# ajzhai/PEANUT

Measured on AMD Instinct MI355X. Metric: maps/sec for 480x480x(4+N_cat) prediction fwd, batch 32, higher is better.
Workload: dtype f32; 1 GPU; 480x480, 14-channel (4+10) partial maps -> 6-class prediction forward (PSPNet R50-V1c-D8), batch 32 per GPU, seeded random-init weights; survey_config=2, global_batch=32, parallelism=dp1 (map shards, no data-path collective)

## Files before the change

include/peanut_hip.h:

```cpp
#ifndef PEANUT_HIP_H_
#define PEANUT_HIP_H_

#include <stddef.h>
#include <stdint.h>

#ifdef __cplusplus
extern "C" {
#endif

#define PEANUT_OK 0
#define PEANUT_EINVAL (-2)
#define PEANUT_EHIP (-3)
#define PEANUT_EWEIGHTS (-4)
#define PEANUT_ERANGE (-5)

const char* peanut_last_error(void);
const char* peanut_last_conv_kernel(void);
int peanut_abi_version(void);
const char* peanut_build_arch(void);
const char* peanut_source_hash(void);
int peanut_debug_weight_pieces(const float* values, int n, int precision, unsigned short* pieces, float* pack_scale);
int peanut_debug_wino_weights(const float* w_oihw, int cout, int cin, int tile, float* out);
long long peanut_debug_deferred_splitk_count(void);
int peanut_debug_lds_canary(int workgroups, int lds_bytes, int rounds, int* mismatches, void* stream);
// ... 28 lines not shown
#define PEANUT_PREC_FP16X3 2
#define PEANUT_PREC_BF16X6 3

typedef struct peanut_tensor {
  const char* name;
  const float* data;
  int ndim;
  int64_t shape[4];
} peanut_tensor;

typedef struct peanut_pred peanut_pred_t;

int peanut_pred_create(peanut_pred_t** out, const peanut_pred_cfg* cfg, const peanut_tensor* tensors,
                       int n_tensors);
void peanut_pred_destroy(peanut_pred_t* h);

int peanut_pred_forward(peanut_pred_t* h, const float* in_dev, float* out_dev, int B, int H, int W,
                        int apply_sigmoid, void* stream);

size_t peanut_pred_workspace_bytes(peanut_pred_t* h, int B, int H, int W);

double peanut_pred_flops_per_map(peanut_pred_t* h, int H, int W);

int peanut_pred_debug_keep(peanut_pred_t* h, int keep);
int peanut_pred_debug_tensor(peanut_pred_t* h, const char* name, const float** dev_out, int dims[4]);
int peanut_pred_debug_read(peanut_pred_t* h, const char* name, float* dst_dev, size_t max_floats, int dims[4],
                           void* stream);

int peanut_pred_probe_enable(peanut_pred_t* h, int enable);
int peanut_pred_probe_collect(peanut_pred_t* h, int max_ops, const char** names, const char** kernels,
                              double* ms_sum, double* flops, double* bytes, int* n_forwards);
int peanut_pred_use_graph(peanut_pred_t* h, int enable);
int peanut_pred_set_option(peanut_pred_t* h, const char* key, long long value);
int peanut_pred_get_option(peanut_pred_t* h, const char* key, long long* value);


typedef struct peanut_map_cfg {
  int frame_height, frame_width;
  int map_resolution;
  int map_size_cm;
  int global_downscaling;
  int vision_range;
  double hfov;
  int du_scale;
  double cat_pred_threshold, exp_pred_threshold, map_pred_threshold;
  int num_sem_categories;
  double camera_height;
} peanut_map_cfg;

typedef struct peanut_map peanut_map_t;

int peanut_map_create(peanut_map_t** out, const peanut_map_cfg* cfg);
void peanut_map_destroy(peanut_map_t* h);
int peanut_map_dims(peanut_map_t* h, int dims[4]);

int peanut_map_forward(peanut_map_t* h, const float* obs, const float* pose_obs, const float* maps_last,
                       float* poses_inout, float* fp_map_pred, float* map_pred, void* stream);
int peanut_map_mark_agent(float* local_map, int channels, int m, int r0, int r1, int c0, int c1, const uint8_t* selem,
                          int selem_radius, int n_centres, const int* centres_rc, void* stream);
int peanut_map_use_graph(peanut_map_t* h, int enable);

#define PEANUT_MAP_MAX_BATCH 16
int peanut_map_reserve(peanut_map_t* h, int max_batch);
int peanut_map_forward_batch(peanut_map_t* h, int E, const float* obs, const float* pose_obs, const float* const* maps_last,
                             float* poses_inout, float* fp_map_pred, float* const* map_pred, void* stream);
int peanut_map_mark_agent_batch(int E, float* const* local_maps, int channels, int m, const int* squares, const uint8_t* selem,
                                int selem_radius, const int* n_centres, const int* centres_rc, void* stream);
int peanut_map_debug_launches(peanut_map_t* h);

typedef struct peanut_rcnn_cfg {
  int depth;
  int stem_out;
  int res2_out;
  int stride_in_1x1;
  int fpn_out;
  int num_anchors;
  int min_size, max_size;
  int size_divisibility;
  float pixel_mean[3], pixel_std[3];
  float bn_eps;
  int precision;
  int conv_algo;
  float anchor_sizes[5];
  float aspect_ratios[8];
  int rpn_pre_nms_topk;
  int rpn_post_nms_topk;
  float rpn_nms_thresh;
  float rpn_bbox_weights[4];
  int num_classes;
  int box_pooler_resolution, mask_pooler_resolution;
  int fc_dim;
  int mask_conv_dim, num_mask_convs;
  float roi_bbox_weights[4];
  float score_thresh_test;
  float nms_thresh_test;
  int detections_per_image;
  float mask_threshold;
} peanut_rcnn_cfg;

typedef struct peanut_rcnn peanut_rcnn_t;

int peanut_rcnn_create(peanut_rcnn_t** out, const peanut_rcnn_cfg* cfg, const peanut_tensor* tensors, int n_tensors);
void peanut_rcnn_destroy(peanut_rcnn_t* h);
int peanut_rcnn_set_option(peanut_rcnn_t* h, const char* key, long long value);
int peanut_rcnn_plan(peanut_rcnn_t* h, int B, int H, int W, int resized_hw[2], int padded_hw[2], int level_hw[10],
                     size_t* workspace_bytes, double* flops_per_image);
int peanut_rcnn_forward_front(peanut_rcnn_t* h, const uint8_t* img_bgr, int B, int H, int W, float* const* pyramid,
                              float* const* objectness, float* const* deltas, void* stream);

int peanut_rcnn_probe_front(peanut_rcnn_t* h, const uint8_t* img_bgr, int B, int H, int W, int reps, int max_ops,
                            const char** names, const char** kernels, double* ms, double* flops, void* stream);

int peanut_rcnn_set_stage_timing(peanut_rcnn_t* h, int on);
int peanut_rcnn_stage_times(peanut_rcnn_t* h, int max_stages, const char** names, const char** bounds, double* ms, double* work);

int peanut_rcnn_preprocess(peanut_rcnn_t* h, const uint8_t* img_bgr, int B, int H, int W, float* out_nchw, void* stream);

int peanut_rcnn_inference(peanut_rcnn_t* h, const uint8_t* img_bgr, int B, int H, int W, int* n_det_host, float* boxes,
                          float* scores, int32_t* classes, uint8_t* masks, void* stream);
int peanut_rcnn_semantic(peanut_rcnn_t* h, const uint8_t* img_bgr, int B, int H, int W, int n_cats, float sem_pred_prob_thr,
                         float goal_thr, const int32_t* goal_cat_host, float* semantic, int* n_det_host, float* boxes,
                         float* scores, int32_t* classes, uint8_t* masks, void* stream);
int peanut_rcnn_debug_stage(peanut_rcnn_t* h, const char* name, const void** dev, size_t* bytes);

int peanut_roi_align(const float* const* feats, const int* feat_hw, const float* scales, int n_levels, int C,
                     const float* rois, const int* levels, int n_rois, int pooled, int sampling_ratio, int aligned,
                     float* out, void* stream);
size_t peanut_nms_workspace_bytes(int n);
int peanut_nms(const float* boxes_sorted, const int* categories, int n, float iou_threshold, void* workspace,
               unsigned char* keep, void* stream);
int peanut_nms_segments(const float* boxes_sorted, const int* categories, const int* seg_offsets_host, int n_segments,
                        float iou_threshold, void* workspace, unsigned char* keep, void* stream);
int peanut_paste_masks(const float* masks, const float* boxes, int n, int M, int H, int W, float threshold,
                       unsigned char* out, void* stream);

int peanut_preprocess_obs(const uint8_t* rgb, const float* depth, const float* sem, int H, int W, int ncat, int ds,
                          double min_d, double max_d, float* obs, void* stream);
int peanut_preprocess_obs_batch(const uint8_t* rgb, const float* depth, const float* sem, int E, int H, int W, int ncat, int ds,
                                double min_d, double max_d, float* obs, void* stream);

int peanut_seg_accumulate(const uint8_t* masks, const int32_t* classes, const float* scores, int n, int H, int W,
                          int n_cats, float sem_pred_prob_thr, float goal_thr, int goal_cat, float* out,
                          void* stream);

typedef struct peanut_conv peanut_conv_t;
int peanut_conv_create(peanut_conv_t** out, const float* w_oihw_host, const float* scale_host,
                       const float* shift_host, int cout, int cin, int cin_pad, int kh, int kw, int stride,
                       int pad, int dil, int relu, int precision, int conv_algo);
void peanut_conv_destroy(peanut_conv_t* c);
int peanut_conv_precision(peanut_conv_t* c);
int peanut_conv_set_option(peanut_conv_t* c, const char* key, long long value);
int peanut_conv_forward(peanut_conv_t* c, const float* x_dev, const float* x2_dev, int c1, const float* res_dev,
                        float* y_dev, int B, int H, int W, void* stream);

typedef struct peanut_goal peanut_goal_t;
int peanut_goal_create(peanut_goal_t** out, int full_h, int full_w, int col_rad);
void peanut_goal_destroy(peanut_goal_t* g);
int peanut_goal_reset(peanut_goal_t* g);
int peanut_goal_rounds(peanut_goal_t* g);
int peanut_goal_passes(peanut_goal_t* g);
int peanut_goal_converged(peanut_goal_t* g);
int peanut_goal_traversible(peanut_goal_t* g, const float* full_obstacle, const uint8_t* collision_map,
                            const uint8_t* visited_vis, uint8_t* trav_out, void* stream);
int peanut_fmm_distance(peanut_goal_t* g, const uint8_t* traversible, const uint8_t* goal_mask, int goal_r, int goal_c,
                        int fill_mode, double* dist_out, void* stream);
int peanut_goal_select_begin(peanut_goal_t* g, const float* full_obstacle, const uint8_t* collision_map,
                             const uint8_t* visited_vis, const int lmb[4], int loc_r, int loc_c, void* stream);
int peanut_goal_select(peanut_goal_t* g, const float* full_obstacle, const uint8_t* collision_map,
                       const uint8_t* visited_vis, const int lmb[4], int loc_r, int loc_c, const float* target_pred,
                       double dist_weight_temperature, int map_resolution, int goal_rc_out[2], double stats_out[4],
                       double* dist_out, double* value_out, void* stream);
#define PEANUT_GOAL_MAX_BATCH 16
int peanut_goal_select_begin_batch(int E, peanut_goal_t* const* g, const float* const* full_obstacle,
                                   const uint8_t* const* collision_map, const uint8_t* const* visited_vis,
                                   const int* lmb, const int* loc_rc, void* stream);
int peanut_goal_select_batch(int E, peanut_goal_t* const* g, const float* const* full_obstacle,
                             const uint8_t* const* collision_map, const uint8_t* const* visited_vis,
                             const int* lmb, const int* loc_rc, const float* const* target_pred,
                             double dist_weight_temperature, int map_resolution, int* goal_rc_out, double* stats_out,
                             double* const* dist_out, double* const* value_out, void* stream);

#define PEANUT_COMM_ID_BYTES 128
typedef struct peanut_comm peanut_comm_t;
int peanut_comm_unique_id(unsigned char id[PEANUT_COMM_ID_BYTES]);
int peanut_comm_create(peanut_comm_t** out, int n_ranks, int rank, const unsigned char id[PEANUT_COMM_ID_BYTES]);
void peanut_comm_destroy(peanut_comm_t* c);
int peanut_comm_info(peanut_comm_t* c, int* n_ranks, int* rank);
const char* peanut_comm_backend(void);
int peanut_allgather_maps(peanut_comm_t* c, const float* local, float* all, size_t count, void* stream);

#ifdef __cplusplus
}
#endif
#endif
```

peanut_amd/_lib.py:

```python
from __future__ import annotations

import ctypes as C
import os
import threading

import torch

from . import build as _build

_LOCK = threading.Lock()
_LIB = None
ABI_VERSION = 17


class PeanutHipError(RuntimeError):
    pass


class PeanutRangeError(PeanutHipError, FloatingPointError):
    """PEANUT_ERANGE: precision fp16x3 and a value left fp16's exponent range (include/peanut_hip.h)."""


class PredCfgC(C.Structure):
    _fields_ = [
        ("in_channels", C.c_int), ("num_classes", C.c_int),
        ("strides", C.c_int * 4), ("dilations", C.c_int * 4), ("contract_dilation", C.c_int),
        ("pool_scales", C.c_int * 8), ("n_pool_scales", C.c_int),
        ("head_channels", C.c_int), ("align_corners", C.c_int), ("bn_eps", C.c_float),
        ("precision", C.c_int), ("fold_ppm", C.c_int), ("conv_algo", C.c_int),
    ]


class MapCfgC(C.Structure):
    _fields_ = [
        ("frame_height", C.c_int), ("frame_width", C.c_int), ("map_resolution", C.c_int),
        ("map_size_cm", C.c_int), ("global_downscaling", C.c_int), ("vision_range", C.c_int),
        ("hfov", C.c_double), ("du_scale", C.c_int),
        ("cat_pred_threshold", C.c_double), ("exp_pred_threshold", C.c_double),
        ("map_pred_threshold", C.c_double), ("num_sem_categories", C.c_int), ("camera_height", C.c_double),
    ]


class RcnnCfgC(C.Structure):
    _fields_ = [
        ("depth", C.c_int), ("stem_out", C.c_int), ("res2_out", C.c_int), ("stride_in_1x1", C.c_int),
        ("fpn_out", C.c_int), ("num_anchors", C.c_int), ("min_size", C.c_int), ("max_size", C.c_int),
        ("size_divisibility", C.c_int), ("pixel_mean", C.c_float * 3), ("pixel_std", C.c_float * 3),
        ("bn_eps", C.c_float), ("precision", C.c_int), ("conv_algo", C.c_int),
        ("anchor_sizes", C.c_float * 5), ("aspect_ratios", C.c_float * 8),
        ("rpn_pre_nms_topk", C.c_int), ("rpn_post_nms_topk", C.c_int), ("rpn_nms_thresh", C.c_float),
        ("rpn_bbox_weights", C.c_float * 4), ("num_classes", C.c_int), ("box_pooler_resolution", C.c_int),
        ("mask_pooler_resolution", C.c_int), ("fc_dim", C.c_int), ("mask_conv_dim", C.c_int), ("num_mask_convs", C.c_int),
        ("roi_bbox_weights", C.c_float * 4), ("score_thresh_test", C.c_float), ("nms_thresh_test", C.c_float),
        ("detections_per_image", C.c_int), ("mask_threshold", C.c_float),
    ]


class TensorC(C.Structure):
    _fields_ = [("name", C.c_char_p), ("data", C.c_void_p), ("ndim", C.c_int), ("shape", C.c_int64 * 4)]


_P = C.c_void_p
SIGNATURES = {
    "peanut_last_error": (C.c_char_p, []),
    "peanut_last_conv_kernel": (C.c_char_p, []),
    "peanut_abi_version": (C.c_int, []),
    "peanut_build_arch": (C.c_char_p, []),
    "peanut_source_hash": (C.c_char_p, []),
    "peanut_debug_weight_pieces": (C.c_int, [C.c_void_p, C.c_int, C.c_int, C.c_void_p, C.POINTER(C.c_float)]),
    "peanut_debug_wino_weights": (C.c_int, [C.c_void_p, C.c_int, C.c_int, C.c_int, C.c_void_p]),
    "peanut_debug_deferred_splitk_count": (C.c_longlong, []),
    "peanut_debug_lds_canary": (C.c_int, [C.c_int, C.c_int, C.c_int, C.c_void_p, C.c_void_p]),
    "peanut_debug_pkfma_canary": (C.c_int, [C.c_int, C.c_int, C.c_void_p, C.c_void_p]),
    "peanut_pred_create": (C.c_int, [C.POINTER(_P), C.POINTER(PredCfgC), C.POINTER(TensorC), C.c_int]),
    "peanut_pred_destroy": (None, [_P]),
    "peanut_pred_forward": (C.c_int, [_P, _P, _P, C.c_int, C.c_int, C.c_int, C.c_int, _P]),
    "peanut_pred_workspace_bytes": (C.c_size_t, [_P, C.c_int, C.c_int, C.c_int]),
    "peanut_pred_flops_per_map": (C.c_double, [_P, C.c_int, C.c_int]),
    "peanut_pred_debug_keep": (C.c_int, [_P, C.c_int]),
    "peanut_pred_debug_tensor": (C.c_int, [_P, C.c_char_p, C.POINTER(_P), C.POINTER(C.c_int * 4)]),
    "peanut_pred_debug_read": (C.c_int, [_P, C.c_char_p, _P, C.c_size_t, C.POINTER(C.c_int * 4), _P]),
    "peanut_pred_probe_enable": (C.c_int, [_P, C.c_int]),
    "peanut_pred_use_graph": (C.c_int, [_P, C.c_int]),
    "peanut_map_use_graph": (C.c_int, [_P, C.c_int]),
    "peanut_map_mark_agent": (C.c_int, [_P, C.c_int, C.c_int, C.c_int, C.c_int, C.c_int, C.c_int, _P, C.c_int, C.c_int, _P, _P]),
    "peanut_pred_probe_collect": (C.c_int, [_P, C.c_int, C.POINTER(C.c_char_p), C.POINTER(C.c_char_p),
                                            C.POINTER(C.c_double), C.POINTER(C.c_double), C.POINTER(C.c_double),
                                            C.POINTER(C.c_int)]),
    "peanut_map_create": (C.c_int, [C.POINTER(_P), C.POINTER(MapCfgC)]),
    "peanut_map_destroy": (None, [_P]),
    "peanut_map_dims": (C.c_int, [_P, C.POINTER(C.c_int * 4)]),
    "peanut_map_forward": (C.c_int, [_P, _P, _P, _P, _P, _P, _P, _P]),
    "peanut_map_reserve": (C.c_int, [_P, C.c_int]),
    "peanut_map_forward_batch": (C.c_int, [_P, C.c_int, _P, _P, C.POINTER(_P), _P, _P, C.POINTER(_P), _P]),
    "peanut_map_mark_agent_batch": (C.c_int, [C.c_int, C.POINTER(_P), C.c_int, C.c_int, C.POINTER(C.c_int), _P, C.c_int,
                                              C.POINTER(C.c_int), C.POINTER(C.c_int), _P]),
    "peanut_map_debug_launches": (C.c_int, [_P]),
    "peanut_preprocess_obs_batch": (C.c_int, [_P, _P, _P, C.c_int, C.c_int, C.c_int, C.c_int, C.c_int, C.c_double, C.c_double, _P, _P]),
    "peanut_rcnn_create": (C.c_int, [C.POINTER(_P), C.POINTER(RcnnCfgC), C.POINTER(TensorC), C.c_int]),
    "peanut_rcnn_destroy": (None, [_P]),
    "peanut_rcnn_plan": (C.c_int, [_P, C.c_int, C.c_int, C.c_int, C.POINTER(C.c_int * 2), C.POINTER(C.c_int * 2),
                                   C.POINTER(C.c_int * 10), C.POINTER(C.c_size_t), C.POINTER(C.c_double)]),
    "peanut_rcnn_forward_front": (C.c_int, [_P, _P, C.c_int, C.c_int, C.c_int, C.POINTER(_P), C.POINTER(_P),
                                            C.POINTER(_P), _P]),
    "peanut_rcnn_probe_front": (C.c_int, [_P, _P, C.c_int, C.c_int, C.c_int, C.c_int, C.c_int, C.POINTER(C.c_char_p), C.POINTER(C.c_char_p),
                                          C.POINTER(C.c_double), C.POINTER(C.c_double), _P]),
    "peanut_rcnn_set_stage_timing": (C.c_int, [_P, C.c_int]),
    "peanut_rcnn_stage_times": (C.c_int, [_P, C.c_int, C.POINTER(C.c_char_p), C.POINTER(C.c_char_p), C.POINTER(C.c_double), C.POINTER(C.c_double)]),
    "peanut_rcnn_preprocess": (C.c_int, [_P, _P, C.c_int, C.c_int, C.c_int, _P, _P]),
    "peanut_rcnn_inference": (C.c_int, [_P, _P, C.c_int, C.c_int, C.c_int, C.POINTER(C.c_int), _P, _P, _P, _P, _P]),
    "peanut_rcnn_semantic": (C.c_int, [_P, _P, C.c_int, C.c_int, C.c_int, C.c_int, C.c_float, C.c_float, C.POINTER(C.c_int32), _P,
                                       C.POINTER(C.c_int), _P, _P, _P, _P, _P]),
    "peanut_rcnn_debug_stage": (C.c_int, [_P, C.c_char_p, C.POINTER(_P), C.POINTER(C.c_size_t)]),
    "peanut_roi_align": (C.c_int, [C.POINTER(_P), C.POINTER(C.c_int), C.POINTER(C.c_float), C.c_int, C.c_int, _P, _P,
                                   C.c_int, C.c_int, C.c_int, C.c_int, _P, _P]),
    "peanut_nms_workspace_bytes": (C.c_size_t, [C.c_int]),
    "peanut_nms": (C.c_int, [_P, _P, C.c_int, C.c_float, _P, _P, _P]),
    "peanut_nms_segments": (C.c_int, [_P, _P, C.POINTER(C.c_int), C.c_int, C.c_float, _P, _P, _P]),
    "peanut_paste_masks": (C.c_int, [_P, _P, C.c_int, C.c_int, C.c_int, C.c_int, C.c_float, _P, _P]),
    "peanut_preprocess_obs": (C.c_int, [_P, _P, _P, C.c_int, C.c_int, C.c_int, C.c_int, C.c_double, C.c_double, _P, _P]),
    "peanut_seg_accumulate": (C.c_int, [_P, _P, _P, C.c_int, C.c_int, C.c_int, C.c_int, C.c_float, C.c_float,
                                        C.c_int, _P, _P]),
    "peanut_goal_create": (C.c_int, [C.POINTER(_P), C.c_int, C.c_int, C.c_int]),
    "peanut_goal_destroy": (None, [_P]),
    "peanut_goal_reset": (C.c_int, [_P]),
    "peanut_goal_rounds": (C.c_int, [_P]),
    "peanut_goal_passes": (C.c_int, [_P]),
    "peanut_goal_select_begin": (C.c_int, [_P, _P, _P, _P, _P, C.c_int, C.c_int, _P]),
    "peanut_goal_converged": (C.c_int, [_P]),
    "peanut_goal_traversible": (C.c_int, [_P, _P, _P, _P, _P, _P]),
    "peanut_fmm_distance": (C.c_int, [_P, _P, _P, C.c_int, C.c_int, C.c_int, _P, _P]),
    "peanut_goal_select": (C.c_int, [_P, _P, _P, _P, C.POINTER(C.c_int * 4), C.c_int, C.c_int, _P, C.c_double, C.c_int,
                                     C.POINTER(C.c_int * 2), C.POINTER(C.c_double * 4), _P, _P, _P]),
    "peanut_goal_select_begin_batch": (C.c_int, [C.c_int, C.POINTER(_P), C.POINTER(_P), C.POINTER(_P), C.POINTER(_P),
                                                 C.POINTER(C.c_int), C.POINTER(C.c_int), _P]),
    "peanut_goal_select_batch": (C.c_int, [C.c_int, C.POINTER(_P), C.POINTER(_P), C.POINTER(_P), C.POINTER(_P), C.POINTER(C.c_int),
                                           C.POINTER(C.c_int), C.POINTER(_P), C.c_double, C.c_int, C.POINTER(C.c_int),
                                           C.POINTER(C.c_double), C.POINTER(_P), C.POINTER(_P), _P]),
    "peanut_comm_unique_id": (C.c_int, [C.POINTER(C.c_ubyte * 128)]),
    "peanut_comm_create": (C.c_int, [C.POINTER(_P), C.c_int, C.c_int, C.POINTER(C.c_ubyte * 128)]),
    "peanut_comm_destroy": (None, [_P]),
    "peanut_comm_info": (C.c_int, [_P, C.POINTER(C.c_int), C.POINTER(C.c_int)]),
    "peanut_comm_backend": (C.c_char_p, []),
    "peanut_allgather_maps": (C.c_int, [_P, _P, _P, C.c_size_t, _P]),
    "peanut_conv_create": (C.c_int, [C.POINTER(_P), _P, _P, _P] + [C.c_int] * 11),
    "peanut_conv_destroy": (None, [_P]),
    "peanut_conv_precision": (C.c_int, [_P]),
    "peanut_conv_forward": (C.c_int, [_P, _P, _P, C.c_int, _P, _P, C.c_int, C.c_int, C.c_int, _P]),
    "peanut_set_default_option": (C.c_int, [C.c_char_p, C.c_longlong]),
    "peanut_get_default_option": (C.c_int, [C.c_char_p, C.POINTER(C.c_longlong)]),
    "peanut_option_list": (C.c_char_p, []),
    "peanut_pred_set_option": (C.c_int, [_P, C.c_char_p, C.c_longlong]),
    "peanut_pred_get_option": (C.c_int, [_P, C.c_char_p, C.POINTER(C.c_longlong)]),
    "peanut_conv_set_option": (C.c_int, [_P, C.c_char_p, C.c_longlong]),
    "peanut_rcnn_set_option": (C.c_int, [_P, C.c_char_p, C.c_longlong]),
}


CONV_ALGOS = {"auto": 0, "direct": 1}
PRECISIONS = {"fp32": 0, "bf16x3": 1, "fp16x3": 2, "bf16x6": 3}


def lib_path() -> str:
    return os.environ.get("PEANUT_HIP_LIB", _build.LIB_PATH)


def _stale_reason(lib, path) -> str:
    if path != _build.LIB_PATH or not os.path.isdir(_build.CSRC):
        return ""
    have = (lib.peanut_source_hash() or b"").decode()
    want = _build.source_hash()
    return "" if have == want else f"built from sources {have or '<unknown>'}, the tree holds {want}"


def load() -> C.CDLL:
    global _LIB
    with _LOCK:
        if _LIB is not None:
            return _LIB
        path = lib_path()
        if path == _build.LIB_PATH and os.path.exists(path) and os.path.isdir(_build.CSRC) and _build._built_hash() and \
                _build._built_hash() != _build.source_hash():
            try:
                _build.build()
            except Exception as e:
                raise PeanutHipError(f"{path} is stale (csrc/ changed since it was built) and rebuilding failed: {e}") from e
        if not os.path.exists(path):
            raise PeanutHipError(
                f"HIP extension not built: {path} is missing. Build it with "
                "`python -c 'import __graft_entry__ as g; g.build()'` (or `python -m peanut_amd.build`). "
                "peanut_amd has no CPU fallback.")
        try:
            lib = C.CDLL(path, mode=C.RTLD_LOCAL)
        except OSError as e:
            raise PeanutHipError(f"failed to load {path}: {e}") from e
        for name, (res, args) in SIGNATURES.items():
            try:
                fn = getattr(lib, name)
            except AttributeError as e:
                raise PeanutHipError(f"{path} does not export {name}; rebuild the extension") from e
            fn.restype = res
            fn.argtypes = args
        got = lib.peanut_abi_version()
        if got != ABI_VERSION:
            raise PeanutHipError(f"{path} implements ABI version {got}, this package binds version {ABI_VERSION}: "
                                 "rebuild the extension (python -m peanut_amd.build --force)")
        why = _stale_reason(lib, path)
        if why:
            raise PeanutHipError(f"{path} is stale: {why}.  Rebuild it (python -m peanut_amd.build --force); a stale kernel "
                                 "library must not answer for the sources next to it")
        _LIB = lib
        return lib


_OPTION_LOCK = threading.RLock()


class default_options:

    def __init__(self, **options):
        self.options = {k: int(v) for k, v in options.items()}
        self.saved = {}

    def __enter__(self):
        lib = load()
        _OPTION_LOCK.acquire()
        try:
            for k, v in self.options.items():
                old = C.c_longlong()
                check(lib.peanut_get_default_option(k.encode(), C.byref(old)), "peanut_get_default_option")
                self.saved[k] = old.value
                check(lib.peanut_set_default_option(k.encode(), v), "peanut_set_default_option")
        except Exception:
            self.__exit__(None, None, None)
            raise
        return self

    def __exit__(self, *exc):
        lib = load()
        try:
            for k, v in self.saved.items():
                lib.peanut_set_default_option(k.encode(), v)
            self.saved = {}
        finally:
            _OPTION_LOCK.release()
        return False


def check(rc: int, what: str = "") -> None:
    if rc != 0:
        msg = load().peanut_last_error()
        if rc == -5:
            raise PeanutRangeError(f"{what} failed (code {rc}): {msg.decode() if msg else ''}")
        raise PeanutHipError(f"{what} failed (code {rc}): {msg.decode() if msg else ''}")


def current_stream_ptr(device=None) -> int:
    return int(torch.cuda.current_stream(device).cuda_stream)
```

peanut_amd/csrc/common.h:

```cpp
#pragma once
#include <hip/hip_runtime.h>
#include <stdint.h>
#include <string>

namespace peanut {

void set_error(const std::string& msg);
int fail(int code, const std::string& msg);
void note_kernel(const char* family);
const char* noted_kernel();

#define PEANUT_HIP_CHECK(expr)                                                            \
  do {                                                                                    \
    hipError_t _e = (expr);                                                               \
    if (_e != hipSuccess)                                                                 \
      return ::peanut::fail(-3, std::string(#expr) + ": " + hipGetErrorString(_e));       \
  } while (0)

struct ConvDesc {
  int cin;
  int cout;
  int kh, kw, stride, pad, dil;
  int relu;
  int bn_tile;
  int bk;
  int cout_pad;
  const float* w_packed;
  const float* scale;
  const float* shift;
  int rs;
  const void* w_s;
  int s_planes;
  float s_alpha;
  int flush_ch;
};

struct DeferredSplit {
  bool valid;
  const float* partial;
  int split_p, ntiles, M, cout, relu;
  const float* scale;
  const float* shift;
  float alpha;
};

struct ConvArgs {
  const float* x;
  const float* x2;
  const float* res;
  float* y;
  int B, H, W;
  int c1, c2;
  int Ho, Wo;
  float* ws;
  size_t ws_floats;
  int mt_per_group;
  size_t w_group_stride;
  int ss_group_stride;
  int group_valid_rows;
  DeferredSplit* defer;
  const int* group_rows;
};

constexpr size_t kSplitKScratchFloats = (size_t)48 << 20;
constexpr size_t kSplitKSideFloats = (size_t)8 << 20;

#if defined(__HIP_DEVICE_COMPILE__)
#define PEANUT_NO_PK_F32 __attribute__((target("no-packed-fp32-ops")))
#else
#define PEANUT_NO_PK_F32
#endif

__device__ __forceinline__ float paste_value(const float* __restrict__ m, int M, const float* __restrict__ bx, int x, int y) {
#pragma clang fp contract(off)
  const float gx = ((float)x + 0.5f - bx[0]) / (bx[2] - bx[0]) * 2.f - 1.f;
  const float gy = ((float)y + 0.5f - bx[1]) / (bx[3] - bx[1]) * 2.f - 1.f;
  const float ix = ((gx + 1.f) * (float)M - 1.f) / 2.f, iy = ((gy + 1.f) * (float)M - 1.f) / 2.f;
  const float fx = floorf(ix), fy = floorf(iy);
  const int x0 = (int)fminf(fmaxf(fx, -2.f), (float)M + 1.f), y0 = (int)fminf(fmaxf(fy, -2.f), (float)M + 1.f);
  if (x0 < -1 || x0 >= M || y0 < -1 || y0 >= M) return 0.f;
  const float lx = ix - fx, ly = iy - fy;
  const float wx = 1.f - lx, wy = 1.f - ly;
  auto at = [&](int yy, int xx) -> float {
    return ((unsigned)yy < (unsigned)M && (unsigned)xx < (unsigned)M) ? m[yy * M + xx] : 0.f;
  };
  return at(y0, x0) * wy * wx + at(y0, x0 + 1) * wy * lx + at(y0 + 1, x0) * ly * wx + at(y0 + 1, x0 + 1) * ly * lx;
}

inline int conv_out_dim(int n, int k, int s, int p, int d) { return (n + 2 * p - d * (k - 1) - 1) / s + 1; }

void conv_pick_tiles(int cin_pad, int cout, int* bn_tile, int* bk, bool pointwise = false);
size_t conv_packed_floats(int cin_pad, int cout, int kh, int kw, int bn_tile);
void pack_conv_weights(const float* w_oihw, int cout, int cin_real, int cin_pad, int kh, int kw,
                       int bn_tile, int bk, float* out);
int launch_conv(const ConvDesc& d, const ConvArgs& a, hipStream_t stream);
bool conv_pw_enabled();
bool conv_pw_uses_256(int cout, long long M, int mt_per_group, int bn_tile, int cin);
int conv_pw_256_min_k();
bool conv_pw_uses_256w(int cout, long long M, int mt_per_group, int bn_tile, int cin, int flush_ktiles);
bool conv_pw_narrow_tiles(int cin, int cout, long long M, int bn_tile, int mt_per_group);
bool conv_pw_uses_256p(int cout, long long M, int mt_per_group, int bn_tile, int cin, int flush_ktiles, long long in_pixels = 0);
struct ConvKParams;
bool gemm_skinny_takes(const ConvKParams& p, int bn_tile, size_t ws_floats);
int launch_gemm_skinny(const ConvKParams& p, float* ws, size_t ws_floats, hipStream_t stream);
bool conv_pw_uses_256wp(int cout, long long M, int stride, int mt_per_group, int bn_tile, int c1, int c2, int flush_ktiles);
bool conv_pw_uses_ares(int cin, int cout, long long M, int stride, bool two_source, int flush_ktiles, int bn_tile);

bool conv_patch_eligible(const ConvDesc& d, const ConvArgs& a);
const char* conv_patch_kernel_name(const ConvDesc& d, bool nchw);
bool conv_patch_nchw_eligible(const ConvDesc& d, int B, int Ho, int Wo, int creal);
int launch_conv_patch_nchw(const ConvDesc& d, const float* x_nchw, int creal, float* y, int B, int H, int W, int Ho, int Wo, hipStream_t stream);

void wino_geometry(int B, int H, int W, int dil, int* th, int* tw, long long* n_tiles, long long* m_pad, int gran = 128, int m = 4);
void wino_transform_weights(const float* w_oihw, int cout, int cin, float* out, int m = 4);
int launch_wino_input(const float* x, float* V, int B, int H, int W, int C, int dil, hipStream_t s, int gran = 128, int m = 4, long long m_pad_total = 0,
                      const DeferredSplit* df = nullptr);
bool wino_input_accepts_deferred(int B, int H, int W, int C, int dil, int gran, int m);
long long wino_deferred_count();
int launch_wino_output(const float* Mb, const float* scale, const float* shift, const float* res, float* y,
                       int B, int H, int W, int C, int dil, int relu, hipStream_t s, int gran = 128, int m = 4, long long m_pad_total = 0);

bool gemm_rs_uses_256(int cout, long long M, int mt_per_group, int bn_tile, int cin);
const char* gemm_rs_kernel_name(int cout, long long M, int mt_per_group, int bn_tile, int cin, int planes);
size_t sx_packed_bytes(int cin_pad, int cout, int bn_tile, int planes);
void pack_weights_sx(const float* w, int cout, int cin_real, int cin_pad, int bn_tile, int planes, float wscale, void* out);
float sx_pack_scale(const float* w, size_t n, int planes);
size_t sx_conv_packed_bytes(int cin_pad, int cout, int kh, int kw, int bn_tile, int planes);
void pack_weights_sx_conv(const float* w_oihw, int cout, int cin_real, int cin_pad, int kh, int kw, int bn_tile, int planes,
                          float wscale, void* out);

int launch_nchw_to_nhwc_pad(const float* x, float* y, int B, int C, int H, int W, int Cpad, hipStream_t s);
int launch_maxpool3x3s2(const float* x, float* y, int B, int H, int W, int C, int Ho, int Wo, hipStream_t s);
int launch_ppm_pool(const float* x, float* out, int B, int H, int W, int C, const int* scales, int nscales,
                    hipStream_t s, int scale_rows = 0);
size_t ppm_pool_scratch_floats(int B, int H, int C, const int* scales, int nscales);
int launch_ppm_pool2(const float* x, float* scratch, float* out, int B, int H, int W, int C, const int* scales,
                     int nscales, hipStream_t s, int scale_rows = 0);
int launch_ppm_upsample_concat(const float* table, float* out, int B, int H, int W, int Cp, const int* scales,
                               int nscales, int align_corners, hipStream_t s);
int launch_ppm_conv_term(const float* Q, float* R, int B, int H, int W, int C, const int* scales, int nscales,
                         int align_corners, hipStream_t s, int scale_rows = 0);
int launch_upsample_logits(const float* lo, float* out, int B, int h, int w, int K, int H, int W,
                           int align_corners, int sigmoid, hipStream_t s);

}
```

peanut_amd/csrc/conv_common.h:

```cpp
#pragma once
#include <stdlib.h>

#include <atomic>

#include "common.h"
#include "options.h"

namespace peanut {

typedef float f32x16 __attribute__((ext_vector_type(16)));
typedef float f32x4 __attribute__((ext_vector_type(4)));

__device__ __forceinline__ float relu_keep_nan(float v) { return v < 0.f ? 0.f : v; }
__device__ __forceinline__ f32x4 relu_keep_nan(f32x4 v) {
  return f32x4{relu_keep_nan(v.x), relu_keep_nan(v.y), relu_keep_nan(v.z), relu_keep_nan(v.w)};
}

struct ConvKParams {
  const float* x;
  const float* x2;
  const float* w;
  const float* scale;
  const float* shift;
  const float* res;
  const float* zeros;
  float* y;
  int H, W, c1, c2, Ho, Wo, cout;
  int kw, ntaps, stride, pad, dil, relu;
  int M, nkt, ntiles, HoWo;
  int n_full, n_sp, split_p;
  float* partial;
  int mt_per_group;
  long long w_group_stride;
  int ss_group_stride;
  int mtiles;
  int nchunk;
  int res_prefetch;
  float alpha;
  int ares_pbn;
  int phase_shift;
  int sk_units, sk_maxp, sk_g, sk_q;
  int pack_bn;
  int group_valid;
  int p_order;
  float* dump;
  int stagger;
  int flush;
  DeferredSplit* defer;
  const int* group_rows;
};

template <int I>
struct IC { static constexpr int value = I; };
template <int N, int I = 0, class F>
__device__ __forceinline__ void static_for(F&& f) {
  if constexpr (I < N) {
    f(IC<I>{});
    static_for<N, I + 1>(f);
  }
}

struct KIter {
  int tap, ky, kx, cbase;
  const float* wtile;
};


const float* zero_page();
bool conv_pw_enabled();
int launch_conv_pw(const ConvKParams& p, int bn_tile, float* ws, size_t ws_floats, hipStream_t stream);
int launch_conv_pw_ares(const ConvKParams& p, int bn_tile, hipStream_t stream);
int launch_conv_pw256p(const ConvKParams& p, float* ws, size_t ws_floats, hipStream_t stream);
int launch_conv_pw256wp(const ConvKParams& p, float* ws, size_t ws_floats, hipStream_t stream);
int launch_conv_patch(const ConvKParams& p, const ConvDesc& d, int B, hipStream_t stream);
int launch_gemm_rs(const ConvKParams& p, int bn_tile, int planes, float* ws, size_t ws_floats, hipStream_t stream);
int launch_conv_rs(const ConvKParams& p, int bn_tile, int planes, float* ws, size_t ws_floats, hipStream_t stream);


struct Work { int mt, nt, kt0, kt1, item; };

__host__ __device__ __forceinline__ int sk_owner(long long U, int G, long long u) {
  int w = (int)(u * G / U);
  while (w + 1 < G && U * (w + 1) / G <= u) ++w;
  while (w > 0 && U * w / G > u) --w;
  return w;
}

__device__ __forceinline__ void tile_to_mn(const ConvKParams& p, int tile, int* mt_out, int* nt_out) {
  int mt, nt;
  if (p.nchunk > 0 && p.ntiles > p.nchunk) {
    const int full = p.ntiles / p.nchunk, rem = p.ntiles - full * p.nchunk;
    const int per_chunk = p.mtiles * p.nchunk;
    if (tile < full * per_chunk) {
      const int c = tile / per_chunk, r = tile - c * per_chunk;
      mt = r / p.nchunk;
      nt = c * p.nchunk + (r - mt * p.nchunk);
    } else {
      const int r = tile - full * per_chunk;
      mt = r / rem;
      nt = full * p.nchunk + (r - mt * rem);
    }
  } else {
    mt = tile / p.ntiles;
    nt = tile - mt * p.ntiles;
  }
  *mt_out = mt;
  *nt_out = nt;
}

__device__ __forceinline__ Work decode_work(const ConvKParams& p) {
  const int G = gridDim.x, bid = blockIdx.x;
  const int q = G >> 3, r = G & 7, xcd = bid & 7, local = bid >> 3;
  const int sq = p.n_sp >> 3, sr = p.n_sp & 7;
  const int sp_x = sq + (xcd < sr), sp_before = xcd * sq + (xcd < sr ? xcd : sr);
  const int chunk_before = xcd * q + (xcd < r ? xcd : r);
  Work w;
  int tile;
  if (local < sp_x) {
    const int s = sp_before + local;
    const int j = s / p.split_p, part = s - j * p.split_p;
    tile = p.n_full + j;
    w.item = s;
    w.kt0 = (int)((long long)part * p.nkt / p.split_p);
    w.kt1 = (int)((long long)(part + 1) * p.nkt / p.split_p);
  } else {
    tile = (chunk_before - sp_before) + (local - sp_x);
    w.item = -1;
    w.kt0 = 0;
    w.kt1 = p.nkt;
  }
  tile_to_mn(p, tile, &w.mt, &w.nt);
  return w;
}

constexpr int kResPrefetchRows = 8;
struct ResPrefetch { f32x4 v[kResPrefetchRows]; bool on; };

template <int BM, int BN, int EP, int NT>
__device__ __forceinline__ ResPrefetch conv_res_prefetch(const ConvKParams& p, const Work& wk, int m0, int n0) {
  constexpr int NV = BN / 4, ROWS_PER_PASS = NT / NV, ER = BM / EP;
  const int tid = threadIdx.x;
  const int c4 = (tid % NV) * 4, r0 = tid / NV, n = n0 + c4;
  ResPrefetch r;
  r.on = p.res_prefetch && p.res && wk.item < 0 && (p.cout & 3) == 0 && n < p.cout;
  if (r.on) {
#pragma unroll
    for (int i = 0; i < kResPrefetchRows; ++i) {
      const int row = r0 + i * ROWS_PER_PASS, m = m0 + row;
      r.v[i] = (row < ER && m < p.M) ? *reinterpret_cast<const f32x4*>(p.res + (size_t)m * p.cout + n) : f32x4{0.f, 0.f, 0.f, 0.f};
    }
  }
  return r;
}

template <int BM, int BN, int WM, int WN, int EP, int NT = 256, int MI = 0, int NI = 0>
__device__ __forceinline__ void conv_epilogue(const ConvKParams& p, const Work& wk, f32x16 (&acc)[MI][NI], float* smem,
                                              int m0, int n0, const ResPrefetch* early = nullptr) {
  constexpr int TM = BM / WM, TN = BN / WN;
  constexpr int CS = BN + 4, ER = BM / EP;
  static_assert(MI == TM / 32 && NI == TN / 32, "accumulator shape");
  const int tid = threadIdx.x;
  const int lane = tid & 63, wave = tid >> 6;
  const int wm = wave / WN, wn = wave % WN;
  const int li = lane & 31, hi = lane >> 5;
  constexpr int NV = BN / 4;
  constexpr int ROWS_PER_PASS = NT / NV;
  const int c4 = (tid % NV) * 4, r0 = tid / NV;
  const int n = n0 + c4;
  const int ss_off = (p.mt_per_group && p.ss_group_stride) ? (wk.mt / p.mt_per_group) * p.ss_group_stride : 0;
  const f32x4 sc = *reinterpret_cast<const f32x4*>(p.scale + ss_off + n) * p.alpha;
  const f32x4 sh = *reinterpret_cast<const f32x4*>(p.shift + ss_off + n);
  const bool vec_ok = (p.cout & 3) == 0;
  constexpr int PRE = kResPrefetchRows;
  const ResPrefetch rp = early ? *early : conv_res_prefetch<BM, BN, EP, NT>(p, wk, m0, n0);
  const f32x4 (&rpre)[PRE] = rp.v;
  const bool pre = rp.on;
#pragma unroll
  for (int ep = 0; ep < EP; ++ep) {
    if (EP == 1 || wm == ep) {
#pragma unroll
      for (int t = 0; t < MI; ++t)
#pragma unroll
        for (int u = 0; u < NI; ++u)
#pragma unroll
          for (int r = 0; r < 16; ++r) {
            const int row = wm * TM + t * 32 + (r & 3) + 8 * (r >> 2) + 4 * hi - ep * ER;
            smem[row * CS + wn * TN + u * 32 + li] = acc[t][u][r];
          }
    }
    __syncthreads();
    if (wk.item >= 0) {
      float* dst = p.partial + (size_t)wk.item * (BM * BN) + (size_t)ep * ER * BN;
      for (int row = r0; row < ER; row += ROWS_PER_PASS)
        *reinterpret_cast<f32x4*>(dst + row * BN + c4) = *reinterpret_cast<const f32x4*>(smem + row * CS + c4);
    } else {
      int row_first = r0;
      if (pre && ep == 0) {
#pragma unroll
        for (int i = 0; i < PRE; ++i) {
          const int row = r0 + i * ROWS_PER_PASS, m = m0 + row;
          if (row < ER && m < p.M) {
            f32x4 v = *reinterpret_cast<const f32x4*>(smem + row * CS + c4);
            v = v * sc + sh;
// ... 193 lines not shown
```

peanut_amd/csrc/conv_igemm.hip:

```cpp
#include <stdlib.h>

#include "conv_common.h"

namespace peanut {

template <int BN, int BK, int A_PER>
__device__ __forceinline__ void prep_addr(const ConvKParams& p, KIter& it, const int (&a_iy0)[A_PER],
                                          const int (&a_ix0)[A_PER], const int (&a_pix)[A_PER], int a_c4,
                                          unsigned long long (&a_addr)[A_PER], const float*& b_tile) {
  const bool second = it.cbase >= p.c1;
  const float* src = second ? p.x2 : p.x;
  const int C = second ? p.c2 : p.c1, cb = second ? it.cbase - p.c1 : it.cbase;
  const int dy = it.ky * p.dil, dx = it.kx * p.dil;
  static_for<A_PER>([&](auto J) __attribute__((always_inline)) {
    constexpr int j = decltype(J)::value;
    const int iy = a_iy0[j] + dy, ix = a_ix0[j] + dx;
    const bool ok = (unsigned)iy < (unsigned)p.H && (unsigned)ix < (unsigned)p.W;
    const float* ptr = src + (size_t)(a_pix[j] + iy * p.W + ix) * C + cb + a_c4;
    const unsigned long long m = ok ? ~0ull : 0ull;
    a_addr[j] = ((unsigned long long)ptr & m) | ((unsigned long long)p.zeros & ~m);
  });
  b_tile = it.wtile;
  it.wtile += BN * BK;
  const int tap1 = it.tap + 1, kx1 = it.kx + 1;
// ... 100 lines not shown
#define PEANUT_STORE_TILES(stage) store_tiles<BM, BN, BK, A_PER, B_PER>(stage, tid, ra, rb)

  const int lane = tid & 63, wave = tid >> 6;
  const int wm = wave / WN, wn = wave % WN;
  const int li = lane & 31, hi = lane >> 5;
  const int a_off = (wm * TM + li) * LS + hi * 4;
  const int b_off = BM * LS + (wn * TN + li) * LS + hi * 4;

  f32x16 acc[MI][NI];
#pragma unroll
  for (int t = 0; t < MI; ++t)
#pragma unroll
    for (int u = 0; u < NI; ++u)
#pragma unroll
      for (int r = 0; r < 16; ++r) acc[t][u][r] = 0.f;

  PEANUT_PREP_ADDR();
  PEANUT_ISSUE_LOADS();
  PEANUT_STORE_TILES(smem);
  PEANUT_PREP_ADDR();
  if (nk > 1) PEANUT_ISSUE_LOADS();
  PEANUT_PREP_ADDR();
  __syncthreads();

  constexpr int KH = BK / 16;
  f32x4 afA[KH][MI], bfA[KH][NI], afB[KH][MI], bfB[KH][NI];
#define PEANUT_LOAD_FRAGS(af, bf, stage, half)                                                           \
  _Pragma("unroll") for (int j = 0; j < KH; ++j) {                                                       \
    _Pragma("unroll") for (int t = 0; t < MI; ++t)                                                       \
      af[j][t] = *reinterpret_cast<const f32x4*>((stage) + a_off + t * 32 * LS + ((half) * KH + j) * 8); \
    _Pragma("unroll") for (int u = 0; u < NI; ++u)                                                       \
      bf[j][u] = *reinterpret_cast<const f32x4*>((stage) + b_off + u * 32 * LS + ((half) * KH + j) * 8); \
  }
#define PEANUT_MFMA_HALF(af, bf)                                                                         \
  _Pragma("unroll") for (int j = 0; j < KH; ++j)                                                         \
    _Pragma("unroll") for (int kk = 0; kk < 4; ++kk)                                                     \
      _Pragma("unroll") for (int t = 0; t < MI; ++t)                                                     \
        _Pragma("unroll") for (int u = 0; u < NI; ++u)                                                   \
          acc[t][u] = __builtin_amdgcn_mfma_f32_32x32x2f32(af[j][t][kk], bf[j][u][kk], acc[t][u], 0, 0, 0);

  PEANUT_LOAD_FRAGS(afA, bfA, smem, 0);
  int kt = 0;
  for (; kt + 2 < nk; ++kt) {
    float* const nxt = smem + ((kt + 1) & 1) * STAGE;
    const float* const cur = smem + (kt & 1) * STAGE;
    PEANUT_STORE_TILES(nxt);
    PEANUT_ISSUE_LOADS();
    PEANUT_LOAD_FRAGS(afB, bfB, cur, 1);
    __builtin_amdgcn_sched_barrier(0);
    PEANUT_PREP_ADDR();
    PEANUT_MFMA_HALF(afA, bfA);
    __builtin_amdgcn_sched_barrier(0);
    __syncthreads();
    PEANUT_LOAD_FRAGS(afA, bfA, nxt, 0);
    __builtin_amdgcn_sched_barrier(0);
    PEANUT_MFMA_HALF(afB, bfB);
    __builtin_amdgcn_sched_barrier(0);
  }
  if (kt + 1 < nk) {
    float* const nxt = smem + ((kt + 1) & 1) * STAGE;
    const float* const cur = smem + (kt & 1) * STAGE;
    PEANUT_STORE_TILES(nxt);
    PEANUT_LOAD_FRAGS(afB, bfB, cur, 1);
    __builtin_amdgcn_sched_barrier(0);
    PEANUT_MFMA_HALF(afA, bfA);
    __builtin_amdgcn_sched_barrier(0);
    __syncthreads();
    PEANUT_LOAD_FRAGS(afA, bfA, nxt, 0);
    __builtin_amdgcn_sched_barrier(0);
    PEANUT_MFMA_HALF(afB, bfB);
    __builtin_amdgcn_sched_barrier(0);
    ++kt;
  }
  {
    const float* const cur = smem + (kt & 1) * STAGE;
    PEANUT_LOAD_FRAGS(afB, bfB, cur, 1);
    __builtin_amdgcn_sched_barrier(0);
    PEANUT_MFMA_HALF(afA, bfA);
    PEANUT_MFMA_HALF(afB, bfB);
  }
  __syncthreads();
#undef PEANUT_LOAD_FRAGS
#undef PEANUT_MFMA_HALF

  conv_epilogue<BM, BN, WM, WN, EP>(p, wk, acc, smem, m0, n0);
}

const float* zero_page() {
  static float* pages[64] = {nullptr};
  int dev = 0;
  if (hipGetDevice(&dev) != hipSuccess || dev < 0 || dev >= 64) return nullptr;
  if (!pages[dev]) {
    float* ptr = nullptr;
    if (hipMalloc(&ptr, 4096) != hipSuccess) return nullptr;
    if (hipMemset(ptr, 0, 4096) != hipSuccess) return nullptr;
    pages[dev] = ptr;
  }
  return pages[dev];
}

void conv_pick_tiles(int cin_pad, int cout, int* bn_tile, int* bk, bool pointwise) {
  const int forced_bk = (int)opt(OPT_FP32_BK);
  *bk = (cin_pad % 32 == 0) ? 32 : 16;
  if (forced_bk == 16) *bk = 16;
  *bn_tile = cout >= 128 ? 128 : (cout > 32 ? 64 : 32);
  const int bn64_maxk = (int)opt(pointwise ? OPT_PW_BN64_MAXK : OPT_BN64_MAXK);
  if (*bn_tile == 128 && cin_pad <= bn64_maxk) *bn_tile = 64;
}

size_t conv_packed_floats(int cin_pad, int cout, int kh, int kw, int bn_tile) {
  const int cout_pad = (cout + bn_tile - 1) / bn_tile * bn_tile;
  return (size_t)cout_pad * kh * kw * cin_pad;
}

void pack_conv_weights(const float* w, int cout, int cin_real, int cin_pad, int kh, int kw, int bn_tile,
                       int bk, float* out) {
  const int ntaps = kh * kw;
  const int cout_pad = (cout + bn_tile - 1) / bn_tile * bn_tile;
  const int nchunks = cin_pad / bk;
  const int nkt = nchunks * ntaps;
  for (int n = 0; n < cout_pad; ++n) {
    const int nt = n / bn_tile, nn = n % bn_tile;
    for (int ch = 0; ch < nchunks; ++ch)
      for (int tap = 0; tap < ntaps; ++tap) {
        float* dst = out + (((size_t)nt * nkt + (size_t)ch * ntaps + tap) * bn_tile + nn) * bk;
        for (int c = 0; c < bk; ++c) {
          const int ci = ch * bk + c;
          dst[c] = (n < cout && ci < cin_real) ? w[((size_t)n * cin_real + ci) * ntaps + tap] : 0.f;
        }
      }
  }
}

template <int BM, int BN, int BK, int WM, int WN>
static int launch_t(const ConvKParams& p, float* ws, size_t ws_floats, hipStream_t stream) {
  static SlotCache slots;
  return launch_with_tail_split<decltype(&conv_igemm_kernel<BM, BN, BK, WM, WN>), BM, BN>(
      &conv_igemm_kernel<BM, BN, BK, WM, WN>, p, ws, ws_floats, stream, &slots);
}

int launch_conv(const ConvDesc& d, const ConvArgs& a, hipStream_t stream) {
  if (a.c1 + a.c2 != d.cin) return fail(-2, "launch_conv: c1 + c2 != cin");
  const bool rs_fallback = d.rs == 1 && a.c2 != 0 && d.stride != 1;
  const int kgran = (d.rs && !rs_fallback) ? 16 : d.bk;
  if (a.c1 % kgran != 0 || (a.c2 % kgran) != 0) return fail(-2, "launch_conv: channel split not a multiple of the k-tile");
  ConvKParams p{};
  p.x = a.x; p.x2 = a.x2 ? a.x2 : a.x; p.w = d.w_packed; p.scale = d.scale; p.shift = d.shift;
  p.res = a.res; p.y = a.y;
  p.zeros = zero_page();
  if (!p.zeros) return fail(-3, "launch_conv: zero page allocation failed");
  p.H = a.H; p.W = a.W; p.c1 = a.c1; p.c2 = a.c2; p.Ho = a.Ho; p.Wo = a.Wo; p.cout = d.cout;
  p.kw = d.kw; p.ntaps = d.kh * d.kw; p.stride = d.stride; p.pad = d.pad; p.dil = d.dil; p.relu = d.relu;
  p.HoWo = a.Ho * a.Wo;
  const long long M = (long long)a.B * p.HoWo;
  if (M <= 0 || M > 0x7fffffffLL || (long long)a.B * a.H * a.W > 0x7fffffffLL)
    return fail(-2, "launch_conv: problem size out of range");
  p.M = (int)M;
  p.nkt = (d.cin / d.bk) * p.ntaps;
  p.ntiles = d.cout_pad / d.bn_tile;
  p.n_full = 0; p.n_sp = 0; p.split_p = 1; p.partial = nullptr;
  p.alpha = 1.f;
  p.flush = (d.rs && !rs_fallback) ? 0 : d.flush_ch / d.bk;
  p.mt_per_group = a.mt_per_group; p.w_group_stride = (long long)a.w_group_stride; p.ss_group_stride = a.ss_group_stride;
  p.group_valid = a.mt_per_group ? a.group_valid_rows : 0;
  if (a.defer) a.defer->valid = false;
  p.defer = a.defer;
  p.group_rows = a.mt_per_group ? a.group_rows : nullptr;
  if (d.rs && !rs_fallback) {
    if (!d.w_s) return fail(-2, "launch_conv: register-split layer without pre-split weights");
    p.w = static_cast<const float*>(d.w_s);
    p.nkt = (d.cin / 16) * p.ntaps;
    p.alpha = d.s_alpha;
    if (d.rs == 2) return launch_conv_rs(p, d.bn_tile, d.s_planes, a.ws, a.ws_floats, stream);
    return launch_gemm_rs(p, d.bn_tile, d.s_planes, a.ws, a.ws_floats, stream);
  }
  if (d.bk == 32 && p.ntaps == 1 && p.pad == 0 && p.c1 % 32 == 0 && p.c2 % 32 == 0 && (p.c2 == 0 || p.stride == 1) && conv_pw_enabled())
    return launch_conv_pw(p, d.bn_tile, a.ws, a.ws_floats, stream);
  if (conv_patch_eligible(d, a)) return launch_conv_patch(p, d, a.B, stream);
  {
    static const char* const names[2][3] = {{"conv_igemm_128x128x32", "conv_igemm_128x64x32", "conv_igemm_128x32x32"},
                                            {"conv_igemm_128x128x16", "conv_igemm_128x64x16", "conv_igemm_128x32x16"}};
    note_kernel(names[d.bk == 32 ? 0 : 1][d.bn_tile == 128 ? 0 : (d.bn_tile == 64 ? 1 : 2)]);
  }
  if (d.bk == 32) {
    if (d.bn_tile == 128) return launch_t<128, 128, 32, 2, 2>(p, a.ws, a.ws_floats, stream);
    if (d.bn_tile == 64) return launch_t<128, 64, 32, 2, 2>(p, a.ws, a.ws_floats, stream);
    if (d.bn_tile == 32) return launch_t<128, 32, 32, 4, 1>(p, a.ws, a.ws_floats, stream);
  } else if (d.bk == 16) {
    if (d.bn_tile == 128) return launch_t<128, 128, 16, 2, 2>(p, a.ws, a.ws_floats, stream);
    if (d.bn_tile == 64) return launch_t<128, 64, 16, 2, 2>(p, a.ws, a.ws_floats, stream);
    if (d.bn_tile == 32) return launch_t<128, 32, 16, 4, 1>(p, a.ws, a.ws_floats, stream);
  }
  return fail(-2, "launch_conv: unsupported tile configuration");
}

}
```

peanut_amd/csrc/conv_pw.hip:

```cpp
#include <stdlib.h>

#include "common.h"
#include "conv_common.h"

namespace peanut {

namespace {

typedef const __attribute__((address_space(1))) void* gptr_t;
typedef __attribute__((address_space(3))) void* lptr_t;

template <int BN, int WM, int WN>
__global__ __launch_bounds__(256) __attribute__((amdgpu_waves_per_eu(BN == 128 ? 2 : (BN == 64 ? 3 : 4))))
void conv_pw_glds_kernel(const ConvKParams p) {
  constexpr int BM = 128, BK = 32;
  constexpr int TM = BM / WM, TN = BN / WN;
  constexpr int MI = TM / 32, NI = TN / 32;
  constexpr int A_FLOATS = BM * BK, B_FLOATS = BN * BK, STAGE = A_FLOATS + B_FLOATS;
  constexpr int A_INSTR = BM / 32, B_INSTR = BN / 32;
  constexpr int CS = BN + 4;
  constexpr int EP = (BM * CS > 2 * STAGE) ? WM : 1;
  constexpr int ER = BM / EP;
  constexpr int SMEM_FLOATS = (2 * STAGE > ER * CS) ? 2 * STAGE : ER * CS;
  static_assert(WM * WN == 4 && TM % 32 == 0 && TN % 32 == 0, "4 waves, wave tile a multiple of 32x32");
  __shared__ __attribute__((aligned(1024))) float smem[SMEM_FLOATS];

  const int tid = threadIdx.x;
  const Work wk = decode_work(p);
  const int mt = wk.mt, nt = wk.nt, nk = wk.kt1 - wk.kt0;
  const int m0 = mt * BM, n0 = nt * BN;
  const int lane = tid & 63;
  const int wave = __builtin_amdgcn_readfirstlane(tid >> 6);
  const int lr = lane >> 3, lp = lane & 7;

  const float* a_src[A_INSTR];
  const float* a_src2[A_INSTR];
#pragma unroll
  for (int j = 0; j < A_INSTR; ++j) {
    const int r = (wave * A_INSTR + j) * 8 + lr;
    const int m = m0 + r;
    const int mc = m < p.M ? m : p.M - 1;
    const int b = mc / p.HoWo;
    const int rem = mc - b * p.HoWo;
    const int oy = rem / p.Wo, ox = rem - oy * p.Wo;
    const size_t pix = (size_t)b * p.H * p.W + (size_t)oy * p.stride * p.W + (size_t)ox * p.stride;
    const int c = lp ^ ((r >> 1) & 7);
    const int k1 = p.c1 / BK;
    a_src[j] = wk.kt0 < k1 ? p.x + pix * p.c1 + (size_t)wk.kt0 * BK + c * 4 : p.x2 + pix * p.c2 + (size_t)(wk.kt0 - k1) * BK + c * 4;
    a_src2[j] = p.x2 + pix * p.c2 + c * 4;
  }
  int to_switch = p.c2 ? p.c1 / BK - wk.kt0 : 0x7fffffff;
  const float* b_src[B_INSTR];
  {
    const int pack = p.pack_bn > BN ? p.pack_bn : BN;
    const int n_row = nt * BN;
    const float* wtile = p.w + (p.mt_per_group ? (size_t)(mt / p.mt_per_group) * p.w_group_stride : 0) +
                         ((size_t)(n_row / pack) * p.nkt + wk.kt0) * ((size_t)pack * BK) + (size_t)(n_row % pack) * BK;
#pragma unroll
    for (int j = 0; j < B_INSTR; ++j) {
      const int r = (wave * B_INSTR + j) * 8 + lr;
      const int c = lp ^ ((r >> 1) & 7);
      b_src[j] = wtile + r * BK + c * 4;
    }
  }
  const int b_step = (p.pack_bn > BN ? p.pack_bn : BN) * BK;
#define PEANUT_DMA_TILE(stage)                                                                                   \
  {                                                                                                              \
    if (to_switch-- == 0) {                                                                                      \
      _Pragma("unroll") for (int j = 0; j < A_INSTR; ++j) a_src[j] = a_src2[j];                                  \
    }                                                                                                            \
    _Pragma("unroll") for (int j = 0; j < A_INSTR; ++j) {                                                        \
      __builtin_amdgcn_global_load_lds((gptr_t)a_src[j], (lptr_t)((stage) + (wave * A_INSTR + j) * 256), 16, 0, 0); \
      a_src[j] += BK;                                                                                            \
    }                                                                                                            \
    _Pragma("unroll") for (int j = 0; j < B_INSTR; ++j) {                                                        \
      __builtin_amdgcn_global_load_lds((gptr_t)b_src[j], (lptr_t)((stage) + A_FLOATS + (wave * B_INSTR + j) * 256), 16, 0, 0); \
      b_src[j] += b_step;                                                                                        \
    }                                                                                                            \
  }
#define PEANUT_DMA_LANDED_BARRIER()          \
  asm volatile("s_waitcnt vmcnt(0)" ::: "memory"); \
  __syncthreads();

  const int wm = wave / WN, wn = wave % WN;
  const int li = lane & 31, hi = lane >> 5;
  const int swz = (li >> 1) & 7;
  int sw[BK / 8];
#pragma unroll
  for (int ks = 0; ks < BK / 8; ++ks) sw[ks] = ((ks * 2 + hi) ^ swz) * 4;
  const int a_row = (wm * TM + li) * BK;
  const int b_row = A_FLOATS + (wn * TN + li) * BK;

  f32x16 acc[MI][NI];
#pragma unroll
  for (int t = 0; t < MI; ++t)
#pragma unroll
    for (int u = 0; u < NI; ++u)
#pragma unroll
      for (int r = 0; r < 16; ++r) acc[t][u][r] = 0.f;
  PEANUT_FLUSH_DECL();

  constexpr int KH = BK / 16;
  f32x4 afA[KH][MI], bfA[KH][NI], afB[KH][MI], bfB[KH][NI];
#define PEANUT_LOAD_FRAGS(af, bf, stage, half)                                                          \
  _Pragma("unroll") for (int j = 0; j < KH; ++j) {                                                      \
    _Pragma("unroll") for (int t = 0; t < MI; ++t)                                                      \
      af[j][t] = *reinterpret_cast<const f32x4*>((stage) + a_row + t * 32 * BK + sw[(half) * KH + j]);  \
    _Pragma("unroll") for (int u = 0; u < NI; ++u)                                                      \
      bf[j][u] = *reinterpret_cast<const f32x4*>((stage) + b_row + u * 32 * BK + sw[(half) * KH + j]);  \
  }
#define PEANUT_MFMA_HALF(af, bf)                                                                        \
  _Pragma("unroll") for (int j = 0; j < KH; ++j)                                                        \
    _Pragma("unroll") for (int kk = 0; kk < 4; ++kk)                                                    \
      _Pragma("unroll") for (int t = 0; t < MI; ++t)                                                    \
        _Pragma("unroll") for (int u = 0; u < NI; ++u)                                                  \
          acc[t][u] = __builtin_amdgcn_mfma_f32_32x32x2f32(af[j][t][kk], bf[j][u][kk], acc[t][u], 0, 0, 0);

  PEANUT_DMA_TILE(smem);
  PEANUT_DMA_LANDED_BARRIER();
  PEANUT_LOAD_FRAGS(afA, bfA, smem, 0);

  int kt = 0;
  for (; kt + 1 < nk; ++kt) {
    float* const nxt = smem + ((kt + 1) & 1) * STAGE;
    const float* const cur = smem + (kt & 1) * STAGE;
    PEANUT_DMA_TILE(nxt);
    PEANUT_LOAD_FRAGS(afB, bfB, cur, 1);
    __builtin_amdgcn_sched_barrier(0);
    PEANUT_MFMA_HALF(afA, bfA);
    __builtin_amdgcn_sched_barrier(0);
    PEANUT_DMA_LANDED_BARRIER();
    PEANUT_LOAD_FRAGS(afA, bfA, nxt, 0);
    __builtin_amdgcn_sched_barrier(0);
    PEANUT_MFMA_HALF(afB, bfB);
    __builtin_amdgcn_sched_barrier(0);
    PEANUT_FLUSH_STEP();
  }
  const ResPrefetch rp = conv_res_prefetch<BM, BN, EP, 256>(p, wk, m0, n0);
  {
    const float* const cur = smem + (kt & 1) * STAGE;
    PEANUT_LOAD_FRAGS(afB, bfB, cur, 1);
    __builtin_amdgcn_sched_barrier(0);
    PEANUT_MFMA_HALF(afA, bfA);
    PEANUT_MFMA_HALF(afB, bfB);
  }
  PEANUT_FLUSH_FINISH();
  __syncthreads();
#undef PEANUT_LOAD_FRAGS
#undef PEANUT_MFMA_HALF
#undef PEANUT_DMA_TILE
#undef PEANUT_DMA_LANDED_BARRIER

  conv_epilogue<BM, BN, WM, WN, EP>(p, wk, acc, smem, m0, n0, &rp);
}

__global__ __launch_bounds__(512) void conv_pw_glds256_kernel(const ConvKParams p) {
  constexpr int BM = 256, BN = 128, BK = 32, WM = 4, WN = 2, NT = 512, STAGES = 3;
  constexpr int TM = BM / WM, TN = BN / WN;
  constexpr int MI = TM / 32, NI = TN / 32;
  constexpr int A_FLOATS = BM * BK, B_FLOATS = BN * BK, STAGE = A_FLOATS + B_FLOATS;
  constexpr int A_INSTR = BM / 64, B_INSTR = BN / 64;
  constexpr int CS = BN + 4;
  constexpr int SMEM_FLOATS = (STAGES * STAGE > BM * CS) ? STAGES * STAGE : BM * CS;
  __shared__ __attribute__((aligned(1024))) float smem[SMEM_FLOATS];

  const int tid = threadIdx.x;
  const Work wk = decode_work(p);
  const int mt = wk.mt, nt = wk.nt, nk = wk.kt1 - wk.kt0;
  const int m0 = mt * BM, n0 = nt * BN;
  const int lane = tid & 63;
  const int wave = __builtin_amdgcn_readfirstlane(tid >> 6);
  const int lr = lane >> 3, lp = lane & 7;

  const float* a_src[A_INSTR];
  const float* a_src2[A_INSTR];
#pragma unroll
  for (int j = 0; j < A_INSTR; ++j) {
    const int r = (wave * A_INSTR + j) * 8 + lr;
    const int m = m0 + r;
    const int mc = m < p.M ? m : p.M - 1;
    const int b = mc / p.HoWo;
    const int rem = mc - b * p.HoWo;
    const int oy = rem / p.Wo, ox = rem - oy * p.Wo;
    const size_t pix = (size_t)b * p.H * p.W + (size_t)oy * p.stride * p.W + (size_t)ox * p.stride;
    const int c = lp ^ ((r >> 1) & 7);
    const int k1 = p.c1 / BK;
    a_src[j] = wk.kt0 < k1 ? p.x + pix * p.c1 + (size_t)wk.kt0 * BK + c * 4 : p.x2 + pix * p.c2 + (size_t)(wk.kt0 - k1) * BK + c * 4;
    a_src2[j] = p.x2 + pix * p.c2 + c * 4;
  }
  int to_switch = p.c2 ? p.c1 / BK - wk.kt0 : 0x7fffffff;
  const float* b_src[B_INSTR];
  {
    const float* wtile = p.w + (p.mt_per_group ? (size_t)(mt / p.mt_per_group) * p.w_group_stride : 0) +
                         ((size_t)nt * p.nkt + wk.kt0) * (BN * BK);
#pragma unroll
    for (int j = 0; j < B_INSTR; ++j) {
      const int r = (wave * B_INSTR + j) * 8 + lr;
      const int c = lp ^ ((r >> 1) & 7);
      b_src[j] = wtile + r * BK + c * 4;
    }
  }
#define PW256_DMA_TILE(stage)                                                                                    \
// ... 90 lines not shown
#undef PW256_MFMA_GROUP
  PEANUT_FLUSH_FINISH();
  conv_epilogue<BM, BN, WM, WN, 1, NT>(p, wk, acc, smem, m0, n0);
}

__global__ __launch_bounds__(512) void conv_pw_glds256w_kernel(const ConvKParams p) {
  constexpr int BM = 256, BN = 256, BK = 32, WM = 4, WN = 2, NT = 512, STAGES = 2;
  constexpr int TM = BM / WM, TN = BN / WN;
  constexpr int MI = TM / 32, NI = TN / 32;
  constexpr int A_FLOATS = BM * BK, B_FLOATS = BN * BK, STAGE = A_FLOATS + B_FLOATS;
  constexpr int A_INSTR = BM / 64, B_INSTR = BN / 64;
  constexpr int CS = BN + 4, ER = BM / WM;
  constexpr int SMEM_FLOATS = (STAGES * STAGE > ER * CS) ? STAGES * STAGE : ER * CS;
  __shared__ __attribute__((aligned(1024))) float smem[SMEM_FLOATS];

  const int tid = threadIdx.x;
  const Work wk = decode_work(p);
  const int mt = wk.mt, nt = wk.nt, nk = wk.kt1 - wk.kt0;
  const int m0 = mt * BM, n0 = nt * BN;
  const int lane = tid & 63;
  const int wave = __builtin_amdgcn_readfirstlane(tid >> 6);
  const int lr = lane >> 3, lp = lane & 7;

  const float* a_src[A_INSTR];
  const float* a_src2[A_INSTR];
#pragma unroll
  for (int j = 0; j < A_INSTR; ++j) {
    const int r = (wave * A_INSTR + j) * 8 + lr;
    const int m = m0 + r;
    const int mc = m < p.M ? m : p.M - 1;
    const int b = mc / p.HoWo;
    const int rem = mc - b * p.HoWo;
    const int oy = rem / p.Wo, ox = rem - oy * p.Wo;
    const size_t pix = (size_t)b * p.H * p.W + (size_t)oy * p.stride * p.W + (size_t)ox * p.stride;
    const int c = lp ^ ((r >> 1) & 7);
    const int k1 = p.c1 / BK;
    a_src[j] = wk.kt0 < k1 ? p.x + pix * p.c1 + (size_t)wk.kt0 * BK + c * 4 : p.x2 + pix * p.c2 + (size_t)(wk.kt0 - k1) * BK + c * 4;
    a_src2[j] = p.x2 + pix * p.c2 + c * 4;
  }
  int to_switch = p.c2 ? p.c1 / BK - wk.kt0 : 0x7fffffff;
  const float* b_src[B_INSTR];
#pragma unroll
  for (int j = 0; j < B_INSTR; ++j) {
    const int r = (wave * B_INSTR + j) * 8 + lr;
    const int c = lp ^ ((r >> 1) & 7);
    b_src[j] = p.w + ((size_t)(2 * nt + (r >> 7)) * p.nkt + wk.kt0) * (128 * BK) + (r & 127) * BK + c * 4;
  }
#define PW256W_DMA_TILE(stage)                                                                                   \
  {                                                                                                              \
    if (to_switch-- == 0) {                                                                                      \
      _Pragma("unroll") for (int j = 0; j < A_INSTR; ++j) a_src[j] = a_src2[j];                                  \
    }                                                                                                            \
    _Pragma("unroll") for (int j = 0; j < A_INSTR; ++j) {                                                        \
      __builtin_amdgcn_global_load_lds((gptr_t)a_src[j], (lptr_t)((stage) + (wave * A_INSTR + j) * 256), 16, 0, 0); \
      a_src[j] += BK;                                                                                            \
    }                                                                                                            \
    _Pragma("unroll") for (int j = 0; j < B_INSTR; ++j) {                                                        \
      __builtin_amdgcn_global_load_lds((gptr_t)b_src[j], (lptr_t)((stage) + A_FLOATS + (wave * B_INSTR + j) * 256), 16, 0, 0); \
      b_src[j] += 128 * BK;                                                                                      \
    }                                                                                                            \
  }
#define PW256W_BARRIER()                                  \
  asm volatile("s_waitcnt lgkmcnt(0)" ::: "memory");      \
  __builtin_amdgcn_s_barrier();                           \
  asm volatile("" ::: "memory");

  const int wm = wave / WN, wn = wave % WN;
  const int li = lane & 31, hi = lane >> 5;
  const int swz = (li >> 1) & 7;
  int sw[BK / 8];
#pragma unroll
  for (int ks = 0; ks < BK / 8; ++ks) sw[ks] = ((ks * 2 + hi) ^ swz) * 4;
  const int a_row = (wm * TM + li) * BK;
  const int b_row = A_FLOATS + (wn * TN + li) * BK;

  f32x16 acc[MI][NI];
#pragma unroll
  for (int t = 0; t < MI; ++t)
#pragma unroll
    for (int u = 0; u < NI; ++u)
#pragma unroll
      for (int r = 0; r < 16; ++r) acc[t][u][r] = 0.f;

  PW256W_DMA_TILE(smem);
  asm volatile("s_waitcnt vmcnt(0)" ::: "memory");
  PW256W_BARRIER();
  const bool late = p.phase_shift && wave >= 4;
#define PW256W_READ_PAIR(g)                                                                                          \
  _Pragma("unroll") for (int j = 0; j < 2; ++j) {                                                                    \
    _Pragma("unroll") for (int t = 0; t < MI; ++t) af[j][t] = *reinterpret_cast<const f32x4*>(cur + a_row + t * 32 * BK + sw[(g) + j]); \
    _Pragma("unroll") for (int u = 0; u < NI; ++u) bf[j][u] = *reinterpret_cast<const f32x4*>(cur + b_row + u * 32 * BK + sw[(g) + j]); \
  }
#define PW256W_MFMA_PAIR()                                                                                \
  _Pragma("unroll") for (int j = 0; j < 2; ++j)                                                           \
    _Pragma("unroll") for (int kk = 0; kk < 4; ++kk)                                                      \
      _Pragma("unroll") for (int t = 0; t < MI; ++t)                                                      \
        _Pragma("unroll") for (int u = 0; u < NI; ++u)                                                    \
          acc[t][u] = __builtin_amdgcn_mfma_f32_32x32x2f32(af[j][t][kk], bf[j][u][kk], acc[t][u], 0, 0, 0);
  for (int kt = 0; kt < nk; ++kt) {
    const float* const cur = smem + (kt & 1) * STAGE;
    float* const fill = smem + ((kt + 1) & 1) * STAGE;
    const bool more = kt + 1 < nk;
    if (more && !late) PW256W_DMA_TILE(fill);
    f32x4 af[2][MI], bf[2][NI];
    PW256W_READ_PAIR(0);
    PW256W_MFMA_PAIR();
    __builtin_amdgcn_sched_barrier(0);
    if (more && late) PW256W_DMA_TILE(fill);
    __builtin_amdgcn_sched_barrier(0);
    PW256W_READ_PAIR(2);
    PW256W_MFMA_PAIR();
    asm volatile("s_waitcnt vmcnt(0)" ::: "memory");
    PW256W_BARRIER();
  }
#undef PW256W_DMA_TILE
#undef PW256W_BARRIER
#undef PW256W_READ_PAIR
#undef PW256W_MFMA_PAIR
  conv_epilogue<BM, BN, WM, WN, WM, NT>(p, wk, acc, smem, m0, n0);
}

template <int BN, int WM, int WN>
int launch_pw_t(const ConvKParams& p, float* ws, size_t ws_floats, hipStream_t stream) {
  static SlotCache slots;
  return launch_with_tail_split<decltype(&conv_pw_glds_kernel<BN, WM, WN>), 128, BN>(&conv_pw_glds_kernel<BN, WM, WN>, p, ws,
                                                                                      ws_floats, stream, &slots);
}

}

bool conv_pw_enabled() { return opt(OPT_PW_GLDS) != 0; }

int conv_pw_256_min_k() { return (int)opt(OPT_PW256_MINK); }
bool conv_pw_uses_256(int cout, long long M, int mt_per_group, int bn_tile, int cin) {
  const long long min_tiles = opt(OPT_PW256_MINTILES);
  return bn_tile == 128 && cin >= conv_pw_256_min_k() && mt_per_group % 2 == 0 && M * cout >= min_tiles * 256 * 128;
}

bool conv_pw_uses_256w(int cout, long long M, int mt_per_group, int bn_tile, int cin, int flush) {
  const int min_k = (int)opt(OPT_PW256W_MINK);
  const long long min_tiles = opt(OPT_PW256W_MINTILES);
  return min_k > 0 && bn_tile == 128 && cout % 256 == 0 && mt_per_group == 0 && flush == 0 && cin >= min_k &&
         ((M + 255) / 256) * (cout / 256) >= min_tiles;
}

bool conv_pw_narrow_tiles(int cin, int cout, long long M, int bn_tile, int mt_per_group) {
  (void)mt_per_group;
  if (bn_tile != 128 || cin > opt(OPT_BN64_MAXK) || cout % 128 != 0) return false;
  return ((M + 127) / 128) * (cout / 128) < opt(OPT_PW64_MAXTILES);
}

int launch_conv_pw(const ConvKParams& p, int bn_tile, float* ws, size_t ws_floats, hipStream_t stream) {
  const int phase_shift_w = opt(OPT_PW256_PHASE) != 0;
  if (gemm_skinny_takes(p, bn_tile, ws ? ws_floats : 0)) return launch_gemm_skinny(p, ws, ws_floats, stream);
  if (conv_pw_uses_256wp(p.cout, p.M, p.stride, p.mt_per_group, bn_tile, p.c1, p.c2, p.flush)) {
    const int rc = launch_conv_pw256wp(p, ws, ws_floats, stream);
    if (rc != 1) return rc;
  }
  if (conv_pw_uses_ares(p.c1, p.cout, p.M, p.stride, p.c2 != 0, p.flush, bn_tile)) return launch_conv_pw_ares(p, bn_tile, stream);
  if (conv_pw_uses_256w(p.cout, p.M, p.mt_per_group, bn_tile, p.c1 + p.c2, p.flush)) {
    static SlotCache slots256w;
    ConvKParams q = p;
    q.ntiles = p.cout / 256;
    q.phase_shift = phase_shift_w;
    note_kernel("conv_pw_glds_256x256");
    return launch_with_tail_split<decltype(&conv_pw_glds256w_kernel), 256, 256, 512>(&conv_pw_glds256w_kernel, q, ws, ws_floats, stream,
                                                                                      &slots256w);
  }
  if (conv_pw_uses_256p(p.cout, p.M, p.mt_per_group, bn_tile, p.c1 + p.c2, p.flush, (long long)(p.M / p.HoWo) * p.H * p.W) && !(p.flush && p.res)) {
    const int rc = launch_conv_pw256p(p, ws, ws_floats, stream);
    if (rc != 1) return rc;
  }
  if (conv_pw_uses_256(p.cout, p.M, p.mt_per_group, bn_tile, p.c1 + p.c2)) {
    static SlotCache slots256;
    ConvKParams q = p;
    if (q.mt_per_group) q.mt_per_group /= 2;
    q.phase_shift = phase_shift_w;
    if (opt(OPT_PW256_SKIP_PAD) == 0) q.group_valid = 0;
    note_kernel("conv_pw_glds_256x128");
    return launch_with_tail_split<decltype(&conv_pw_glds256_kernel), 256, 128, 512>(&conv_pw_glds256_kernel, q, ws, ws_floats, stream,
                                                                                     &slots256);
  }
  if (conv_pw_narrow_tiles(p.c1 + p.c2, p.cout, p.M, bn_tile, p.mt_per_group)) {
    ConvKParams q = p;
    q.pack_bn = 128;
    q.ntiles = p.ntiles * 2;
    note_kernel("conv_pw_glds_128x64");
    return launch_pw_t<64, 2, 2>(q, ws, ws_floats, stream);
  }
  note_kernel(bn_tile == 128 ? "conv_pw_glds_128x128" : (bn_tile == 64 ? "conv_pw_glds_128x64" : "conv_pw_glds_128x32"));
  if (bn_tile == 128) return launch_pw_t<128, 2, 2>(p, ws, ws_floats, stream);
  if (bn_tile == 64) return launch_pw_t<64, 2, 2>(p, ws, ws_floats, stream);
  if (bn_tile == 32) return launch_pw_t<32, 4, 1>(p, ws, ws_floats, stream);
  return fail(-2, "launch_conv_pw: unsupported tile configuration");
}

}
```

peanut_amd/csrc/conv_pw256p.hip:

```cpp
#include <stdlib.h>

#include "common.h"
#include "conv_common.h"

namespace peanut {

namespace {

typedef const __attribute__((address_space(1))) void* gptr_t;
typedef __attribute__((address_space(3))) void* lptr_t;

__device__ __forceinline__ float p_load_uncounted(const float* base, unsigned byte_off) {
  float v;
  asm volatile("s_nop 4\n\tglobal_load_dword %0, %1, %2" : "=v"(v) : "v"(byte_off), "s"(base) : "memory");
  return v;
}
template <int N>
__device__ __forceinline__ void p_wait(const float (&r)[8], float a, float b, float c, float d) {
  __builtin_amdgcn_sched_barrier(0);
  if constexpr (N == 6)
    asm volatile("s_waitcnt vmcnt(6)" ::"v"(r[0]), "v"(r[1]), "v"(r[2]), "v"(r[3]), "v"(r[4]), "v"(r[5]), "v"(r[6]), "v"(r[7]), "v"(a), "v"(b),
                 "v"(c), "v"(d)
                 : "memory");
  else
    asm volatile("s_waitcnt vmcnt(0)" ::"v"(r[0]), "v"(r[1]), "v"(r[2]), "v"(r[3]), "v"(r[4]), "v"(r[5]), "v"(r[6]), "v"(r[7]), "v"(a), "v"(b),
                 "v"(c), "v"(d)
                 : "memory");
  __builtin_amdgcn_sched_barrier(0);
}

struct PItem { int mt, nt, kt0, kt1, part; };

template <bool RAGGED, bool FLUSH>
__global__ __launch_bounds__(512) void conv_pw_glds256p_kernel(const ConvKParams p) {
  constexpr int BM = 256, BN = 128, BK = 32, WN = 2;
  constexpr int A_FLOATS = BM * BK, B_FLOATS = BN * BK, STAGE = A_FLOATS + B_FLOATS;
  constexpr int A_INSTR = 4, B_INSTR = 2;
  constexpr int kMaxItems = 120;
  __shared__ __attribute__((aligned(1024))) float smem[3 * STAGE + kMaxItems * 8];
  int* const plan = reinterpret_cast<int*>(smem + 3 * STAGE);

  const int tid = threadIdx.x, lane = tid & 63;
  const int wave = __builtin_amdgcn_readfirstlane(tid >> 6);
  const int lr = lane >> 3, lp = lane & 7;
  const int wm = wave / WN, wn = wave % WN;
  const int li = lane & 31, hi = lane >> 5;
  const bool late = p.phase_shift && wave >= 4;

  const int G = gridDim.x, bid = blockIdx.x;
  const int lw = (bid & 7) * (G >> 3) + (bid >> 3);
  const int nf = p.n_full / G;
  const int sp0 = (int)((long long)p.n_sp * lw / G), sp1 = (int)((long long)p.n_sp * (lw + 1) / G);
  const long long skU = p.sk_units;
  const int u0 = (skU > 0 && lw < p.sk_g) ? (int)(skU * lw / p.sk_g) : 0, u1 = (skU > 0 && lw < p.sk_g) ? (int)(skU * (lw + 1) / p.sk_g) : 0;
  const int upt = skU > 0 ? p.nkt / p.sk_q : 1;
  const int n_frag = u1 > u0 ? (u1 - 1) / upt - u0 / upt + 1 : 0;
  const int n_items = nf + (skU > 0 ? n_frag : sp1 - sp0);
  if (n_items == 0) return;
  if (n_items > kMaxItems) __builtin_trap();
  if (tid < n_items) {
    const int i = tid;
    PItem it;
    int tile;
    if (i >= nf && skU > 0) {
      const int j = u0 / upt + (i - nf);
      const int t0 = j * upt;
      it.kt0 = ((u0 > t0 ? u0 : t0) - t0) * p.sk_q;
      it.kt1 = ((u1 < t0 + upt ? u1 : t0 + upt) - t0) * p.sk_q;
      it.part = j * p.sk_maxp + (lw - sk_owner(skU, p.sk_g, (long long)t0));
      tile = p.n_full + j;
    } else if (i < nf) {
      tile = p.p_order ? (lw / (G >> 3)) * (nf * (G >> 3)) + i * (G >> 3) + lw % (G >> 3) : lw * nf + i;
      it.kt0 = 0; it.kt1 = p.nkt; it.part = -1;
    } else {
      const int s = sp0 + (i - nf);
      const int j = s / p.split_p, part = s - j * p.split_p;
      tile = p.n_full + j;
      it.part = s;
      it.kt0 = (int)((long long)part * p.nkt / p.split_p);
      it.kt1 = (int)((long long)(part + 1) * p.nkt / p.split_p);
    }
    tile_to_mn(p, tile, &it.mt, &it.nt);
    int* e = plan + i * 8;
    e[0] = it.mt; e[1] = it.nt; e[2] = it.kt0; e[3] = it.kt1; e[4] = it.part;
  }
  __syncthreads();
  auto item_at = [&](int i) {
    const int* e = plan + i * 8;
    PItem it;
    it.mt = __builtin_amdgcn_readfirstlane(e[0]);
    it.nt = __builtin_amdgcn_readfirstlane(e[1]);
    it.kt0 = __builtin_amdgcn_readfirstlane(e[2]);
    it.kt1 = __builtin_amdgcn_readfirstlane(e[3]);
    it.part = __builtin_amdgcn_readfirstlane(e[4]);
    return it;
  };

  unsigned a_pix[A_INSTR], a_chunk[A_INSTR], b_off[B_INSTR];
#pragma unroll
  for (int j = 0; j < A_INSTR; ++j) {
    const int r = (wave * A_INSTR + j) * 8 + lr;
    a_chunk[j] = (unsigned)((lp ^ ((r >> 1) & 7)) * 16);
    a_pix[j] = 0;
  }
#pragma unroll
  for (int j = 0; j < B_INSTR; ++j) {
    const int r = (wave * B_INSTR + j) * 8 + lr;
    b_off[j] = (unsigned)(r * BK * 4 + (lp ^ ((r >> 1) & 7)) * 16);
  }
  int d_item = 0, d_left = 0, d_kt = 0;
  const float* d_wtile = p.w;
  auto cursor_open = [&](int i) {
    const PItem it = item_at(i);
    const int m0 = it.mt * BM;
#pragma unroll
    for (int j = 0; j < A_INSTR; ++j) {
      int m = m0 + (wave * A_INSTR + j) * 8 + lr;
      if (RAGGED) m = m < p.M ? m : p.M - 1;
      const int b = m / p.HoWo;
      const int rem = m - b * p.HoWo;
      const int oy = rem / p.Wo, ox = rem - oy * p.Wo;
      a_pix[j] = (unsigned)(b * p.H * p.W + oy * p.stride * p.W + ox * p.stride);
    }
    d_wtile = p.w + (p.mt_per_group ? (size_t)(it.mt / p.mt_per_group) * p.w_group_stride : 0) + (size_t)it.nt * p.nkt * (BN * BK);
    d_kt = it.kt0;
    d_left = it.kt1 - it.kt0;
  };
  const int k1 = p.c1 / BK;
  auto request = [&](float* stage) {
    const bool live = d_left > 0;
    if (!live) --d_kt;
    const bool second = d_kt >= k1;
    const char* abase = reinterpret_cast<const char*>(second ? p.x2 : p.x) + (size_t)(second ? d_kt - k1 : d_kt) * (BK * 4);
    const unsigned cbytes = (unsigned)(second ? p.c2 : p.c1) * 4u;
#pragma unroll
    for (int j = 0; j < A_INSTR; ++j)
      __builtin_amdgcn_global_load_lds((gptr_t)(abase + (a_pix[j] * cbytes + a_chunk[j])), (lptr_t)(stage + (wave * A_INSTR + j) * 256), 16, 0, 0);
    const char* bbase = reinterpret_cast<const char*>(d_wtile + (size_t)d_kt * (BN * BK));
#pragma unroll
    for (int j = 0; j < B_INSTR; ++j)
      __builtin_amdgcn_global_load_lds((gptr_t)(bbase + b_off[j]), (lptr_t)(stage + A_FLOATS + (wave * B_INSTR + j) * 256), 16, 0, 0);
    ++d_kt;
    if (live) --d_left;
  };
  auto cursor_advance = [&]() {
    if (d_left == 0 && d_item + 1 < n_items) {
      ++d_item;
      cursor_open(d_item);
    }
  };

  const int swz = (li >> 1) & 7;
  int sw[4];
#pragma unroll
  for (int ks = 0; ks < 4; ++ks) sw[ks] = ((ks * 2 + hi) ^ swz) * 4;
  const int a_row = (wm * 64 + li) * BK;
  const int b_row = A_FLOATS + (wn * 64 + li) * BK;

  f32x16 acc[2][2], prev[2][2], acc2[2][2];
#pragma unroll
  for (int t = 0; t < 2; ++t)
#pragma unroll
    for (int u = 0; u < 2; ++u)
#pragma unroll
      for (int r = 0; r < 16; ++r) { acc[t][u][r] = 0.f; prev[t][u][r] = 0.f; acc2[t][u][r] = 0.f; }
#define P256_PREV(t, u, r) (FLUSH ? acc2[t][u][r] : prev[t][u][r])
#define P256_FLUSH_STEP()                                                                                 \
  if (FLUSH) {                                                                                            \
    _Pragma("unroll") for (int t = 0; t < 2; ++t)                                                         \
      _Pragma("unroll") for (int u = 0; u < 2; ++u) {                                                     \
        acc2[t][u] += acc[t][u];                                                                          \
        _Pragma("unroll") for (int r = 0; r < 16; ++r) acc[t][u][r] = 0.f;                                \
      }                                                                                                   \
  }

  const int cout = p.cout;
  bool prev_valid = false, prev_raw = false;
  const float* prev_res = p.zeros;
  float* prev_out = p.y;
  const float* prev_ss = p.scale;
  unsigned prev_rs = 0;
  unsigned prev_os = (unsigned)cout * 4;
  int prev_rows = BM;
  const unsigned lane_row = (unsigned)(wm * 64 + 4 * hi), lane_col = (unsigned)(wn * 64 + li);
  const unsigned ss_lane = lane_col * 4;
  const unsigned shift_delta = (unsigned)((p.shift - p.scale) * 4);
  float sc0 = 1.f, sc1 = 1.f, sh0 = 0.f, sh1 = 0.f;
  const bool has_res = p.res != nullptr;
  const float alpha = p.alpha;
  const bool relu = p.relu != 0;

#define P256_EPI_SS_LOADS()                                                                                       \
  {                                                                                                               \
    sc0 = p_load_uncounted(prev_ss, ss_lane);                                                                     \
    sc1 = p_load_uncounted(prev_ss, ss_lane + 128);                                                               \
    sh0 = p_load_uncounted(prev_ss, ss_lane + shift_delta);                                                       \
    sh1 = p_load_uncounted(prev_ss, ss_lane + shift_delta + 128);                                                 \
  }
#define P256_EPI_LOADS(c)                                                                                         \
  float resv[8];                                                                                                  \
  {                                                                                                               \
    if ((c) == 0) {                                                                                               \
      sc0 = p_load_uncounted(prev_ss, ss_lane);                                                                   \
      sc1 = p_load_uncounted(prev_ss, ss_lane + 128);                                                             \
      sh0 = p_load_uncounted(prev_ss, ss_lane + shift_delta);                                                     \
      sh1 = p_load_uncounted(prev_ss, ss_lane + shift_delta + 128);                                               \
    }                                                                                                             \
    const unsigned lane_off = (lane_row * prev_rs) + (prev_rs ? lane_col * 4 : 0);                                \
                                                      \
    int row_limit = prev_rows - 1;                                                                                \
    if (RAGGED) asm volatile("" : "+s"(row_limit));                                                               \
    _Pragma("unroll") for (int i = 0; i < 8; ++i) {                                                               \
      const int r = ((c) & 1) * 8 + i, row = ((c) >> 2) * 32 + (r & 3) + 8 * (r >> 2);                            \
      unsigned roff = lane_off + (unsigned)row * prev_rs;                                                         \
      if (RAGGED) {                                                                                               \
        const int rr = (int)lane_row + row;                                                                       \
                                           \
        roff = __umul24((unsigned)(rr < row_limit ? rr : row_limit), prev_rs) + (prev_rs ? lane_col * 4 : 0);     \
      }                                                                                                           \
      resv[i] = p_load_uncounted(prev_res, roff + (prev_rs ? (((c) >> 1) & 1) * 128u : 0u));                      \
    }                                                                                                             \
  }
#define P256_EPI_FINISH(c) P256_EPI_FINISH_RV(c, resv)
#define P256_EPI_FINISH_RV(c, RV)                                                                                 \
  if (prev_valid) {                                                                                               \
    const float scv = (((c) >> 1) & 1) ? sc1 : sc0, shv = (((c) >> 1) & 1) ? sh1 : sh0;                           \
    char* const obase = reinterpret_cast<char*>(prev_out) + (lane_row * prev_os + lane_col * 4 + (((c) >> 1) & 1) * 128u); \
    _Pragma("unroll") for (int i = 0; i < 8; ++i) {                                                               \
      const int r = ((c) & 1) * 8 + i, row = ((c) >> 2) * 32 + (r & 3) + 8 * (r >> 2);                            \
      float v = P256_PREV((c) >> 2, ((c) >> 1) & 1, r);                                                           \
      if (!prev_raw) {                                                                                            \
        v = v * (scv * alpha) + shv;                                                                              \
        v += RV[i];                                                                                               \
        if (relu) v = relu_keep_nan(v);                                                                           \
      }                                                                                                           \
      if (!RAGGED || (int)lane_row + row < prev_rows) *reinterpret_cast<float*>(obase + (unsigned)row * prev_os) = v; \
    }                                                                                                             \
  }

  cursor_open(0);
  request(smem);
  cursor_advance();
  request(smem + STAGE);
  cursor_advance();
  asm volatile("s_waitcnt vmcnt(6)" ::: "memory");
  asm volatile("s_waitcnt lgkmcnt(0)" ::: "memory");
  __builtin_amdgcn_s_barrier();
  asm volatile("" ::: "memory");
  int o_cur = 0, o_mid = STAGE, o_fill = 2 * STAGE;

#define P256_MFMA_PAIR()                                                                                  \
  _Pragma("unroll") for (int j = 0; j < 2; ++j)                                                           \
    _Pragma("unroll") for (int kk = 0; kk < 4; ++kk)                                                      \
      _Pragma("unroll") for (int t = 0; t < 2; ++t)                                                       \
        _Pragma("unroll") for (int u = 0; u < 2; ++u)                                                     \
          acc[t][u] = __builtin_amdgcn_mfma_f32_32x32x2f32(af[j][t][kk], bf[j][u][kk], acc[t][u], 0, 0, 0);
#define P256_READ_PAIR(g)                                                                                            \
  _Pragma("unroll") for (int j = 0; j < 2; ++j) {                                                                    \
    _Pragma("unroll") for (int t = 0; t < 2; ++t) af[j][t] = *reinterpret_cast<const f32x4*>(cur + a_row + t * 32 * BK + sw[(g) + j]); \
    _Pragma("unroll") for (int u = 0; u < 2; ++u) bf[j][u] = *reinterpret_cast<const f32x4*>(cur + b_row + u * 32 * BK + sw[(g) + j]); \
  }
#define P256_ITERATION()                                                                                  \
  {                                                                                                       \
    const float* const cur = smem + o_cur;                                                                \
    float* const fill = smem + o_fill;                                                                    \
    float resv_none[8] = {0.f, 0.f, 0.f, 0.f, 0.f, 0.f, 0.f, 0.f};                                        \
    (void)resv_none;                                                                                      \
    P256_EPI_LOADS_IF                                                                                     \
    if (!late) request(fill);                                                                             \
    __builtin_amdgcn_sched_barrier(0);                                                                    \
    f32x4 af[2][2], bf[2][2];                                                                             \
    P256_READ_PAIR(0);                                                                                    \
    P256_MFMA_PAIR();                                                                                     \
    __builtin_amdgcn_sched_barrier(0);                                                                    \
    if (late) request(fill);                                                                              \
    __builtin_amdgcn_sched_barrier(0);                                                                    \
    P256_READ_PAIR(2);                                                                                    \
    P256_MFMA_PAIR();                                                                                     \
    p_wait<6>(P256_RESV, sc0, sc1, sh0, sh1);                                                             \
    P256_EPI_FINISH_IF                                                                                    \
    P256_FLUSH_IF                                                                                         \
    cursor_advance();                                                                                     \
    asm volatile("s_waitcnt lgkmcnt(0)" ::: "memory");                                                    \
    __builtin_amdgcn_s_barrier();                                                                         \
    asm volatile("" ::: "memory");                                                                        \
    { const int tmp = o_cur; o_cur = o_mid; o_mid = o_fill; o_fill = tmp; }                               \
  }

  for (int ci = 0; ci < n_items; ++ci) {
    const PItem it = item_at(ci);
    const int nk = it.kt1 - it.kt0;
    static_for<8>([&](auto kc) {
      constexpr int c = decltype(kc)::value;
      if (c < nk) {
        if constexpr (!FLUSH) {
#define P256_EPI_LOADS_IF P256_EPI_LOADS(c)
#define P256_EPI_FINISH_IF P256_EPI_FINISH(c)
#define P256_FLUSH_IF
#define P256_RESV resv
          P256_ITERATION()
#undef P256_EPI_LOADS_IF
#undef P256_EPI_FINISH_IF
#undef P256_FLUSH_IF
#undef P256_RESV
        } else {
#define P256_EPI_LOADS_IF if (c == 0) P256_EPI_SS_LOADS()
#define P256_EPI_FINISH_IF                                                                   \
  if (c == 0) { P256_EPI_FINISH_RV(0, resv_none) P256_EPI_FINISH_RV(1, resv_none) P256_EPI_FINISH_RV(2, resv_none) P256_EPI_FINISH_RV(3, resv_none) } \
  if (c == 1) {                                                                              \
    P256_EPI_FINISH_RV(4, resv_none) P256_EPI_FINISH_RV(5, resv_none) P256_EPI_FINISH_RV(6, resv_none) P256_EPI_FINISH_RV(7, resv_none) \
    _Pragma("unroll") for (int t = 0; t < 2; ++t)                                            \
      _Pragma("unroll") for (int u = 0; u < 2; ++u)                                          \
        _Pragma("unroll") for (int r = 0; r < 16; ++r) acc2[t][u][r] = 0.f;                  \
  }
#define P256_FLUSH_IF if (c & 1) { P256_FLUSH_STEP() }
#define P256_RESV resv_none
          P256_ITERATION()
#undef P256_EPI_LOADS_IF
#undef P256_EPI_FINISH_IF
#undef P256_FLUSH_IF
#undef P256_RESV
        }
      }
    });
    for (int kt = 8; kt < nk; ++kt) {
#define P256_EPI_LOADS_IF
#define P256_EPI_FINISH_IF
#define P256_FLUSH_IF if (kt & 1) { P256_FLUSH_STEP() }
#define P256_RESV resv_none
      P256_ITERATION()
#undef P256_EPI_LOADS_IF
#undef P256_EPI_FINISH_IF
#undef P256_FLUSH_IF
#undef P256_RESV
    }
    if (FLUSH && (nk & 1)) { P256_FLUSH_STEP() }
    if (!FLUSH && nk < 8 && prev_valid) {
      static_for<8>([&](auto kc) {
        constexpr int c = decltype(kc)::value;
        if (c >= nk) {
          P256_EPI_LOADS(c)
          p_wait<0>(resv, sc0, sc1, sh0, sh1);
          P256_EPI_FINISH(c)
        }
      });
    }
    if (!FLUSH) {
#pragma unroll
      for (int t = 0; t < 2; ++t)
#pragma unroll
        for (int u = 0; u < 2; ++u) {
          prev[t][u] = acc[t][u];
#pragma unroll
          for (int r = 0; r < 16; ++r) acc[t][u][r] = 0.f;
        }
    }
    {
      const size_t tile_el = (size_t)it.mt * BM * cout + (size_t)it.nt * BN;
      prev_valid = true;
      prev_raw = it.part >= 0;
      prev_rows = BM;
      if (prev_raw) {
        prev_out = p.partial + (size_t)it.part * (BM * BN);
        prev_os = BN * 4;
        prev_res = p.zeros;
        prev_rs = 0;
      } else {
        if (RAGGED && p.M - it.mt * BM < BM) prev_rows = p.M - it.mt * BM;
        prev_out = p.y + tile_el;
        prev_os = (unsigned)cout * 4;
        prev_res = has_res ? p.res + tile_el : p.zeros;
        prev_rs = has_res ? (unsigned)cout * 4 : 0;
      }
      prev_ss = p.scale + ((p.mt_per_group && p.ss_group_stride) ? (it.mt / p.mt_per_group) * p.ss_group_stride : 0) + it.nt * BN;
    }
  }
  static_for<8>([&](auto kc) {
    constexpr int c = decltype(kc)::value;
    P256_EPI_LOADS(c)
    p_wait<0>(resv, sc0, sc1, sh0, sh1);
    P256_EPI_FINISH(c)
  });
  asm volatile("s_waitcnt vmcnt(0)" ::: "memory");
#undef P256_PREV
#undef P256_FLUSH_STEP
#undef P256_EPI_SS_LOADS
#undef P256_EPI_FINISH_RV
#undef P256_ITERATION
#undef P256_READ_PAIR
#undef P256_MFMA_PAIR
#undef P256_EPI_LOADS
#undef P256_EPI_FINISH
}

}

bool conv_pw_uses_256p(int cout, long long M, int mt_per_group, int bn_tile, int cin, int flush_ktiles, long long in_pixels) {
  const int min_k = (int)opt(OPT_PW256P_MINK);
  if (min_k <= 0 || bn_tile != 128 || cin < min_k || cin < 256) return false;
  if (flush_ktiles != 0 && (flush_ktiles != 2 || cin > opt(OPT_PW256P_FLUSH))) return false;
  if (mt_per_group % 2 != 0) return false;
  if (cout % 128 != 0) return false;
  const long long in_rows = in_pixels > M ? in_pixels : M;
  if (in_rows * (long long)cin * 4 >= (1LL << 32) || M * (long long)cout * 4 >= (1LL << 32)) return false;
  return ((M + 255) / 256) * (cout / 128) >= opt(OPT_PW256P_MINTILES);
}

int launch_conv_pw256p(const ConvKParams& p0, float* ws, size_t ws_floats, hipStream_t stream) {
  ConvKParams p = p0;
  int dev = 0, cus = 0;
  if (hipGetDevice(&dev) != hipSuccess || hipDeviceGetAttribute(&cus, hipDeviceAttributeMultiprocessorCount, dev) != hipSuccess || cus < 8)
    return fail(-3, "conv_pw256p: no current device");
  const int mtiles = (p.M + 255) / 256;
  const int T = mtiles * p.ntiles;
  const int G = cus - cus % 8;
  const int t = T % G;
  int sp = 1;
  if (t > 0) {
    double best = 1e30;
    for (int cand = 1; cand <= 16 && p.nkt / cand >= 4; ++cand) {
      if (ws == nullptr || (size_t)t * cand * 256 * 128 > ws_floats) break;
      const double parts = (double)(((long long)t * cand + G - 1) / G);
      const double cost = parts * ((double)p.nkt / cand + 1.5 + (p.nkt / cand < 8 ? 2.0 : 0.0));
      if (cost < best - 1e-9) { best = cost; sp = cand; }
    }
  }
  p.split_p = sp;
  p.n_sp = t * sp;
  p.n_full = T - t;
  p.sk_units = 0; p.sk_maxp = 0; p.sk_g = 0; p.sk_q = 1;
  const int q = p.flush ? 2 : 1;
  if (t * 4 >= G && opt(OPT_PW256P_STREAMK) != 0 && ws != nullptr && p.nkt % q == 0) {
    const int upt = p.nkt / q;
    const long long U = (long long)t * upt;
    const int Gs = (int)std::min<long long>(G, std::max<long long>(1, U * q / 4));
    const int run = (int)(U / Gs);
    const int maxp = run > 0 ? (upt + run - 1) / run + 1 : 0;
    const double parts_now = (double)(((long long)t * sp + G - 1) / G);
    const double cost_now = parts_now * ((double)p.nkt / sp + 1.5 + (p.nkt / sp < 8 ? 2.0 : 0.0));
    const double cost_stream = (double)((U + Gs - 1) / Gs) * q + 3.0;
    if (run * q >= 4 && (size_t)t * maxp * 256 * 128 <= ws_floats && cost_stream < cost_now - 0.5) {
      p.sk_units = (int)U; p.sk_maxp = maxp; p.sk_g = Gs; p.sk_q = q;
      p.n_sp = 0; p.split_p = 1;
    }
  }
  if (p.n_sp > 0 && (!ws || (size_t)p.n_sp * 256 * 128 > ws_floats)) return fail(-2, "conv_pw256p: split-K scratch too small");
  if (p.n_full / G + (p.n_sp + G - 1) / G + 4 > 120) return 1;
  p.partial = ws;
  p.mtiles = mtiles;
  p.nchunk = (int)opt(OPT_NCHUNK);
  p.phase_shift = opt(OPT_PW256_PHASE) != 0;
  p.p_order = opt(OPT_PW256P_ORDER) != 0;
  note_kernel("conv_pw_glds_256x128p");
  if (p.mt_per_group) p.mt_per_group /= 2;
  const bool ragged = p.M % 256 != 0;
  if (p.flush) {
    if (p.res) return fail(-2, "conv_pw256p: the two-level accumulation variant takes no residual");
    if (ragged) hipLaunchKernelGGL((conv_pw_glds256p_kernel<true, true>), dim3((unsigned)G), dim3(512), 0, stream, p);
    else hipLaunchKernelGGL((conv_pw_glds256p_kernel<false, true>), dim3((unsigned)G), dim3(512), 0, stream, p);
  } else {
    if (ragged) hipLaunchKernelGGL((conv_pw_glds256p_kernel<true, false>), dim3((unsigned)G), dim3(512), 0, stream, p);
    else hipLaunchKernelGGL((conv_pw_glds256p_kernel<false, false>), dim3((unsigned)G), dim3(512), 0, stream, p);
  }
  if (p.n_sp > 0 || p.sk_units > 0)
    hipLaunchKernelGGL((conv_splitk_reduce_kernel<256, 128>), dim3((unsigned)t, 256 / 16), dim3(256), 0, stream, p);
  hipError_t e = hipGetLastError();
  if (e != hipSuccess) return fail(-3, std::string("conv_pw256p launch: ") + hipGetErrorString(e));
  return 0;
}

}
```

peanut_amd/csrc/options.h:

```cpp
#pragma once
#include <stdlib.h>
#include <string.h>

#include <string>

namespace peanut {

enum OptionId {
  OPT_PW_GLDS, OPT_PW256_MINK, OPT_PW256_MINTILES, OPT_PW256_PHASE, OPT_PW256_SKIP_PAD, OPT_PW256W_MINK, OPT_PW256W_MINTILES, OPT_PW256P_MINK, OPT_PW256P_MINTILES, OPT_PW256P_FLUSH, OPT_PW256P_ORDER, OPT_PW256P_STREAMK, OPT_PW256WP_MINK, OPT_PW256WP_MINTILES, OPT_PW256WP_NPRE, OPT_PW256WP_STAGGER, OPT_PW_ARES, OPT_PW_SKINNY,
  OPT_PW_ARES_MINUNITS, OPT_PATCH_MINTILES, OPT_STEM_NCHW, OPT_BN64_MAXK, OPT_PW_BN64_MAXK, OPT_PW64_MAXTILES, OPT_FP32_BK, OPT_NCHUNK, OPT_RES_PREFETCH, OPT_SPLIT_MODEL,
  OPT_RS_CONV, OPT_RS_BN64_MAXK, OPT_RS256_MINK, OPT_RS256_MINTILES, OPT_RS64_MAXK, OPT_RS64_MAXTILES,
  OPT_WINO_M, OPT_WINO_HEAD_M, OPT_WINO6_MAXDIL, OPT_WINO5_MINDIL, OPT_WINO_FLUSH_CH, OPT_WINO_MIN_CIN, OPT_WINO_NARROW_MINPIX, OPT_WINO_SMALL_MAXWG, OPT_DEFER_SPLITK,
  OPT_PPM_OVERLAP, OPT_PPM_GROUPED, OPT_PPM_TERM_ROWS, OPT_PPM_GROUP_ROWS, OPT_RCNN_WINO_M, OPT_RCNN_STEM_S2D, OPT_RCNN_RPN_FUSED, OPT_RCNN_FPN_OVERLAP, OPT_RCNN_RANK_SORT, OPT_RCNN_TOPK_SLICE, OPT_RCNN_NMS_LEVELS, OPT_FMM_LOCAL32, OPT_FMM_MAX_PASSES, OPT_FMM_BLOCKED, OPT_FMM_INNER,
  OPT_COUNT
};

struct OptionInfo {
  const char* key;
  long long def;
  bool upload_time;
  const char* help;
};

inline const OptionInfo* option_table() {
  static const OptionInfo t[OPT_COUNT] = {
      {"pw_glds", 1, false, "fp32 1x1 convs / grouped GEMMs on the LDS-DMA kernels of conv_pw.hip (0: conv_igemm)"},
      {"pw256_mink", 1024, false, "fewest input channels for the 256 x 128 three-stage kernel"},
      {"pw256_mintiles", 256, false, "fewest 256 x 128 tiles for that kernel"},
      {"pw256_phase", 1, false, "the two waves of a SIMD request their LDS-DMA pieces half an iteration apart"},
      {"pw256_skip_pad", 1, false, "256 x 128 kernel, grouped GEMMs: waves whose rows are all group padding issue no MFMAs (0: compute the zero rows)"},
      {"pw256w_mink", 768, false, "fewest input channels for the 256 x 256 two-stage kernel (0: off)"},
      {"pw256w_mintiles", 1536, false, "fewest 256 x 256 tiles for that kernel"},
      {"pw256p_mink", 512, false, "fewest input channels for the persistent 256 x 128 kernel (conv_pw256p.hip; 0: off)"},
      {"pw256p_mintiles", 512, false, "fewest 256 x 128 tiles for that kernel"},
      {"pw256p_flush", 512, false, "most input channels of a Winograd position GEMM (two-level accumulation) that runs on the persistent kernel (0: none)"},
      {"pw256p_order", 1, false, "persistent 256 x 128 kernel: 1 = the workgroups of an XCD walk its run of tiles side by side (neighbours share operand panels in L2), 0 = one contiguous run per workgroup"},
      {"pw256p_streamk", 1, false, "persistent 256 x 128 kernel: the tail tiles' k-tiles as one stream in equal runs per workgroup (0: every tail tile cut into the same number of parts)"},
      {"pw256wp_mink", 512, false, "fewest input channels for the persistent 256 x 256 kernel (conv_pw256wp.hip; 0: off)"},
      {"pw256wp_mintiles", 768, false, "fewest 256 x 256 tiles for that kernel"},
      {"pw256wp_npre", 0, false, "persistent 256 x 256 kernel: accumulator blocks per in-place epilogue group (2 or 4; 0 = two with a residual, four without)"},
      {"pw256wp_stagger", 0, false, "persistent 256 x 256 kernel: spread of the workgroups' start times in sleeps of ~3.4 us (their tile boundaries -- 512 KiB of epilogue traffic per CU -- then fall at different times)"},
      {"pw_ares", 1, false, "K = 128 / 256 pointwise layers on the persistent A-resident kernel (conv_pw_ares.hip)"},
      {"pw_skinny", 1, false, "grouped pointwise launches with at most 64 data rows per group (the PSP pyramid's per-scale convs and Q tables at batch 1) on the skinny weight-streaming kernel (gemm_skinny.hip: 6 KiB of LDS, fits next to any other kernel; 0: the MFMA kernels on 128-row padded tiles)"},
      {"pw_ares_minunits", 512, false, "fewest (m-tile, n-tile) units for that kernel"},
      {"patch_mintiles", 1024, false, "3x3 convs of 16 / 32 input channels on the persistent LDS-patch kernel (conv_patch.hip) from this many 8 x 16 output tiles (0: off)"},
      {"stem_nchw", 1, false, "prediction forward: the first stem conv reads the NCHW input itself (conv_patch.hip, NCHW variant) instead of a layout pass + NHWC conv (fp32 mode, when the patch kernel takes the layer)"},
      {"bn64_maxk", 256, true, "128 x 64 tiles for layers with at most this many input channels"},
      {"pw_bn64_maxk", 128, true, "pointwise layers / Winograd position GEMMs: weights PACKED 64 wide up to this many input channels (wider layers: 128-wide packing, 64-wide tiles chosen per shape)"},
      {"pw64_maxtiles", 512, false, "a 128-wide-packed pointwise layer with at most bn64_maxk input channels runs 128 x 64 tiles while its 128 x 128 tiling has fewer tiles than this (two per CU)"},
      {"fp32_bk", 0, true, "16: force 16-channel k-tiles in conv_igemm (experiment)"},
      {"nchunk", 8, false, "n-tiles per chunk of the tile order (0: n fastest over all n-tiles)"},
      {"res_prefetch", 1, false, "request the first residual rows before the last k-tile's MFMAs"},
      {"split_model", 1, false, "tail split-K plan counts CUs (1) or resident slots (0)"},
      {"rs_conv", 1, true, "emulated modes: non-pointwise convs on conv_rs.hip (0: fp32 MFMA kernel)"},
      {"rs_bn64_maxk", 128, true, "emulated modes: 128 x 64 tiles up to this many input channels"},
      {"rs256_mink", 512, false, "emulated modes: fewest input channels for the 256 x 256 kernel"},
      {"rs256_mintiles", 256, false, "emulated modes: fewest 256 x 256 tiles for it"},
      {"rs64_maxk", 512, false, "emulated modes: 64 x 64 tiles up to this many input channels"},
      {"rs64_maxtiles", 128, false, "emulated modes: ... and below this many 128-row tiles"},
      {"wino_m", 0, true, "4 / 5 / 6: force one Winograd form on every eligible layer (0: policy)"},
      {"wino_head_m", 0, true, "4 / 5 / 6: Winograd form of the PSP bottleneck (0: policy)"},
      {"wino6_maxdil", 4, true, "largest dilation that gets an F(6x6) form"},
      {"wino5_mindil", 4, true, "smallest dilation that also gets an F(5x5) form (0: none)"},
      {"wino_flush_ch", 64, true, "channels per partial sum of the position GEMMs' two-level accumulation (0: off)"},
      {"wino_min_cin", 0, true, "fewest input channels of a Winograd layer (0: the planner's policy)"},
      {"wino_narrow_minpix", 20000, false, "layers under 128 channels take their Winograd form from this many input pixels on (round 6: 100 000 -> 20 000 -- with the small-problem transforms one 720 x 720 map's layer1 conv2, 32 400 pixels, gains 5 us per layer as F(6x6); profiles/r9e)"},
      {"wino_small_maxwg", 1024, false, "Winograd transforms: launches with fewer workgroups than this of the one-thread-per-tile kernels take the small-problem variants (a workgroup per tile and 64-channel slice, a thread per line, through LDS; bit-identical; 0: never)"},
      {"defer_splitk", 1, false, "a Bottleneck conv1 whose every tile is split along k leaves its partial tiles unsummed and conv2's (small-problem) Winograd input transform sums them: one launch fewer per block at batch 1, bit-identical (0: every conv runs its own reduce); read when a (B, H, W) plan is built"},
      {"ppm_overlap", -1, false, "pyramid branch of the PSP head on a side stream: 0 / 1, -1 = by size"},
      {"ppm_grouped", -1, false, "per-scale PSP GEMMs as one grouped launch: 0 / 1, -1 = by size"},
      {"ppm_term_rows", 1, false, "folded pyramid term: one wave per output row, no barrier in the row loop (0: the workgroup-wide two-phase kernel)"},
      {"ppm_group_rows", 0, false, "pyramid pooling, row pass: rows added up per workgroup (1..5; 0 = by size: as many as still leave ~768 workgroups)"},
      {"rcnn_wino_m", 0, true, "detector front end: 4 / 5 / 6 pins one Winograd form (0: per shape)"},
      {"rcnn_stem_s2d", 1, true, "detector stem 7x7 stride 2 as a space-to-depth 4x4 conv"},
      {"rcnn_rpn_fused", 1, false, "detector: the RPN head on all five pyramid levels as one chain (five input transforms, ONE grouped Winograd GEMM, five output transforms, one objectness and one anchor-delta GEMM over all levels' rows: 12 launches instead of 25); read when a (B, H, W) plan is built"},
      {"rcnn_fpn_overlap", 0, false, "detector: the FPN output convs of p5, p4, p3 on a side stream next to the lateral / top-down chain that ends in p2's (round 5 experiment, bit-identical; measured SLOWER at batch 1, 5.70 against 5.61 ms per frame, profiles/r8: off); read when a (B, H, W) plan is built"},
      {"rcnn_rank_sort", 1, false, "detector: the RPN candidates of an image are ordered by counting the larger keys (n / 64 workgroups) instead of one workgroup's bitonic sort (round 5; same order: the keys are distinct)"},
      {"rcnn_topk_slice", 20480, false, "detector: objectness logits per workgroup of the per-level top-k (a level is cut into up to 8 ranges whose k largest are merged by counting; 0: one workgroup per level, round 4)"},
      {"rcnn_nms_levels", 1, false, "detector: the proposal NMS level by level (five 16 x 16-word suppression blocks and five scans per image side by side, post-NMS top-k by counting) instead of one score-sorted list per image (round 5; same proposals)"},
      {"fmm_local32", 1, false, "goal solver: single-precision local solve inside a tile"},
      {"fmm_max_passes", 24, false, "goal solver: hard ceiling of the second-order ordering passes; they stop as soon as a pass changes nothing (6-10 passes on the agent's 960 x 960 map; peanut_goal_converged reports whether they reached their fixed point)"},
      {"fmm_blocked", 1, false, "goal solver: a wave relaxes its 8 x 8 block of the tile to convergence between workgroup barriers (round 5; 0: one Jacobi sweep of the whole tile per barrier pair)"},
      {"fmm_inner", 48, false, "goal solver: iterations a wave spends on its block before it publishes it (blocked rounds)"},
  };
  return t;
}

struct Options {
  long long v[OPT_COUNT];
};

inline int option_index(const char* key) {
  if (!key) return -1;
  std::string k(key);
  for (auto& c : k) c = (char)((c >= 'A' && c <= 'Z') ? c - 'A' + 'a' : c);
  if (k.rfind("peanut_", 0) == 0) k = k.substr(7);
  const OptionInfo* t = option_table();
  for (int i = 0; i < OPT_COUNT; ++i)
    if (k == t[i].key) return i;
  return -1;
}

inline Options& default_options() {
  static Options d = [] {
    Options o;
    const OptionInfo* t = option_table();
    for (int i = 0; i < OPT_COUNT; ++i) {
      o.v[i] = t[i].def;
      std::string env = "PEANUT_";
      for (const char* c = t[i].key; *c; ++c) env += (char)((*c >= 'a' && *c <= 'z') ? *c - 'a' + 'A' : *c);
      const char* e = getenv(env.c_str());
      if (e && *e) o.v[i] = atoll(e);
    }
    return o;
  }();
  return d;
}

inline const Options*& active_options_ptr() {
  static thread_local const Options* p = nullptr;
  return p;
}

inline long long opt(OptionId id) {
  const Options* a = active_options_ptr();
  return (a ? a : &default_options())->v[id];
}

struct OptionScope {
  const Options* saved;
  explicit OptionScope(const Options* o) : saved(active_options_ptr()) { active_options_ptr() = o; }
  ~OptionScope() { active_options_ptr() = saved; }
  OptionScope(const OptionScope&) = delete;
  OptionScope& operator=(const OptionScope&) = delete;
};

}
```

peanut_amd/csrc/pred_api.hip:

```cpp
#include <math.h>
#include <string.h>

#include <map>
#include <memory>
#include <string>
#include <vector>

#include "net_common.h"

namespace peanut {

static thread_local std::string g_err;
void set_error(const std::string& msg) { g_err = msg; }
int fail(int code, const std::string& msg) {
  g_err = msg;
  return code;
}
static thread_local const char* g_kernel = "";
void note_kernel(const char* family) { g_kernel = family; }
const char* noted_kernel() { return g_kernel; }

namespace {

enum OpKind { OP_TO_NHWC, OP_CONV, OP_CONV_NCHW, OP_MAXPOOL, OP_PPM_POOL, OP_PPM_UP, OP_PPM_TERM, OP_UPSAMPLE, OP_WINO_IN, OP_WINO_GEMM, OP_WINO_OUT };

struct Op {
  OpKind kind;
  std::string name;
  std::string kernel;
  const ConvLayer* conv = nullptr;
  Act in, in2, res, out;
  bool has_in2 = false, has_res = false;
  double flops = 0;
  double bytes = 0;
  int wino_mt_per_group = 0;
  int wino_valid_rows = 0;
  int wino_gran = 128;
  int branch = 0;
  bool fork_before = false, join_before = false;
  int group_mt = 0;
  int ppm_scale_rows = 0;
  bool defer_ok = false;
};

struct Plan {
  int B = 0, H = 0, W = 0;
  Act splitk;
  Act splitk2;
  bool keep_all = false;
  size_t bytes = 0;
  std::vector<Op> ops;
  std::map<std::string, Act> named;
};

}
}

using namespace peanut;

struct peanut_conv {
  Options opts = default_options();
  ConvLayer L;
  DevBuf ws;
  DevBuf wino_v, wino_m;
};

struct peanut_pred {
  Options opts = default_options();
  DeferredSplit deferred{};
  peanut_pred_cfg cfg{};
  int cin_pad = 0;
  std::vector<std::unique_ptr<ConvLayer>> convs;
  ConvLayer* stem[3] = {nullptr, nullptr, nullptr};
  struct Block { ConvLayer *c1, *c2, *c3, *down, *c3d; };
  std::vector<std::vector<Block>> layers;
  std::vector<ConvLayer*> ppm;
  ConvLayer* bottleneck = nullptr;
  ConvLayer* bottleneck_x = nullptr;
  std::vector<ConvLayer*> ppm_q;
  std::unique_ptr<ConvLayer> ppm_grouped, ppmq_grouped;
  ConvLayer* conv_seg = nullptr;
  int feat_channels = 0;
  bool keep_all = false;
  std::map<std::string, std::unique_ptr<Plan>> plans;
  Plan* last_plan = nullptr;
  DevBuf ws;
  bool use_graph = false;
  GraphCache graphs;
  bool probe = false;
  Plan* probe_plan = nullptr;
  std::vector<std::vector<hipEvent_t>> probe_events;
  std::vector<hipEvent_t> event_pool;
  hipStream_t side = nullptr;
  hipEvent_t ev_fork = nullptr, ev_join = nullptr;
  ~peanut_pred() {
    for (auto& v : probe_events) for (auto e : v) (void)hipEventDestroy(e);
    for (auto e : event_pool) (void)hipEventDestroy(e);
    if (ev_fork) (void)hipEventDestroy(ev_fork);
    if (ev_join) (void)hipEventDestroy(ev_join);
    if (side) (void)hipStreamDestroy(side);
  }
};

namespace {

int bn_fold(peanut_pred* h, const TensorMap& tm, const std::string& bn, int cout, float* scale, float* shift) {
  return bn_fold_eps(tm, bn, cout, h->cfg.bn_eps, scale, shift);
}

int add_conv(peanut_pred* h, const TensorMap& tm, const std::string& conv, const std::string& bn, int cin,
             int cin_pad, int cout, int k, int stride, int pad, int dil, int relu, ConvLayer** out) {
  int rc = 0;
  const int64_t wshape[4] = {cout, cin, k, k};
  const peanut_tensor* w = tm.get(conv + ".weight", 4, wshape, &rc);
  if (!w) return rc;
  std::vector<float> scale(cout, 1.f), shift(cout, 0.f);
  const int64_t cshape[1] = {cout};
  if (!bn.empty()) {
    if ((rc = bn_fold(h, tm, bn, cout, scale.data(), shift.data()))) return rc;
  } else {
    const peanut_tensor* b = tm.get(conv + ".bias", 1, cshape, &rc); if (!b) return rc;
    for (int n = 0; n < cout; ++n) shift[n] = b->data[n];
  }
  auto L = std::make_unique<ConvLayer>();
  L->name = conv;
  rc = upload_conv(*L, w->data, scale.data(), shift.data(), cout, cin, cin_pad, k, k, stride, pad, dil, relu,
                   h->cfg.precision);
  if (rc) return rc;
  if (h->cfg.conv_algo == PEANUT_ALGO_AUTO && wino_eligible(cin_pad, cout, k, k, stride, pad, dil, h->cfg.precision, 64) &&
      (rc = upload_wino_forms(*L, w->data, scale.data(), shift.data(), cout, cin, cin_pad, pad, dil, relu, h->cfg.precision, 0)))
    return rc;
  *out = L.get();
  h->convs.push_back(std::move(L));
  return 0;
}

int add_fused_c3d(peanut_pred* h, const TensorMap& tm, const std::string& blk, int planes, int inplanes, int cout, ConvLayer** out) {
  int rc = 0;
  const int64_t w3s[4] = {cout, planes, 1, 1}, wds[4] = {cout, inplanes, 1, 1};
  const peanut_tensor* w3 = tm.get(blk + ".conv3.weight", 4, w3s, &rc);
  if (!w3) return rc;
  const peanut_tensor* wd = tm.get(blk + ".downsample.0.weight", 4, wds, &rc);
  if (!wd) return rc;
  std::vector<float> s3(cout), b3(cout), sd(cout), bd(cout);
  if ((rc = bn_fold(h, tm, blk + ".bn3", cout, s3.data(), b3.data()))) return rc;
  if ((rc = bn_fold(h, tm, blk + ".downsample.1", cout, sd.data(), bd.data()))) return rc;
  const int cin = planes + inplanes;
  std::vector<float> w((size_t)cout * cin), shift(cout);
  for (int n = 0; n < cout; ++n) {
    for (int c = 0; c < planes; ++c) w[(size_t)n * cin + c] = s3[n] * w3->data[(size_t)n * planes + c];
    for (int c = 0; c < inplanes; ++c) w[(size_t)n * cin + planes + c] = sd[n] * wd->data[(size_t)n * inplanes + c];
    shift[n] = b3[n] + bd[n];
  }
  auto L = std::make_unique<ConvLayer>();
  L->name = blk + ".conv3+downsample";
  if ((rc = upload_conv(*L, w.data(), nullptr, shift.data(), cout, cin, cin, 1, 1, 1, 0, 1, 1,
                        rs_planes_of(h->cfg.precision) ? h->cfg.precision : PEANUT_PREC_FP32))) return rc;
  *out = L.get();
  h->convs.push_back(std::move(L));
  return 0;
}

std::unique_ptr<ConvLayer> build_grouped(const std::vector<ConvLayer*>& parts, const std::string& name, int* rc) {
  *rc = 0;
  if (parts.size() < 2) return nullptr;
  const ConvDesc& d0 = parts[0]->d;
  for (const ConvLayer* L : parts)
    if (L->d.kh != 1 || L->d.kw != 1 || L->d.cin != d0.cin || L->d.cout != d0.cout || L->d.bn_tile != d0.bn_tile ||
        L->d.bk != d0.bk || L->d.relu != d0.relu || L->w.bytes != parts[0]->w.bytes || L->ss.bytes != parts[0]->ss.bytes)
      return nullptr;
  auto G = std::make_unique<ConvLayer>();
  G->name = name;
  G->d = d0;
  G->cin_real = parts[0]->cin_real;
  const size_t wb = parts[0]->w.bytes, sb = (size_t)d0.cout_pad * sizeof(float), n = parts.size();
  if ((*rc = G->w.ensure(wb * n)) || (*rc = G->ss.ensure(2 * sb * n))) return nullptr;
  for (size_t i = 0; i < n; ++i) {
    if (hipMemcpy((char*)G->w.p + i * wb, parts[i]->w.p, wb, hipMemcpyDeviceToDevice) != hipSuccess ||
        hipMemcpy((char*)G->ss.p + i * sb, parts[i]->d.scale, sb, hipMemcpyDeviceToDevice) != hipSuccess ||
        hipMemcpy((char*)G->ss.p + (n + i) * sb, parts[i]->d.shift, sb, hipMemcpyDeviceToDevice) != hipSuccess) {
      *rc = fail(PEANUT_EHIP, name + ": grouping the per-scale layers failed");
      return nullptr;
    }
  }
  G->d.w_packed = (const float*)G->w.p;
  G->d.scale = (const float*)G->ss.p;
  G->d.shift = (const float*)G->ss.p + n * d0.cout_pad;
  G->d.w_s = nullptr;
  G->d.rs = 0;
  return G;
}

std::string conv_kernel_name(const ConvDesc& d, bool two_source = false, long long M = 0, int mt_per_group = 0, const Act* out = nullptr,
                             bool has_res = false) {
  if (out && !two_source && !has_res) {
    ConvArgs a{};
    a.B = out->B; a.Ho = out->H; a.Wo = out->W;
    if (conv_patch_eligible(d, a)) return conv_patch_kernel_name(d, false);
  }
  if (d.rs == 2) return std::string(d.s_planes == 3 ? "conv_rs6_128x" : (d.s_planes == 4 ? "conv_rs3h_128x" : "conv_rs3_128x")) + std::to_string(d.bn_tile);
  if (d.rs) return gemm_rs_kernel_name(d.cout, M, mt_per_group, d.bn_tile, d.cin, d.s_planes);
  if (d.bk == 32 && d.kh == 1 && d.kw == 1 && d.pad == 0 && (!two_source || d.stride == 1) && d.cin % 32 == 0 && conv_pw_enabled())
  {
    const int flush = d.flush_ch / d.bk;
    if (conv_pw_uses_256wp(d.cout, M, d.stride, mt_per_group, d.bn_tile, d.cin, 0, flush))
      return "conv_pw_glds_256x256p";
    if (conv_pw_uses_ares(d.cin, d.cout, M, d.stride, two_source, flush, d.bn_tile)) return "conv_pw_ares_128x128";
    if (conv_pw_uses_256w(d.cout, M, mt_per_group, d.bn_tile, d.cin, flush)) return "conv_pw_glds_256x256";
    if (conv_pw_uses_256p(d.cout, M, mt_per_group, d.bn_tile, d.cin, flush, M * d.stride * d.stride)) return "conv_pw_glds_256x128p";
    if (conv_pw_uses_256(d.cout, M, mt_per_group, d.bn_tile, d.cin)) return "conv_pw_glds_256x128";
    if (conv_pw_narrow_tiles(d.cin, d.cout, M, d.bn_tile, mt_per_group)) return "conv_pw_glds_128x64";
    return "conv_pw_glds_128x" + std::to_string(d.bn_tile);
  }
  return "conv_igemm_128x" + std::to_string(d.bn_tile) + "x" + std::to_string(d.bk);
}

void push_conv(Plan& pl, const ConvLayer* L, const Act& in, const Act* in2, const Act* res, const Act& out, Arena* ar = nullptr) {
  const bool wino = L->has_wino && !in2 && ar && (long long)in.B * in.H * in.W >= wino_min_pixels(L->d.cin);
  if (wino) L = wino_pick_form(L, in.B, in.H, in.W);
  if (wino) {
    int th, tw;
    long long n_tiles, m_pad;
    const bool rs_gemm = L->wino.rs != 0;
    const int gran = wino_gran_for(*L, in.B, in.H, in.W);
    wino_geometry(in.B, in.H, in.W, L->d.dil, &th, &tw, &n_tiles, &m_pad, gran, L->wino_m);
    const double np = (double)L->wino_np();
    const long long npl = L->wino_np();
    Act v = make_act(*ar, 1, 1, (int)(npl * m_pad), in.C);
    Act m = make_act(*ar, 1, 1, (int)(npl * m_pad), L->d.cout);
    const std::string fam = L->wino_m == 6 ? "wino6_" : (L->wino_m == 5 ? "wino5_" : "wino_");
    const std::string tag = "[" + fam;
    Op a; a.kind = OP_WINO_IN; a.name = L->name + tag + "in]"; a.kernel = fam + "input"; a.conv = L; a.in = in; a.out = v;
    a.wino_gran = gran;
    a.bytes = (double)in.bytes + np * (double)n_tiles * in.C * 4.0;
    pl.ops.push_back(a);
    Op g; g.kind = OP_WINO_GEMM; g.name = L->name + tag + "gemm]"; g.kernel = conv_kernel_name(L->wino, false, npl * m_pad, (int)(m_pad / 128)); g.conv = L;
    g.in = v; g.in.W = (int)(npl * m_pad); g.in.C = in.C; g.out = m; g.wino_mt_per_group = (int)(m_pad / 128); g.wino_gran = gran; g.wino_valid_rows = (int)n_tiles;
    g.flops = 2.0 * np * (double)m_pad * L->d.cout * L->cin_real;
    g.bytes = np * (double)m_pad * (in.C * 4.0 + L->d.cout * 4.0) +
              np * (rs_gemm ? (double)L->wino_group_bytes : (double)L->wino_group_floats * 4);
    pl.ops.push_back(g);
    Op o; o.kind = OP_WINO_OUT; o.name = L->name + tag + "out]"; o.kernel = fam + "output"; o.conv = L; o.in = m; o.out = out;
    if (res) { o.res = *res; o.has_res = true; }
    o.wino_gran = gran;
    o.bytes = np * (double)n_tiles * L->d.cout * 4 + (double)out.bytes + (res ? (double)out.bytes : 0.0);
    pl.ops.push_back(o);
    ar->release(v.off, v.bytes);
    ar->release(m.off, m.bytes);
    return;
  }
  Op op;
  op.kind = OP_CONV; op.name = L->name; op.conv = L; op.in = in; op.out = out;
  op.kernel = conv_kernel_name(L->d, in2 != nullptr, (long long)out.B * out.H * out.W, 0, &out, res != nullptr);
  if (in2) { op.in2 = *in2; op.has_in2 = true; }
  if (res) { op.res = *res; op.has_res = true; }
  op.flops = conv_flops(L, out);
  op.bytes = (double)in.bytes + (in2 ? (double)in2->bytes : 0.0) + (double)out.bytes + (res ? (double)out.bytes : 0.0) +
             (L->d.rs == 2 ? (double)sx_conv_packed_bytes(L->d.cin, L->d.cout, L->d.kh, L->d.kw, L->d.bn_tile, L->d.s_planes)
              : L->d.rs ? (double)sx_packed_bytes(L->d.cin, L->d.cout, L->d.bn_tile, L->d.s_planes)
                      : (double)conv_packed_floats(L->d.cin, L->d.cout, L->d.kh, L->d.kw, L->d.bn_tile) * 4);
  pl.ops.push_back(op);
}

std::unique_ptr<Plan> build_plan(const peanut_pred* h, int B, int H, int W) {
  auto pl = std::make_unique<Plan>();
  pl->B = B; pl->H = H; pl->W = W; pl->keep_all = h->keep_all;
  Arena ar;
  ar.keep_all = h->keep_all;
  auto rel = [&](const Act& t) { ar.release(t.off, t.bytes); };

  pl->splitk.bytes = kSplitKScratchFloats * sizeof(float);
  pl->splitk.off = ar.alloc(pl->splitk.bytes);
  pl->splitk.B = pl->splitk.H = pl->splitk.W = 1; pl->splitk.C = 0;
  const ConvDesc& d0 = h->stem[0]->d;
  const int ho0 = conv_out_dim(H, d0.kh, d0.stride, d0.pad, d0.dil), wo0 = conv_out_dim(W, d0.kw, d0.stride, d0.pad, d0.dil);
  const bool nchw_stem = conv_patch_nchw_eligible(d0, B, ho0, wo0, h->cfg.in_channels);
  Act x{};
  x.B = B; x.H = H; x.W = W; x.C = h->cin_pad;
  if (!nchw_stem) {
    x = make_act(ar, B, H, W, h->cin_pad);
    Op op; op.kind = OP_TO_NHWC; op.name = "nchw_to_nhwc"; op.kernel = "nchw_to_nhwc"; op.out = x;
    op.bytes = (double)B * H * W * h->cfg.in_channels * 4.0 + (double)x.bytes;
    pl->ops.push_back(op);
  }

  for (int i = 0; i < 3; ++i) {
    const ConvDesc& d = h->stem[i]->d;
    Act y = make_act(ar, B, conv_out_dim(x.H, d.kh, d.stride, d.pad, d.dil),
                     conv_out_dim(x.W, d.kw, d.stride, d.pad, d.dil), d.cout);
    if (i == 0 && nchw_stem) {
      Op op; op.kind = OP_CONV_NCHW; op.name = h->stem[0]->name; op.kernel = conv_patch_kernel_name(d, true); op.conv = h->stem[0];
      op.in = x; op.out = y;
      op.flops = conv_flops(h->stem[0], y);
      op.bytes = (double)B * H * W * h->cfg.in_channels * 4.0 + (double)y.bytes + (double)conv_packed_floats(d.cin, d.cout, d.kh, d.kw, d.bn_tile) * 4;
      pl->ops.push_back(op);
    } else {
      push_conv(*pl, h->stem[i], x, nullptr, nullptr, y);
    }
    pl->named["stem" + std::to_string(i)] = y;
    if (!(i == 0 && nchw_stem)) rel(x);
    x = y;
  }
  {
    Act y = make_act(ar, B, conv_out_dim(x.H, 3, 2, 1, 1), conv_out_dim(x.W, 3, 2, 1, 1), x.C);
    Op op; op.kind = OP_MAXPOOL; op.name = "maxpool"; op.kernel = "maxpool"; op.in = x; op.out = y;
    op.bytes = (double)x.bytes + (double)y.bytes;
    pl->ops.push_back(op);
    pl->named["pool"] = y;
    rel(x);
    x = y;
  }
  for (size_t li = 0; li < h->layers.size(); ++li) {
    for (size_t bi = 0; bi < h->layers[li].size(); ++bi) {
      const auto& blk = h->layers[li][bi];
      const ConvDesc& d2 = blk.c2->d;
      Act t1 = make_act(ar, B, x.H, x.W, blk.c1->d.cout);
      push_conv(*pl, blk.c1, x, nullptr, nullptr, t1);
      const int h2 = conv_out_dim(x.H, 3, d2.stride, d2.pad, d2.dil), w2 = conv_out_dim(x.W, 3, d2.stride, d2.pad, d2.dil);
      Act t2 = make_act(ar, B, h2, w2, d2.cout);
      const size_t c1_idx = pl->ops.size() - 1;
      push_conv(*pl, blk.c2, t1, nullptr, nullptr, t2, &ar);
      {
        const Op& win = pl->ops[c1_idx + 1];
        if (opt(OPT_DEFER_SPLITK) != 0 && !h->keep_all && win.kind == OP_WINO_IN && pl->ops[c1_idx].kind == OP_CONV && !win.conv->d.rs &&
            wino_input_accepts_deferred(t1.B, t1.H, t1.W, t1.C, win.conv->d.dil, win.wino_gran, win.conv->wino_m))
          pl->ops[c1_idx].defer_ok = true;
      }
      rel(t1);
      Act idn = x;
      bool own_idn = false;
      const bool fused_c3d = blk.c3d != nullptr && !h->keep_all;
      if (blk.down && !fused_c3d) {
        idn = make_act(ar, B, h2, w2, blk.down->d.cout);
        push_conv(*pl, blk.down, x, nullptr, nullptr, idn);
        own_idn = true;
      }
      Act y = make_act(ar, B, h2, w2, blk.c3->d.cout);
      if (fused_c3d) push_conv(*pl, blk.c3d, t2, &x, nullptr, y);
      else push_conv(*pl, blk.c3, t2, nullptr, &idn, y);
      rel(t2);
      if (own_idn) rel(idn);
      rel(x);
      x = y;
    }
    pl->named["layer" + std::to_string(li + 1)] = x;
  }
  const int overlap_env = (int)opt(OPT_PPM_OVERLAP);
  const bool overlap = h->bottleneck_x != nullptr && (overlap_env >= 0 ? overlap_env == 1 : (long long)B * x.H * x.W >= 4096);
  const size_t side_first = pl->ops.size();
  if (overlap) {
    pl->splitk2.bytes = kSplitKScratchFloats * sizeof(float);
    pl->splitk2.off = ar.alloc(pl->splitk2.bytes);
    pl->splitk2.B = pl->splitk2.H = pl->splitk2.W = 1; pl->splitk2.C = 0;
  }
  std::vector<Act> side_bufs;
  auto rel_side = [&](const Act& t) { if (overlap) side_bufs.push_back(t); else rel(t); };
  int nbins = 0, kmax = 0;
  for (int i = 0; i < h->cfg.n_pool_scales; ++i) {
    nbins += h->cfg.pool_scales[i] * h->cfg.pool_scales[i];
    kmax = std::max(kmax, h->cfg.pool_scales[i]);
  }
  int srows = 0;
  if (h->ppm_grouped && h->ppmq_grouped && !h->keep_all) {
    const int cand = (B * kmax * kmax + 127) / 128 * 128;
    long long separate = 0;
    for (int i = 0; i < h->cfg.n_pool_scales; ++i) separate += ((long long)B * h->cfg.pool_scales[i] * h->cfg.pool_scales[i] + 127) / 128 * 128;
    const int env = (int)opt(OPT_PPM_GROUPED);
    if (env != 0 && ((long long)h->cfg.n_pool_scales * cand <= 2 * separate || env == 1)) srows = cand;
  }
  const int prow = srows ? h->cfg.n_pool_scales * srows : nbins * B;
  Act pooled = make_act(ar, 1, 1, prow, x.C);
  {
    Op op; op.kind = OP_PPM_POOL; op.name = "ppm_pool"; op.kernel = "ppm_pool"; op.in = x; op.out = pooled; op.ppm_scale_rows = srows;
    op.bytes = (double)x.bytes + (double)pooled.bytes;
    const size_t sf = ppm_pool_scratch_floats(B, x.H, x.C, h->cfg.pool_scales, h->cfg.n_pool_scales);
    if (sf) {
      Act scr; scr.B = 1; scr.H = 1; scr.W = 1; scr.C = 0; scr.bytes = sf * sizeof(float); scr.off = ar.alloc(scr.bytes);
      op.in2 = scr; op.has_in2 = true;
      pl->ops.push_back(op);
      rel_side(scr);
    } else {
      pl->ops.push_back(op);
    }
  }
  Act table = make_act(ar, 1, 1, prow, h->cfg.head_channels);
  auto push_grouped = [&](const ConvLayer* G, const Act& in, const Act& out) {
    push_conv(*pl, G, in, nullptr, nullptr, out);
    Op& op = pl->ops.back();
    op.group_mt = srows / 128;
    op.flops = 2.0 * (double)prow * G->d.cout * G->cin_real;
  };
  if (srows) {
    push_grouped(h->ppm_grouped.get(), pooled, table);
  } else {
    size_t row0 = 0;
    for (int i = 0; i < h->cfg.n_pool_scales; ++i) {
      const int k = h->cfg.pool_scales[i];
      Act in = pooled, out = table;
      in.off = pooled.off + row0 * (size_t)x.C * sizeof(float);
      in.H = 1; in.W = k * k; in.C = x.C; in.B = B;
      out.off = table.off + row0 * (size_t)h->cfg.head_channels * sizeof(float);
      out.H = 1; out.W = k * k; out.C = h->cfg.head_channels; out.B = B;
      push_conv(*pl, h->ppm[i], in, nullptr, nullptr, out);
      row0 += (size_t)B * k * k;
    }
  }
  pl->named["ppm_table"] = table;
  rel_side(pooled);
  Act bt;
  int term_scale_rows = 0;
  if (h->bottleneck_x) {
    const int hc = h->cfg.head_channels;
    Act q = make_act(ar, 1, 1, prow, 9 * hc);
    if (srows) {
      push_grouped(h->ppmq_grouped.get(), table, q);
      term_scale_rows = srows;
    } else {
      size_t row0 = 0;
      for (int i = 0; i < h->cfg.n_pool_scales; ++i) {
        const int k = h->cfg.pool_scales[i];
        Act in = table, out = q;
        in.off = table.off + row0 * (size_t)hc * sizeof(float);
        in.H = 1; in.W = k * k; in.C = hc; in.B = B;
        out.off = q.off + row0 * (size_t)(9 * hc) * sizeof(float);
        out.H = 1; out.W = k * k; out.C = 9 * hc; out.B = B;
        push_conv(*pl, h->ppm_q[i], in, nullptr, nullptr, out);
        row0 += (size_t)B * k * k;
      }
    }
    rel_side(table);
    Act r = make_act(ar, B, x.H, x.W, hc);
    {
      Op op; op.kind = OP_PPM_TERM; op.name = "ppm_conv_term"; op.kernel = "ppm_conv_term"; op.in = q; op.out = r; op.ppm_scale_rows = term_scale_rows;
      op.bytes = (double)q.bytes + (double)r.bytes;
      pl->ops.push_back(op);
    }
    rel_side(q);
    const size_t side_end = pl->ops.size();
    bt = make_act(ar, B, x.H, x.W, h->bottleneck_x->d.cout);
    push_conv(*pl, h->bottleneck_x, x, nullptr, &r, bt, &ar);
    if (overlap) {
      for (size_t i = side_first; i < side_end; ++i) pl->ops[i].branch = 1;
      pl->ops[side_first].fork_before = true;
      for (size_t i = side_end; i < pl->ops.size(); ++i)
        if (pl->ops[i].has_res) { pl->ops[i].join_before = true; break; }
      for (const auto& t : side_bufs) rel(t);
    }
    for (size_t i = side_first; i < side_end; ++i) {
      Op& op = pl->ops[i];
      if (op.kind == OP_CONV && op.group_mt == 1 && opt(OPT_PW_SKINNY) != 0 && B * kmax * kmax <= 64 &&
          op.conv->d.bn_tile == 128 && op.conv->d.bk == 32 && op.conv->d.cout % 128 == 0 && (op.conv->d.cin / 32) % 4 == 0)
        op.kernel = "gemm_skinny";
    }
    rel(r);
  } else {
    Act up = make_act(ar, B, x.H, x.W, h->cfg.n_pool_scales * h->cfg.head_channels);
    { Op op; op.kind = OP_PPM_UP; op.name = "ppm_upsample_concat"; op.kernel = "ppm_upsample_concat"; op.in = table; op.out = up; pl->ops.push_back(op); }
    rel(table);
    bt = make_act(ar, B, x.H, x.W, h->bottleneck->d.cout);
    push_conv(*pl, h->bottleneck, x, &up, nullptr, bt);
    rel(up);
  }
  pl->named["bottleneck"] = bt;
  rel(x);
  Act lo = make_act(ar, B, bt.H, bt.W, h->conv_seg->d.cout);
  push_conv(*pl, h->conv_seg, bt, nullptr, nullptr, lo);
  pl->named["logits_lowres"] = lo;
  rel(bt);
  {
    Op op; op.kind = OP_UPSAMPLE; op.name = "upsample_logits"; op.kernel = "upsample_logits"; op.in = lo;
    op.bytes = (double)lo.bytes + (double)B * H * W * h->conv_seg->d.cout * 4.0;
    pl->ops.push_back(op);
  }
  rel(lo);
  return pl;
}

}

static size_t plan_high_water(const Plan& pl) {
  size_t hw = 0;
  auto upd = [&](const Act& a) { if (a.bytes && a.off + Arena::round_up(a.bytes) > hw) hw = a.off + Arena::round_up(a.bytes); };
  for (const auto& op : pl.ops) {
    upd(op.in); upd(op.in2); upd(op.res); upd(op.out);
  }
  for (const auto& kv : pl.named) upd(kv.second);
  upd(pl.splitk);
  upd(pl.splitk2);
  return hw;
}

static Plan* get_plan(peanut_pred* h, int B, int H, int W) {
  if (B <= 0 || H < 16 || W < 16) { set_error("forward: need B >= 1 and H, W >= 16"); return nullptr; }
  const std::string key = std::to_string(B) + "x" + std::to_string(H) + "x" + std::to_string(W) + (h->keep_all ? "k" : "");
  auto it = h->plans.find(key);
  if (it == h->plans.end()) {
    auto pl = build_plan(h, B, H, W);
    pl->bytes = plan_high_water(*pl);
    it = h->plans.emplace(key, std::move(pl)).first;
  }
  return it->second.get();
}

static int run_op(peanut_pred* h, const Plan& pl, const Op& op, const float* in_dev, float* out_dev, int sigmoid,
                  hipStream_t s) {
  char* base = (char*)h->ws.p;
  auto P = [&](const Act& a) { return (float*)(base + a.off); };
  switch (op.kind) {
    case OP_TO_NHWC:
      return launch_nchw_to_nhwc_pad(in_dev, P(op.out), pl.B, h->cfg.in_channels, pl.H, pl.W, h->cin_pad, s);
    case OP_CONV_NCHW:
      return launch_conv_patch_nchw(op.conv->d, in_dev, h->cfg.in_channels, P(op.out), pl.B, pl.H, pl.W, op.out.H, op.out.W, s);
    case OP_CONV: {
      ConvArgs a{};
      a.x = P(op.in);
      a.x2 = op.has_in2 ? P(op.in2) : nullptr;
      a.res = op.has_res ? P(op.res) : nullptr;
      a.y = P(op.out);
      a.B = op.in.B; a.H = op.in.H; a.W = op.in.W;
      a.c1 = op.in.C; a.c2 = op.has_in2 ? op.in2.C : 0;
      a.Ho = op.out.H; a.Wo = op.out.W;
      a.ws = P(op.branch ? pl.splitk2 : pl.splitk); a.ws_floats = kSplitKScratchFloats;
      int scale_rows[8] = {0};
      if (op.group_mt) {
        int most = 0;
        for (int i = 0; i < h->cfg.n_pool_scales && i < 8; ++i) {
          scale_rows[i] = pl.B * h->cfg.pool_scales[i] * h->cfg.pool_scales[i];
          most = std::max(most, scale_rows[i]);
        }
        a.group_valid_rows = most;
        a.group_rows = scale_rows;
        a.mt_per_group = op.group_mt;
        a.w_group_stride = op.conv->w.bytes / sizeof(float) / (size_t)h->cfg.n_pool_scales;
        a.ss_group_stride = op.conv->d.cout_pad;
      }
      if (op.defer_ok) a.defer = &h->deferred;
      return launch_conv(op.conv->d, a, s);
    }
    case OP_WINO_IN: {
      const int rc = launch_wino_input(P(op.in), P(op.out), op.in.B, op.in.H, op.in.W, op.in.C, op.conv->d.dil, s, op.wino_gran, op.conv->wino_m, 0,
                                       h->deferred.valid ? &h->deferred : nullptr);
      h->deferred.valid = false;
      return rc;
    }
    case OP_WINO_GEMM: {
      ConvArgs a{};
      a.x = P(op.in); a.y = P(op.out);
      a.B = 1; a.H = 1; a.W = op.in.W; a.c1 = op.in.C; a.c2 = 0; a.Ho = 1; a.Wo = op.in.W;
      a.ws = P(op.branch ? pl.splitk2 : pl.splitk); a.ws_floats = kSplitKScratchFloats;
      a.mt_per_group = op.wino_mt_per_group;
      a.group_valid_rows = op.wino_valid_rows;
      a.w_group_stride = op.conv->wino.rs ? op.conv->wino_group_bytes : op.conv->wino_group_floats;
      return launch_conv(op.conv->wino, a, s);
    }
    case OP_WINO_OUT:
      return launch_wino_output(P(op.in), op.conv->d.scale, op.conv->d.shift, op.has_res ? P(op.res) : nullptr, P(op.out),
                                op.out.B, op.out.H, op.out.W, op.out.C, op.conv->d.dil, op.conv->d.relu, s, op.wino_gran, op.conv->wino_m);
    case OP_MAXPOOL:
      return launch_maxpool3x3s2(P(op.in), P(op.out), op.in.B, op.in.H, op.in.W, op.in.C, op.out.H, op.out.W, s);
    case OP_PPM_POOL:
      return launch_ppm_pool2(P(op.in), op.has_in2 ? P(op.in2) : nullptr, P(op.out), op.in.B, op.in.H, op.in.W, op.in.C,
                              h->cfg.pool_scales, h->cfg.n_pool_scales, s, op.ppm_scale_rows);
    case OP_PPM_UP:
      return launch_ppm_upsample_concat(P(op.in), P(op.out), op.out.B, op.out.H, op.out.W, h->cfg.head_channels,
                                        h->cfg.pool_scales, h->cfg.n_pool_scales, h->cfg.align_corners, s);
    case OP_PPM_TERM:
      return launch_ppm_conv_term(P(op.in), P(op.out), op.out.B, op.out.H, op.out.W, h->cfg.head_channels,
                                  h->cfg.pool_scales, h->cfg.n_pool_scales, h->cfg.align_corners, s, op.ppm_scale_rows);
    case OP_UPSAMPLE:
      return launch_upsample_logits(P(op.in), out_dev, op.in.B, op.in.H, op.in.W, op.in.C, pl.H, pl.W,
                                    h->cfg.align_corners, sigmoid, s);
  }
  return fail(PEANUT_EINVAL, "unknown op");
}

extern "C" {

const char* peanut_last_error(void) { return g_err.c_str(); }
const char* peanut_last_conv_kernel(void) { return noted_kernel(); }
int peanut_abi_version(void) { return 17; }
const char* peanut_build_arch(void) { return "gfx950"; }
#ifndef PEANUT_SOURCE_HASH
#define PEANUT_SOURCE_HASH ""
#endif
const char* peanut_source_hash(void) { return PEANUT_SOURCE_HASH; }

namespace {
int option_lookup(const char* key, const char* who) {
  const int i = option_index(key);
  if (i < 0) return fail(PEANUT_EINVAL, std::string(who) + ": unknown option '" + (key ? key : "(null)") + "'");
  return i;
}
int handle_set_option(Options& o, const char* key, long long value, const char* who) {
  const int i = option_lookup(key, who);
  if (i < 0) return i;
  if (option_table()[i].upload_time)
    return fail(PEANUT_EINVAL, std::string(who) + ": option '" + option_table()[i].key +
                                   "' shapes the uploaded weights; set it with peanut_set_default_option before creating the handle");
  o.v[i] = value;
  return 0;
}
}

int peanut_set_default_option(const char* key, long long value) {
  const int i = option_lookup(key, "peanut_set_default_option");
  if (i < 0) return i;
  default_options().v[i] = value;
  return 0;
}
int peanut_get_default_option(const char* key, long long* value) {
  const int i = option_lookup(key, "peanut_get_default_option");
  if (i < 0) return i;
  if (value) *value = default_options().v[i];
  return 0;
}
const char* peanut_option_list(void) {
  static const std::string text = [] {
    std::string t;
    const OptionInfo* tab = option_table();
    for (int i = 0; i < OPT_COUNT; ++i)
      t += std::string(tab[i].key) + "=" + std::to_string(tab[i].def) + (tab[i].upload_time ? " [create-time] " : " ") + tab[i].help + "\n";
    return t;
  }();
  return text.c_str();
}
int peanut_pred_set_option(peanut_pred_t* h, const char* key, long long value) {
  if (!h) return fail(PEANUT_EINVAL, "peanut_pred_set_option: null handle");
  if (h->probe) return fail(PEANUT_EINVAL, "peanut_pred_set_option: collect and disable the probe first");
  if (int rc = handle_set_option(h->opts, key, value, "peanut_pred_set_option")) return rc;
  h->graphs.clear();
  h->plans.clear();
  h->last_plan = nullptr;
  h->probe_plan = nullptr;
  return 0;
}
int peanut_pred_get_option(peanut_pred_t* h, const char* key, long long* value) {
  if (!h) return fail(PEANUT_EINVAL, "peanut_pred_get_option: null handle");
  const int i = option_lookup(key, "peanut_pred_get_option");
  if (i < 0) return i;
  if (value) *value = h->opts.v[i];
  return 0;
}
int peanut_conv_set_option(peanut_conv_t* c, const char* key, long long value) {
  if (!c) return fail(PEANUT_EINVAL, "peanut_conv_set_option: null handle");
  return handle_set_option(c->opts, key, value, "peanut_conv_set_option");
}

int peanut_pred_create(peanut_pred_t** out, const peanut_pred_cfg* cfg, const peanut_tensor* tensors, int n) {
  if (!out || !cfg || (!tensors && n > 0)) return fail(PEANUT_EINVAL, "peanut_pred_create: null argument");
  if (cfg->n_pool_scales < 1 || cfg->n_pool_scales > 8) return fail(PEANUT_EINVAL, "n_pool_scales must be 1..8");
  if (cfg->in_channels < 1 || cfg->num_classes < 1 || cfg->num_classes > 32)
    return fail(PEANUT_EINVAL, "in_channels >= 1 and 1 <= num_classes <= 32 required");
  if (cfg->head_channels % 32) return fail(PEANUT_EINVAL, "head_channels must be a multiple of 32");
  if (!precision_known(cfg->precision)) return fail(PEANUT_EINVAL, "precision must be PEANUT_PREC_{FP32,BF16X3,FP16X3,BF16X6}");
  if (cfg->conv_algo != PEANUT_ALGO_AUTO && cfg->conv_algo != PEANUT_ALGO_DIRECT)
    return fail(PEANUT_EINVAL, "conv_algo must be PEANUT_ALGO_{AUTO,DIRECT}");
  auto h = std::make_unique<peanut_pred>();
  OptionScope option_scope(&h->opts);
  h->cfg = *cfg;
  h->cin_pad = (cfg->in_channels + 15) / 16 * 16;
  TensorMap tm;
  for (int i = 0; i < n; ++i)
    if (tensors[i].name) tm.m[tensors[i].name] = &tensors[i];
  int rc;
  const int sc = 64;
  if ((rc = add_conv(h.get(), tm, "backbone.stem.0", "backbone.stem.1", cfg->in_channels, h->cin_pad, sc / 2, 3, 2, 1, 1, 1, &h->stem[0]))) return rc;
  if ((rc = add_conv(h.get(), tm, "backbone.stem.3", "backbone.stem.4", sc / 2, sc / 2, sc / 2, 3, 1, 1, 1, 1, &h->stem[1]))) return rc;
  if ((rc = add_conv(h.get(), tm, "backbone.stem.6", "backbone.stem.7", sc / 2, sc / 2, sc, 3, 1, 1, 1, 1, &h->stem[2]))) return rc;
  const int stage_blocks[4] = {3, 4, 6, 3};
  int inplanes = sc;
  for (int li = 0; li < 4; ++li) {
    const int planes = 64 << li, stride = cfg->strides[li], dilation = cfg->dilations[li];
    if (stride < 1 || dilation < 1) return fail(PEANUT_EINVAL, "strides/dilations must be >= 1");
    const int first_dil = (dilation > 1 && cfg->contract_dilation) ? dilation / 2 : dilation;
    std::vector<peanut_pred::Block> blocks;
    for (int bi = 0; bi < stage_blocks[li]; ++bi) {
      const std::string p = "backbone.layer" + std::to_string(li + 1) + "." + std::to_string(bi);
      const int s = bi == 0 ? stride : 1, d = bi == 0 ? first_dil : dilation;
      peanut_pred::Block b{nullptr, nullptr, nullptr, nullptr, nullptr};
      if ((rc = add_conv(h.get(), tm, p + ".conv1", p + ".bn1", inplanes, inplanes, planes, 1, 1, 0, 1, 1, &b.c1))) return rc;
      if ((rc = add_conv(h.get(), tm, p + ".conv2", p + ".bn2", planes, planes, planes, 3, s, d, d, 1, &b.c2))) return rc;
      if ((rc = add_conv(h.get(), tm, p + ".conv3", p + ".bn3", planes, planes, planes * 4, 1, 1, 0, 1, 1, &b.c3))) return rc;
      if (bi == 0 && (stride != 1 || inplanes != planes * 4)) {
        if ((rc = add_conv(h.get(), tm, p + ".downsample.0", p + ".downsample.1", inplanes, inplanes, planes * 4, 1, stride, 0, 1, 0, &b.down))) return rc;
        if (cfg->conv_algo == PEANUT_ALGO_AUTO && s == 1 && planes % 32 == 0 && inplanes % 32 == 0 && conv_pw_enabled() &&
            (rc = add_fused_c3d(h.get(), tm, p, planes, inplanes, planes * 4, &b.c3d)))
          return rc;
      }
      blocks.push_back(b);
      inplanes = planes * 4;
    }
    h->layers.push_back(blocks);
  }
  h->feat_channels = inplanes;
  const int hc = cfg->head_channels;
  for (int i = 0; i < cfg->n_pool_scales; ++i) {
    if (cfg->pool_scales[i] < 1) return fail(PEANUT_EINVAL, "pool_scales must be >= 1");
    const std::string p = "decode_head.psp_modules." + std::to_string(i) + ".1";
    ConvLayer* L;
    if ((rc = add_conv(h.get(), tm, p + ".conv", p + ".bn", inplanes, inplanes, hc, 1, 1, 0, 1, 1, &L))) return rc;
    h->ppm.push_back(L);
  }
  const int cat = inplanes + cfg->n_pool_scales * hc;
  if (!cfg->fold_ppm) {
    if ((rc = add_conv(h.get(), tm, "decode_head.bottleneck.conv", "decode_head.bottleneck.bn", cat, cat, hc, 3, 1, 1, 1, 1, &h->bottleneck))) return rc;
  } else {
    const int64_t wshape[4] = {hc, cat, 3, 3};
    const peanut_tensor* w = tm.get("decode_head.bottleneck.conv.weight", 4, wshape, &rc);
    if (!w) return rc;
    std::vector<float> scale(hc), shift(hc);
    if ((rc = bn_fold(h.get(), tm, "decode_head.bottleneck.bn", hc, scale.data(), shift.data()))) return rc;
    std::vector<float> wx((size_t)hc * inplanes * 9);
    for (int n = 0; n < hc; ++n)
      memcpy(&wx[(size_t)n * inplanes * 9], &w->data[(size_t)n * cat * 9], (size_t)inplanes * 9 * sizeof(float));
    {
      auto L = std::make_unique<ConvLayer>();
      L->name = "decode_head.bottleneck.conv[x]";
      if ((rc = upload_conv(*L, wx.data(), scale.data(), shift.data(), hc, inplanes, inplanes, 3, 3, 1, 1, 1, 1, cfg->precision))) return rc;
      if (cfg->conv_algo == PEANUT_ALGO_AUTO && wino_eligible(inplanes, hc, 3, 3, 1, 1, 1, cfg->precision) &&
          (rc = upload_wino_forms(*L, wx.data(), scale.data(), shift.data(), hc, inplanes, inplanes, 1, 1, 1, cfg->precision,
                                  wino_head_tile(cfg->precision))))
        return rc;
      h->bottleneck_x = L.get();
      h->convs.push_back(std::move(L));
    }
    std::vector<float> wq((size_t)9 * hc * hc);
    for (int s = 0; s < cfg->n_pool_scales; ++s) {
      for (int tap = 0; tap < 9; ++tap)
        for (int n = 0; n < hc; ++n)
          for (int c = 0; c < hc; ++c)
            wq[((size_t)tap * hc + n) * hc + c] = scale[n] * w->data[((size_t)n * cat + inplanes + (size_t)s * hc + c) * 9 + tap];
      auto L = std::make_unique<ConvLayer>();
      L->name = "decode_head.bottleneck.conv[ppm" + std::to_string(s) + "]";
      if ((rc = upload_conv(*L, wq.data(), nullptr, nullptr, 9 * hc, hc, hc, 1, 1, 1, 0, 1, 0, PEANUT_PREC_FP32))) return rc;
      h->ppm_q.push_back(L.get());
      h->convs.push_back(std::move(L));
    }
  }
  if ((rc = add_conv(h.get(), tm, "decode_head.conv_seg", "", hc, hc, cfg->num_classes, 1, 1, 0, 1, 0, &h->conv_seg))) return rc;
  if (cfg->fold_ppm) {
    h->ppm_grouped = build_grouped(h->ppm, "decode_head.psp_modules.*.1.conv", &rc);
    if (rc) return rc;
    h->ppmq_grouped = build_grouped(h->ppm_q, "decode_head.bottleneck.conv[ppm*]", &rc);
    if (rc) return rc;
  }
  PEANUT_HIP_CHECK(hipDeviceSynchronize());
  *out = h.release();
  return 0;
}

void peanut_pred_destroy(peanut_pred_t* h) { delete h; }

size_t peanut_pred_workspace_bytes(peanut_pred_t* h, int B, int H, int W) {
  if (!h) return 0;
  OptionScope option_scope(&h->opts);
  Plan* pl = get_plan(h, B, H, W);
  return pl ? pl->bytes : 0;
}

double peanut_pred_flops_per_map(peanut_pred_t* h, int H, int W) {
  if (!h) return 0;
  OptionScope option_scope(&h->opts);
  Plan* pl = get_plan(h, 1, H, W);
  if (!pl) return 0;
  double f = 0;
  for (const auto& op : pl->ops) f += op.flops;
  return f;
}

int peanut_pred_debug_keep(peanut_pred_t* h, int keep) {
  if (!h) return fail(PEANUT_EINVAL, "null handle");
  h->keep_all = keep != 0;
  return 0;
}

int peanut_pred_debug_tensor(peanut_pred_t* h, const char* name, const float** dev_out, int dims[4]) {
  if (!h || !name || !dev_out || !dims) return fail(PEANUT_EINVAL, "null argument");
  if (!h->last_plan || !h->last_plan->keep_all) return fail(PEANUT_EINVAL, "debug_tensor: run a forward after peanut_pred_debug_keep(h, 1)");
  auto it = h->last_plan->named.find(name);
  if (it == h->last_plan->named.end()) return fail(PEANUT_EINVAL, std::string("unknown tensor '") + name + "'");
  const Act& a = it->second;
  *dev_out = (const float*)((char*)h->ws.p + a.off);
  dims[0] = a.B; dims[1] = a.H; dims[2] = a.W; dims[3] = a.C;
  return 0;
}

int peanut_pred_debug_read(peanut_pred_t* h, const char* name, float* dst_dev, size_t max_floats, int dims[4],
                           void* stream) {
  const float* src = nullptr;
  int rc = peanut_pred_debug_tensor(h, name, &src, dims);
  if (rc || !dst_dev) return rc;
  const size_t n = (size_t)dims[0] * dims[1] * dims[2] * dims[3];
  if (n > max_floats) return fail(PEANUT_EINVAL, "debug_read: destination too small");
  PEANUT_HIP_CHECK(hipMemcpyAsync(dst_dev, src, n * sizeof(float), hipMemcpyDeviceToDevice, (hipStream_t)stream));
  return 0;
}

int peanut_pred_forward(peanut_pred_t* h, const float* in_dev, float* out_dev, int B, int H, int W, int apply_sigmoid,
                        void* stream) {
  if (!h || !in_dev || !out_dev) return fail(PEANUT_EINVAL, "peanut_pred_forward: null argument");
  OptionScope option_scope(&h->opts);
  Plan* pl = get_plan(h, B, H, W);
  if (!pl) return PEANUT_EINVAL;
  int rc;
  if (pl->bytes > h->ws.bytes) h->graphs.clear();
  if ((rc = h->ws.ensure(pl->bytes))) return rc;
  h->last_plan = pl;
  h->deferred.valid = false;
  hipStream_t s = (hipStream_t)stream;
  if (!h->probe) {
    bool two_streams = false;
    for (const auto& op : pl->ops) two_streams |= op.branch != 0;
    if (two_streams && !h->side) {
      PEANUT_HIP_CHECK(hipStreamCreateWithFlags(&h->side, hipStreamNonBlocking));
      PEANUT_HIP_CHECK(hipEventCreateWithFlags(&h->ev_fork, hipEventDisableTiming));
      PEANUT_HIP_CHECK(hipEventCreateWithFlags(&h->ev_join, hipEventDisableTiming));
    }
    auto enqueue = [&]() -> int {
      for (const auto& op : pl->ops) {
        if (op.fork_before) {
          PEANUT_HIP_CHECK(hipEventRecord(h->ev_fork, s));
          PEANUT_HIP_CHECK(hipStreamWaitEvent(h->side, h->ev_fork, 0));
        }
        if (op.join_before) {
          PEANUT_HIP_CHECK(hipEventRecord(h->ev_join, h->side));
          PEANUT_HIP_CHECK(hipStreamWaitEvent(s, h->ev_join, 0));
        }
        if (int r = run_op(h, *pl, op, in_dev, out_dev, apply_sigmoid, op.branch ? h->side : s)) return r;
      }
      return 0;
    };
    if (!h->use_graph || h->keep_all) return enqueue();
    return h->graphs.run({(uintptr_t)pl, (uintptr_t)in_dev, (uintptr_t)out_dev, (uintptr_t)apply_sigmoid, (uintptr_t)s}, s, enqueue);
  }
  if (h->probe_plan && h->probe_plan != pl) return fail(PEANUT_EINVAL, "probe: shape changed while probing; collect first");
  h->probe_plan = pl;
  std::vector<hipEvent_t> ev(pl->ops.size() + 1);
  for (auto& e : ev) {
    if (!h->event_pool.empty()) { e = h->event_pool.back(); h->event_pool.pop_back(); }
    else PEANUT_HIP_CHECK(hipEventCreate(&e));
  }
  PEANUT_HIP_CHECK(hipEventRecord(ev[0], s));
  for (size_t i = 0; i < pl->ops.size(); ++i) {
    if ((rc = run_op(h, *pl, pl->ops[i], in_dev, out_dev, apply_sigmoid, s))) return rc;
    PEANUT_HIP_CHECK(hipEventRecord(ev[i + 1], s));
  }
  h->probe_events.push_back(std::move(ev));
  return 0;
}

int peanut_pred_use_graph(peanut_pred_t* h, int enable) {
  if (!h) return fail(PEANUT_EINVAL, "null handle");
  h->use_graph = enable != 0;
  if (!h->use_graph) h->graphs.clear();
  return 0;
}

int peanut_pred_probe_enable(peanut_pred_t* h, int enable) {
  if (!h) return fail(PEANUT_EINVAL, "null handle");
  h->probe = enable != 0;
  return 0;
}

int peanut_pred_probe_collect(peanut_pred_t* h, int max_ops, const char** names, const char** kernels, double* ms_sum,
                              double* flops, double* bytes, int* n_forwards) {
  if (!h) return fail(PEANUT_EINVAL, "null handle");
  Plan* pl = h->probe_plan;
  if (!pl || h->probe_events.empty()) { if (n_forwards) *n_forwards = 0; return 0; }
  const int n = (int)pl->ops.size();
  std::vector<double> sum(n, 0.0);
  for (auto& ev : h->probe_events) {
    PEANUT_HIP_CHECK(hipEventSynchronize(ev.back()));
    for (int i = 0; i < n; ++i) {
      float t = 0;
      PEANUT_HIP_CHECK(hipEventElapsedTime(&t, ev[i], ev[i + 1]));
      sum[i] += t;
    }
    for (auto e : ev) h->event_pool.push_back(e);
  }
  if (n_forwards) *n_forwards = (int)h->probe_events.size();
  h->probe_events.clear();
  h->probe_plan = nullptr;
  for (int i = 0; i < n && i < max_ops; ++i) {
    if (names) names[i] = pl->ops[i].name.c_str();
    if (kernels) kernels[i] = pl->ops[i].kernel.c_str();
    if (ms_sum) ms_sum[i] = sum[i];
    if (flops) flops[i] = pl->ops[i].flops;
    if (bytes) bytes[i] = pl->ops[i].bytes;
  }
  return n;
}

int peanut_conv_create(peanut_conv_t** out, const float* w, const float* scale, const float* shift, int cout, int cin,
                       int cin_pad, int kh, int kw, int stride, int pad, int dil, int relu, int precision, int conv_algo) {
  if (!out || !w) return fail(PEANUT_EINVAL, "peanut_conv_create: null argument");
  if (cout < 1 || cin < 1 || kh < 1 || kw < 1 || stride < 1 || dil < 1 || pad < 0)
    return fail(PEANUT_EINVAL, "peanut_conv_create: bad geometry");
  if (!precision_known(precision)) return fail(PEANUT_EINVAL, "peanut_conv_create: bad precision");
  auto c = std::make_unique<peanut_conv>();
  OptionScope option_scope(&c->opts);
  c->L.name = "conv";
  if (conv_algo != PEANUT_ALGO_AUTO && conv_algo != PEANUT_ALGO_DIRECT) return fail(PEANUT_EINVAL, "peanut_conv_create: bad conv_algo");
  int rc = upload_conv(c->L, w, scale, shift, cout, cin, cin_pad, kh, kw, stride, pad, dil, relu, precision);
  if (rc) return rc;
  if (conv_algo == PEANUT_ALGO_AUTO && wino_eligible(cin_pad, cout, kh, kw, stride, pad, dil, precision) &&
      (rc = upload_wino(c->L, w, cout, cin, cin_pad, precision)))
    return rc;
  PEANUT_HIP_CHECK(hipDeviceSynchronize());
  *out = c.release();
  return 0;
}

void peanut_conv_destroy(peanut_conv_t* c) { delete c; }

int peanut_conv_precision(peanut_conv_t* c) {
  if (!c) return PEANUT_EINVAL;
  const ConvDesc& d = (c->L.has_wino && c->L.wino.rs) ? c->L.wino : c->L.d;
  if (d.rs) return precision_of_planes(d.s_planes);
  return PEANUT_PREC_FP32;
}

int peanut_conv_forward(peanut_conv_t* c, const float* x, const float* x2, int c1, const float* res, float* y, int B,
                        int H, int W, void* stream) {
  if (!c || !x || !y) return fail(PEANUT_EINVAL, "peanut_conv_forward: null argument");
  OptionScope option_scope(&c->opts);
  const ConvDesc& d = c->L.d;
  ConvArgs a{};
  a.x = x; a.x2 = x2; a.res = res; a.y = y; a.B = B; a.H = H; a.W = W;
  a.c1 = x2 ? c1 : d.cin;
  a.c2 = x2 ? d.cin - c1 : 0;
  a.Ho = conv_out_dim(H, d.kh, d.stride, d.pad, d.dil);
  a.Wo = conv_out_dim(W, d.kw, d.stride, d.pad, d.dil);
  if (a.Ho < 1 || a.Wo < 1) return fail(PEANUT_EINVAL, "peanut_conv_forward: empty output");
  if (int rc = c->ws.ensure(kSplitKScratchFloats * sizeof(float))) return rc;
  a.ws = (float*)c->ws.p; a.ws_floats = kSplitKScratchFloats;
  if (c->L.has_wino && !x2) {
    size_t vf, mf;
    wino_scratch_floats(c->L, B, H, W, &vf, &mf);
    if (vf * sizeof(float) > c->wino_v.bytes || mf * sizeof(float) > c->wino_m.bytes) PEANUT_HIP_CHECK(hipDeviceSynchronize());
    if (int rc = c->wino_v.ensure(vf * sizeof(float))) return rc;
    if (int rc = c->wino_m.ensure(mf * sizeof(float))) return rc;
  }
  return launch_conv_layer(c->L, a, (float*)c->wino_v.p, (float*)c->wino_m.p, (hipStream_t)stream);
}

int peanut_debug_weight_pieces(const float* values, int n, int precision, unsigned short* pieces, float* pack_scale) {
  const int planes = rs_planes_of(precision);
  if (!values || !pieces || !pack_scale || n < 1 || !planes) return fail(PEANUT_EINVAL, "peanut_debug_weight_pieces: bad arguments");
  const int cin_pad = (n + 15) / 16 * 16, bn = 64, np = planes == 4 ? 2 : planes;
  *pack_scale = sx_pack_scale(values, (size_t)n, planes);
  std::vector<unsigned char> packed(sx_packed_bytes(cin_pad, 1, bn, planes));
  pack_weights_sx(values, 1, n, cin_pad, bn, planes, *pack_scale, packed.data());
  const unsigned short* o = reinterpret_cast<const unsigned short*>(packed.data());
  for (int q = 0; q < 3; ++q)
    for (int c = 0; c < n; ++c)
      pieces[(size_t)q * n + c] = q < np ? o[((size_t)(c / 16) * np + q) * bn * 16 + (c % 16)] : (unsigned short)0;
  return 0;
}

long long peanut_debug_deferred_splitk_count(void) { return wino_deferred_count(); }

int peanut_debug_wino_weights(const float* w_oihw, int cout, int cin, int tile, float* out) {
  if (!w_oihw || !out || cout < 1 || cin < 1 || tile < 4 || tile > 6) return fail(PEANUT_EINVAL, "peanut_debug_wino_weights: bad arguments");
  wino_transform_weights(w_oihw, cout, cin, out, tile);
  return 0;
}

}
```

peanut_amd/ops.py:

```python
from __future__ import annotations

import ctypes as C
from typing import Optional

import numpy as np
import torch

from . import _lib


def round_up(n: int, m: int) -> int:
    return (n + m - 1) // m * m


class FusedConv:

    def __init__(self, weight: torch.Tensor, scale: Optional[torch.Tensor] = None,
                 shift: Optional[torch.Tensor] = None, stride: int = 1, padding: int = 0,
                 dilation: int = 1, relu: bool = False, cin_pad: Optional[int] = None,
                 precision: str = "fp32", conv_algo: str = "auto", device=None, options=None):
        self._lib = _lib.load()
        self.device = torch.device("cuda", torch.cuda.current_device()) if device is None else torch.device(device)
        w = np.ascontiguousarray(weight.detach().cpu().numpy(), dtype=np.float32)
        cout, cin, kh, kw = w.shape
        self.cout, self.cin, self.kh, self.kw = cout, cin, kh, kw
        self.stride, self.padding, self.dilation = stride, padding, dilation
        self.cin_pad = cin_pad if cin_pad is not None else round_up(cin, 16)
        sc = None if scale is None else np.ascontiguousarray(scale.detach().cpu().numpy(), dtype=np.float32)
        sh = None if shift is None else np.ascontiguousarray(shift.detach().cpu().numpy(), dtype=np.float32)
        self._h = C.c_void_p()
        with _lib.default_options(**(options or {})), torch.cuda.device(self.device):
            _lib.check(self._lib.peanut_conv_create(
                C.byref(self._h), w.ctypes.data, None if sc is None else sc.ctypes.data,
                None if sh is None else sh.ctypes.data, cout, cin, self.cin_pad, kh, kw, stride, padding,
                dilation, int(relu), _lib.PRECISIONS[precision], _lib.CONV_ALGOS[conv_algo]), "peanut_conv_create")

    def __del__(self):
        h = getattr(self, "_h", None)
        if h is not None and h.value:
            try:
                self._lib.peanut_conv_destroy(h)
            except Exception:
                pass
            self._h = C.c_void_p()

    def set_option(self, key: str, value: int) -> None:
        _lib.check(self._lib.peanut_conv_set_option(self._h, key.encode(), int(value)), "peanut_conv_set_option")

    def out_hw(self, h: int, w: int):
        def o(n, k):
            return (n + 2 * self.padding - self.dilation * (k - 1) - 1) // self.stride + 1
        return o(h, self.kh), o(w, self.kw)

    def __call__(self, x: torch.Tensor, x2: Optional[torch.Tensor] = None,
                 residual: Optional[torch.Tensor] = None) -> torch.Tensor:
        assert x.is_cuda and x.dtype == torch.float32 and x.is_contiguous() and x.dim() == 4
        if x.device != self.device:
            raise ValueError(f"input lives on {x.device}, the conv's weights on {self.device}")
        b, h, w, c1 = x.shape
        c2 = 0
        if x2 is not None:
            assert x2.is_cuda and x2.is_contiguous() and x2.shape[:3] == x.shape[:3]
            c2 = x2.shape[3]
        if c1 + c2 != self.cin_pad:
            raise ValueError(f"input carries {c1 + c2} channels, conv was built for {self.cin_pad}")
        ho, wo = self.out_hw(h, w)
        y = torch.empty((b, ho, wo, self.cout), dtype=torch.float32, device=x.device)
        if residual is not None:
            assert residual.is_contiguous() and tuple(residual.shape) == tuple(y.shape)
        with torch.cuda.device(x.device):
            rc = self._lib.peanut_conv_forward(
                self._h, x.data_ptr(), None if x2 is None else x2.data_ptr(), c1,
                None if residual is None else residual.data_ptr(), y.data_ptr(), b, h, w,
                _lib.current_stream_ptr(x.device))
        _lib.check(rc, "peanut_conv_forward")
        return y


def to_nhwc_padded(x_nchw: torch.Tensor, cpad: int) -> torch.Tensor:
    b, c, h, w = x_nchw.shape
    y = torch.zeros((b, h, w, cpad), dtype=x_nchw.dtype, device=x_nchw.device)
    y[..., :c] = x_nchw.permute(0, 2, 3, 1)
    return y.contiguous()
```

Before: 886.4 maps/s.

## Fuse strided downsample shortcut into conv3 as a two-source GEMM with separate geometry

Lets the pointwise GEMM read its second source at its own stride and pixel geometry. In the prediction plan this fuses layer2.0's strided 1x1 downsample into conv3, instead of writing the identity tensor and reading it back as a residual. Eligible launches are routed only to the generic pointwise or 256x128p kernels, which gain a GEO2 template path with a second pixel-index array. In exchange, the fused layer loses the skinny, ares and 256w kernel choices, and a new option can switch the fusion off.

```diff
diff --git a/include/peanut_hip.h b/include/peanut_hip.h
--- a/include/peanut_hip.h
+++ b/include/peanut_hip.h
@@ -204,6 +204,8 @@
 int peanut_conv_set_option(peanut_conv_t* c, const char* key, long long value);
 int peanut_conv_forward(peanut_conv_t* c, const float* x_dev, const float* x2_dev, int c1, const float* res_dev,
                         float* y_dev, int B, int H, int W, void* stream);
+int peanut_conv_forward2(peanut_conv_t* c, const float* x_dev, const float* x2_dev, int c1, const float* res_dev, float* y_dev,
+                         int B, int H, int W, int H2, int W2, int s2, void* stream);
 
 typedef struct peanut_goal peanut_goal_t;
 int peanut_goal_create(peanut_goal_t** out, int full_h, int full_w, int col_rad);
diff --git a/peanut_amd/_lib.py b/peanut_amd/_lib.py
--- a/peanut_amd/_lib.py
+++ b/peanut_amd/_lib.py
@@ -10,7 +10,7 @@
 
 _LOCK = threading.Lock()
 _LIB = None
-ABI_VERSION = 17
+ABI_VERSION = 18
 
 
 class PeanutHipError(RuntimeError):
@@ -147,6 +147,7 @@
     "peanut_conv_destroy": (None, [_P]),
     "peanut_conv_precision": (C.c_int, [_P]),
     "peanut_conv_forward": (C.c_int, [_P, _P, _P, C.c_int, _P, _P, C.c_int, C.c_int, C.c_int, _P]),
+    "peanut_conv_forward2": (C.c_int, [_P, _P, _P, C.c_int, _P, _P] + [C.c_int] * 6 + [_P]),
     "peanut_set_default_option": (C.c_int, [C.c_char_p, C.c_longlong]),
     "peanut_get_default_option": (C.c_int, [C.c_char_p, C.POINTER(C.c_longlong)]),
     "peanut_option_list": (C.c_char_p, []),
diff --git a/peanut_amd/csrc/common.h b/peanut_amd/csrc/common.h
--- a/peanut_amd/csrc/common.h
+++ b/peanut_amd/csrc/common.h
@@ -60,6 +60,7 @@
   int group_valid_rows;
   DeferredSplit* defer;
   const int* group_rows;
+  int s2, H2, W2;
 };
 
 constexpr size_t kSplitKScratchFloats = (size_t)48 << 20;
@@ -99,7 +100,7 @@
 int conv_pw_256_min_k();
 bool conv_pw_uses_256w(int cout, long long M, int mt_per_group, int bn_tile, int cin, int flush_ktiles);
 bool conv_pw_narrow_tiles(int cin, int cout, long long M, int bn_tile, int mt_per_group);
-bool conv_pw_uses_256p(int cout, long long M, int mt_per_group, int bn_tile, int cin, int flush_ktiles, long long in_pixels = 0);
+bool conv_pw_uses_256p(int cout, long long M, int mt_per_group, int bn_tile, int cin, int flush_ktiles, long long in_pixels = 0, bool geo2 = false);
 struct ConvKParams;
 bool gemm_skinny_takes(const ConvKParams& p, int bn_tile, size_t ws_floats);
 int launch_gemm_skinny(const ConvKParams& p, float* ws, size_t ws_floats, hipStream_t stream);
diff --git a/peanut_amd/csrc/conv_common.h b/peanut_amd/csrc/conv_common.h
--- a/peanut_amd/csrc/conv_common.h
+++ b/peanut_amd/csrc/conv_common.h
@@ -48,7 +48,10 @@
   int flush;
   DeferredSplit* defer;
   const int* group_rows;
+  int s2, H2, W2;
 };
+
+inline bool conv_geo2(const ConvKParams& p) { return p.c2 != 0 && (p.s2 != p.stride || p.H2 != p.H || p.W2 != p.W); }
 
 template <int I>
 struct IC { static constexpr int value = I; };
diff --git a/peanut_amd/csrc/conv_igemm.hip b/peanut_amd/csrc/conv_igemm.hip
--- a/peanut_amd/csrc/conv_igemm.hip
+++ b/peanut_amd/csrc/conv_igemm.hip
@@ -276,6 +276,15 @@
   p.H = a.H; p.W = a.W; p.c1 = a.c1; p.c2 = a.c2; p.Ho = a.Ho; p.Wo = a.Wo; p.cout = d.cout;
   p.kw = d.kw; p.ntaps = d.kh * d.kw; p.stride = d.stride; p.pad = d.pad; p.dil = d.dil; p.relu = d.relu;
   p.HoWo = a.Ho * a.Wo;
+  p.s2 = a.s2 > 0 ? a.s2 : d.stride; p.H2 = a.H2 > 0 ? a.H2 : a.H; p.W2 = a.W2 > 0 ? a.W2 : a.W;
+  const bool geo2 = conv_geo2(p);
+  if (geo2) {
+    if (d.rs || d.bk != 32 || d.kh != 1 || d.kw != 1 || d.pad != 0 || a.c1 % 32 != 0 || a.c2 % 32 != 0 || a.mt_per_group != 0 || !conv_pw_enabled())
+      return fail(-2, "launch_conv: a second source with its own pixel geometry needs an fp32 pointwise layer with 32-channel k-tiles");
+    if ((long long)(a.Ho - 1) * p.s2 >= p.H2 || (long long)(a.Wo - 1) * p.s2 >= p.W2)
+      return fail(-2, "launch_conv: the second source is smaller than its stride times the output");
+    if ((long long)a.B * p.H2 * p.W2 > 0x7fffffffLL) return fail(-2, "launch_conv: problem size out of range");
+  }
   const long long M = (long long)a.B * p.HoWo;
   if (M <= 0 || M > 0x7fffffffLL || (long long)a.B * a.H * a.W > 0x7fffffffLL)
     return fail(-2, "launch_conv: problem size out of range");
@@ -298,7 +307,7 @@
     if (d.rs == 2) return launch_conv_rs(p, d.bn_tile, d.s_planes, a.ws, a.ws_floats, stream);
     return launch_gemm_rs(p, d.bn_tile, d.s_planes, a.ws, a.ws_floats, stream);
   }
-  if (d.bk == 32 && p.ntaps == 1 && p.pad == 0 && p.c1 % 32 == 0 && p.c2 % 32 == 0 && (p.c2 == 0 || p.stride == 1) && conv_pw_enabled())
+  if (d.bk == 32 && p.ntaps == 1 && p.pad == 0 && p.c1 % 32 == 0 && p.c2 % 32 == 0 && (p.c2 == 0 || p.stride == 1 || geo2) && conv_pw_enabled())
     return launch_conv_pw(p, d.bn_tile, a.ws, a.ws_floats, stream);
   if (conv_patch_eligible(d, a)) return launch_conv_patch(p, d, a.B, stream);
   {
diff --git a/peanut_amd/csrc/conv_pw.hip b/peanut_amd/csrc/conv_pw.hip
--- a/peanut_amd/csrc/conv_pw.hip
+++ b/peanut_amd/csrc/conv_pw.hip
@@ -1,4 +1,6 @@
 #include <stdlib.h>
+
+#include <algorithm>
 
 #include "common.h"
 #include "conv_common.h"
@@ -45,9 +47,10 @@
     const int oy = rem / p.Wo, ox = rem - oy * p.Wo;
     const size_t pix = (size_t)b * p.H * p.W + (size_t)oy * p.stride * p.W + (size_t)ox * p.stride;
     const int c = lp ^ ((r >> 1) & 7);
+    const size_t pix2 = (size_t)b * p.H2 * p.W2 + (size_t)oy * p.s2 * p.W2 + (size_t)ox * p.s2;
     const int k1 = p.c1 / BK;
-    a_src[j] = wk.kt0 < k1 ? p.x + pix * p.c1 + (size_t)wk.kt0 * BK + c * 4 : p.x2 + pix * p.c2 + (size_t)(wk.kt0 - k1) * BK + c * 4;
-    a_src2[j] = p.x2 + pix * p.c2 + c * 4;
+    a_src[j] = wk.kt0 < k1 ? p.x + pix * p.c1 + (size_t)wk.kt0 * BK + c * 4 : p.x2 + pix2 * p.c2 + (size_t)(wk.kt0 - k1) * BK + c * 4;
+    a_src2[j] = p.x2 + pix2 * p.c2 + c * 4;
   }
   int to_switch = p.c2 ? p.c1 / BK - wk.kt0 : 0x7fffffff;
   const float* b_src[B_INSTR];
@@ -444,13 +447,15 @@
 
 int launch_conv_pw(const ConvKParams& p, int bn_tile, float* ws, size_t ws_floats, hipStream_t stream) {
   const int phase_shift_w = opt(OPT_PW256_PHASE) != 0;
-  if (gemm_skinny_takes(p, bn_tile, ws ? ws_floats : 0)) return launch_gemm_skinny(p, ws, ws_floats, stream);
-  if (conv_pw_uses_256wp(p.cout, p.M, p.stride, p.mt_per_group, bn_tile, p.c1, p.c2, p.flush)) {
+  const bool geo2 = conv_geo2(p);
+  const long long in_pixels = std::max((long long)(p.M / p.HoWo) * p.H * p.W, p.c2 ? (long long)(p.M / p.HoWo) * p.H2 * p.W2 : 0LL);
+  if (!geo2 && gemm_skinny_takes(p, bn_tile, ws ? ws_floats : 0)) return launch_gemm_skinny(p, ws, ws_floats, stream);
+  if (!geo2 && conv_pw_uses_256wp(p.cout, p.M, p.stride, p.mt_per_group, bn_tile, p.c1, p.c2, p.flush)) {
     const int rc = launch_conv_pw256wp(p, ws, ws_floats, stream);
     if (rc != 1) return rc;
   }
-  if (conv_pw_uses_ares(p.c1, p.cout, p.M, p.stride, p.c2 != 0, p.flush, bn_tile)) return launch_conv_pw_ares(p, bn_tile, stream);
-  if (conv_pw_uses_256w(p.cout, p.M, p.mt_per_group, bn_tile, p.c1 + p.c2, p.flush)) {
+  if (!geo2 && conv_pw_uses_ares(p.c1, p.cout, p.M, p.stride, p.c2 != 0, p.flush, bn_tile)) return launch_conv_pw_ares(p, bn_tile, stream);
+  if (!geo2 && conv_pw_uses_256w(p.cout, p.M, p.mt_per_group, bn_tile, p.c1 + p.c2, p.flush)) {
     static SlotCache slots256w;
     ConvKParams q = p;
     q.ntiles = p.cout / 256;
@@ -459,11 +464,11 @@
     return launch_with_tail_split<decltype(&conv_pw_glds256w_kernel), 256, 256, 512>(&conv_pw_glds256w_kernel, q, ws, ws_floats, stream,
                                                                                       &slots256w);
   }
-  if (conv_pw_uses_256p(p.cout, p.M, p.mt_per_group, bn_tile, p.c1 + p.c2, p.flush, (long long)(p.M / p.HoWo) * p.H * p.W) && !(p.flush && p.res)) {
+  if (conv_pw_uses_256p(p.cout, p.M, p.mt_per_group, bn_tile, p.c1 + p.c2, p.flush, in_pixels, geo2) && !(p.flush && p.res)) {
     const int rc = launch_conv_pw256p(p, ws, ws_floats, stream);
     if (rc != 1) return rc;
   }
-  if (conv_pw_uses_256(p.cout, p.M, p.mt_per_group, bn_tile, p.c1 + p.c2)) {
+  if (!geo2 && conv_pw_uses_256(p.cout, p.M, p.mt_per_group, bn_tile, p.c1 + p.c2)) {
     static SlotCache slots256;
     ConvKParams q = p;
     if (q.mt_per_group) q.mt_per_group /= 2;
diff --git a/peanut_amd/csrc/conv_pw256p.hip b/peanut_amd/csrc/conv_pw256p.hip
--- a/peanut_amd/csrc/conv_pw256p.hip
+++ b/peanut_amd/csrc/conv_pw256p.hip
@@ -31,7 +31,7 @@
 
 struct PItem { int mt, nt, kt0, kt1, part; };
 
-template <bool RAGGED, bool FLUSH>
+template <bool RAGGED, bool FLUSH, bool GEO2 = false>
 __global__ __launch_bounds__(512) void conv_pw_glds256p_kernel(const ConvKParams p) {
   constexpr int BM = 256, BN = 128, BK = 32, WN = 2;
   constexpr int A_FLOATS = BM * BK, B_FLOATS = BN * BK, STAGE = A_FLOATS + B_FLOATS;
@@ -96,12 +96,13 @@
     return it;
   };
 
-  unsigned a_pix[A_INSTR], a_chunk[A_INSTR], b_off[B_INSTR];
+  unsigned a_pix[A_INSTR], a_pix2[GEO2 ? A_INSTR : 1], a_chunk[A_INSTR], b_off[B_INSTR];
 #pragma unroll
   for (int j = 0; j < A_INSTR; ++j) {
     const int r = (wave * A_INSTR + j) * 8 + lr;
     a_chunk[j] = (unsigned)((lp ^ ((r >> 1) & 7)) * 16);
     a_pix[j] = 0;
+    if (GEO2) a_pix2[j] = 0;
   }
 #pragma unroll
   for (int j = 0; j < B_INSTR; ++j) {
@@ -121,6 +122,7 @@
       const int rem = m - b * p.HoWo;
       const int oy = rem / p.Wo, ox = rem - oy * p.Wo;
       a_pix[j] = (unsigned)(b * p.H * p.W + oy * p.stride * p.W + ox * p.stride);
+      if (GEO2) a_pix2[j] = (unsigned)(b * p.H2 * p.W2 + oy * p.s2 * p.W2 + ox * p.s2);
     }
     d_wtile = p.w + (p.mt_per_group ? (size_t)(it.mt / p.mt_per_group) * p.w_group_stride : 0) + (size_t)it.nt * p.nkt * (BN * BK);
     d_kt = it.kt0;
@@ -135,7 +137,7 @@
     const unsigned cbytes = (unsigned)(second ? p.c2 : p.c1) * 4u;
 #pragma unroll
     for (int j = 0; j < A_INSTR; ++j)
-      __builtin_amdgcn_global_load_lds((gptr_t)(abase + (a_pix[j] * cbytes + a_chunk[j])), (lptr_t)(stage + (wave * A_INSTR + j) * 256), 16, 0, 0);
+      __builtin_amdgcn_global_load_lds((gptr_t)(abase + ((GEO2 && second ? a_pix2[j] : a_pix[j]) * cbytes + a_chunk[j])), (lptr_t)(stage + (wave * A_INSTR + j) * 256), 16, 0, 0);
     const char* bbase = reinterpret_cast<const char*>(d_wtile + (size_t)d_kt * (BN * BK));
 #pragma unroll
     for (int j = 0; j < B_INSTR; ++j)
@@ -395,9 +397,10 @@
 
 }
 
-bool conv_pw_uses_256p(int cout, long long M, int mt_per_group, int bn_tile, int cin, int flush_ktiles, long long in_pixels) {
+bool conv_pw_uses_256p(int cout, long long M, int mt_per_group, int bn_tile, int cin, int flush_ktiles, long long in_pixels, bool geo2) {
   const int min_k = (int)opt(OPT_PW256P_MINK);
-  if (min_k <= 0 || bn_tile != 128 || cin < min_k || cin < 256) return false;
+  if (min_k <= 0 || bn_tile != 128 || (cin < min_k && !geo2) || cin < 256) return false;
+  if (geo2 && (flush_ktiles != 0 || mt_per_group != 0)) return false;
   if (flush_ktiles != 0 && (flush_ktiles != 2 || cin > opt(OPT_PW256P_FLUSH))) return false;
   if (mt_per_group % 2 != 0) return false;
   if (cout % 128 != 0) return false;
@@ -456,8 +459,12 @@
   const bool ragged = p.M % 256 != 0;
   if (p.flush) {
     if (p.res) return fail(-2, "conv_pw256p: the two-level accumulation variant takes no residual");
+    if (conv_geo2(p)) return fail(-2, "conv_pw256p: the two-level accumulation variant reads both sources at the same pixels");
     if (ragged) hipLaunchKernelGGL((conv_pw_glds256p_kernel<true, true>), dim3((unsigned)G), dim3(512), 0, stream, p);
     else hipLaunchKernelGGL((conv_pw_glds256p_kernel<false, true>), dim3((unsigned)G), dim3(512), 0, stream, p);
+  } else if (conv_geo2(p)) {
+    if (ragged) hipLaunchKernelGGL((conv_pw_glds256p_kernel<true, false, true>), dim3((unsigned)G), dim3(512), 0, stream, p);
+    else hipLaunchKernelGGL((conv_pw_glds256p_kernel<false, false, true>), dim3((unsigned)G), dim3(512), 0, stream, p);
   } else {
     if (ragged) hipLaunchKernelGGL((conv_pw_glds256p_kernel<true, false>), dim3((unsigned)G), dim3(512), 0, stream, p);
     else hipLaunchKernelGGL((conv_pw_glds256p_kernel<false, false>), dim3((unsigned)G), dim3(512), 0, stream, p);
diff --git a/peanut_amd/csrc/options.h b/peanut_amd/csrc/options.h
--- a/peanut_amd/csrc/options.h
+++ b/peanut_amd/csrc/options.h
@@ -11,7 +11,7 @@
   OPT_PW_ARES_MINUNITS, OPT_PATCH_MINTILES, OPT_STEM_NCHW, OPT_BN64_MAXK, OPT_PW_BN64_MAXK, OPT_PW64_MAXTILES, OPT_FP32_BK, OPT_NCHUNK, OPT_RES_PREFETCH, OPT_SPLIT_MODEL,
   OPT_RS_CONV, OPT_RS_BN64_MAXK, OPT_RS256_MINK, OPT_RS256_MINTILES, OPT_RS64_MAXK, OPT_RS64_MAXTILES,
   OPT_WINO_M, OPT_WINO_HEAD_M, OPT_WINO6_MAXDIL, OPT_WINO5_MINDIL, OPT_WINO_FLUSH_CH, OPT_WINO_MIN_CIN, OPT_WINO_NARROW_MINPIX, OPT_WINO_SMALL_MAXWG, OPT_DEFER_SPLITK,
-  OPT_PPM_OVERLAP, OPT_PPM_GROUPED, OPT_PPM_TERM_ROWS, OPT_PPM_GROUP_ROWS, OPT_RCNN_WINO_M, OPT_RCNN_STEM_S2D, OPT_RCNN_RPN_FUSED, OPT_RCNN_FPN_OVERLAP, OPT_RCNN_RANK_SORT, OPT_RCNN_TOPK_SLICE, OPT_RCNN_NMS_LEVELS, OPT_FMM_LOCAL32, OPT_FMM_MAX_PASSES, OPT_FMM_BLOCKED, OPT_FMM_INNER,
+  OPT_PPM_OVERLAP, OPT_PPM_GROUPED, OPT_PPM_TERM_ROWS, OPT_PPM_GROUP_ROWS, OPT_RCNN_WINO_M, OPT_RCNN_STEM_S2D, OPT_RCNN_RPN_FUSED, OPT_RCNN_FPN_OVERLAP, OPT_RCNN_RANK_SORT, OPT_RCNN_TOPK_SLICE, OPT_RCNN_NMS_LEVELS, OPT_FMM_LOCAL32, OPT_FMM_MAX_PASSES, OPT_FMM_BLOCKED, OPT_FMM_INNER, OPT_C3D_STRIDED,
   OPT_COUNT
 };
 
@@ -82,6 +82,7 @@
       {"fmm_max_passes", 24, false, "goal solver: hard ceiling of the second-order ordering passes; they stop as soon as a pass changes nothing (6-10 passes on the agent's 960 x 960 map; peanut_goal_converged reports whether they reached their fixed point)"},
       {"fmm_blocked", 1, false, "goal solver: a wave relaxes its 8 x 8 block of the tile to convergence between workgroup barriers (round 5; 0: one Jacobi sweep of the whole tile per barrier pair)"},
       {"fmm_inner", 48, false, "goal solver: iterations a wave spends on its block before it publishes it (blocked rounds)"},
+      {"c3d_strided", 1, false, "prediction forward, fp32: conv3 and the STRIDED 1x1 shortcut of a stage's first block (layer2.0) as one two-source GEMM whose second source is read at the shortcut's stride (0: two layers, the identity tensor written and read back); read when a (B, H, W) plan is built"},
   };
   return t;
 }
diff --git a/peanut_amd/csrc/pred_api.hip b/peanut_amd/csrc/pred_api.hip
--- a/peanut_amd/csrc/pred_api.hip
+++ b/peanut_amd/csrc/pred_api.hip
@@ -31,6 +31,7 @@
   const ConvLayer* conv = nullptr;
   Act in, in2, res, out;
   bool has_in2 = false, has_res = false;
+  int in2_stride = 0;
   double flops = 0;
   double bytes = 0;
   int wino_mt_per_group = 0;
@@ -72,7 +73,7 @@
   int cin_pad = 0;
   std::vector<std::unique_ptr<ConvLayer>> convs;
   ConvLayer* stem[3] = {nullptr, nullptr, nullptr};
-  struct Block { ConvLayer *c1, *c2, *c3, *down, *c3d; };
+  struct Block { ConvLayer *c1, *c2, *c3, *down, *c3d; int c3d_stride; };
   std::vector<std::vector<Block>> layers;
   std::vector<ConvLayer*> ppm;
   ConvLayer* bottleneck = nullptr;
@@ -192,7 +193,7 @@
 }
 
 std::string conv_kernel_name(const ConvDesc& d, bool two_source = false, long long M = 0, int mt_per_group = 0, const Act* out = nullptr,
-                             bool has_res = false) {
+                             bool has_res = false, long long in2_pixels = 0) {
   if (out && !two_source && !has_res) {
     ConvArgs a{};
     a.B = out->B; a.Ho = out->H; a.Wo = out->W;
@@ -203,6 +204,11 @@
   if (d.bk == 32 && d.kh == 1 && d.kw == 1 && d.pad == 0 && (!two_source || d.stride == 1) && d.cin % 32 == 0 && conv_pw_enabled())
   {
     const int flush = d.flush_ch / d.bk;
+    if (in2_pixels > 0 && !d.rs) {
+      if (conv_pw_uses_256p(d.cout, M, mt_per_group, d.bn_tile, d.cin, flush, std::max(in2_pixels, M * d.stride * d.stride), true)) return "conv_pw_glds_256x128p";
+      if (conv_pw_narrow_tiles(d.cin, d.cout, M, d.bn_tile, mt_per_group)) return "conv_pw_glds_128x64";
+      return "conv_pw_glds_128x" + std::to_string(d.bn_tile);
+    }
     if (conv_pw_uses_256wp(d.cout, M, d.stride, mt_per_group, d.bn_tile, d.cin, 0, flush))
       return "conv_pw_glds_256x256p";
     if (conv_pw_uses_ares(d.cin, d.cout, M, d.stride, two_source, flush, d.bn_tile)) return "conv_pw_ares_128x128";
@@ -215,7 +221,7 @@
   return "conv_igemm_128x" + std::to_string(d.bn_tile) + "x" + std::to_string(d.bk);
 }
 
-void push_conv(Plan& pl, const ConvLayer* L, const Act& in, const Act* in2, const Act* res, const Act& out, Arena* ar = nullptr) {
+void push_conv(Plan& pl, const ConvLayer* L, const Act& in, const Act* in2, const Act* res, const Act& out, Arena* ar = nullptr, int in2_stride = 0) {
   const bool wino = L->has_wino && !in2 && ar && (long long)in.B * in.H * in.W >= wino_min_pixels(L->d.cin);
   if (wino) L = wino_pick_form(L, in.B, in.H, in.W);
   if (wino) {
@@ -251,8 +257,9 @@
   }
   Op op;
   op.kind = OP_CONV; op.name = L->name; op.conv = L; op.in = in; op.out = out;
-  op.kernel = conv_kernel_name(L->d, in2 != nullptr, (long long)out.B * out.H * out.W, 0, &out, res != nullptr);
-  if (in2) { op.in2 = *in2; op.has_in2 = true; }
+  op.kernel = conv_kernel_name(L->d, in2 != nullptr, (long long)out.B * out.H * out.W, 0, &out, res != nullptr,
+                               in2 && in2_stride ? (long long)in2->B * in2->H * in2->W : 0);
+  if (in2) { op.in2 = *in2; op.has_in2 = true; op.in2_stride = in2_stride; }
   if (res) { op.res = *res; op.has_res = true; }
   op.flops = conv_flops(L, out);
   op.bytes = (double)in.bytes + (in2 ? (double)in2->bytes : 0.0) + (double)out.bytes + (res ? (double)out.bytes : 0.0) +
@@ -329,14 +336,14 @@
       rel(t1);
       Act idn = x;
       bool own_idn = false;
-      const bool fused_c3d = blk.c3d != nullptr && !h->keep_all;
+      const bool fused_c3d = blk.c3d != nullptr && !h->keep_all && (blk.c3d_stride == 1 || opt(OPT_C3D_STRIDED) != 0);
       if (blk.down && !fused_c3d) {
         idn = make_act(ar, B, h2, w2, blk.down->d.cout);
         push_conv(*pl, blk.down, x, nullptr, nullptr, idn);
         own_idn = true;
       }
       Act y = make_act(ar, B, h2, w2, blk.c3->d.cout);
-      if (fused_c3d) push_conv(*pl, blk.c3d, t2, &x, nullptr, y);
+      if (fused_c3d) push_conv(*pl, blk.c3d, t2, &x, nullptr, y, nullptr, blk.c3d_stride != 1 ? blk.c3d_stride : 0);
       else push_conv(*pl, blk.c3, t2, nullptr, &idn, y);
       rel(t2);
       if (own_idn) rel(idn);
@@ -519,6 +526,7 @@
       a.y = P(op.out);
       a.B = op.in.B; a.H = op.in.H; a.W = op.in.W;
       a.c1 = op.in.C; a.c2 = op.has_in2 ? op.in2.C : 0;
+      if (op.has_in2 && op.in2_stride) { a.s2 = op.in2_stride; a.H2 = op.in2.H; a.W2 = op.in2.W; }
       a.Ho = op.out.H; a.Wo = op.out.W;
       a.ws = P(op.branch ? pl.splitk2 : pl.splitk); a.ws_floats = kSplitKScratchFloats;
       int scale_rows[8] = {0};
@@ -578,7 +586,7 @@
 
 const char* peanut_last_error(void) { return g_err.c_str(); }
 const char* peanut_last_conv_kernel(void) { return noted_kernel(); }
-int peanut_abi_version(void) { return 17; }
+int peanut_abi_version(void) { return 18; }
 const char* peanut_build_arch(void) { return "gfx950"; }
 #ifndef PEANUT_SOURCE_HASH
 #define PEANUT_SOURCE_HASH ""
@@ -677,15 +685,16 @@
     for (int bi = 0; bi < stage_blocks[li]; ++bi) {
       const std::string p = "backbone.layer" + std::to_string(li + 1) + "." + std::to_string(bi);
       const int s = bi == 0 ? stride : 1, d = bi == 0 ? first_dil : dilation;
-      peanut_pred::Block b{nullptr, nullptr, nullptr, nullptr, nullptr};
+      peanut_pred::Block b{nullptr, nullptr, nullptr, nullptr, nullptr, 1};
       if ((rc = add_conv(h.get(), tm, p + ".conv1", p + ".bn1", inplanes, inplanes, planes, 1, 1, 0, 1, 1, &b.c1))) return rc;
       if ((rc = add_conv(h.get(), tm, p + ".conv2", p + ".bn2", planes, planes, planes, 3, s, d, d, 1, &b.c2))) return rc;
       if ((rc = add_conv(h.get(), tm, p + ".conv3", p + ".bn3", planes, planes, planes * 4, 1, 1, 0, 1, 1, &b.c3))) return rc;
       if (bi == 0 && (stride != 1 || inplanes != planes * 4)) {
         if ((rc = add_conv(h.get(), tm, p + ".downsample.0", p + ".downsample.1", inplanes, inplanes, planes * 4, 1, stride, 0, 1, 0, &b.down))) return rc;
-        if (cfg->conv_algo == PEANUT_ALGO_AUTO && s == 1 && planes % 32 == 0 && inplanes % 32 == 0 && conv_pw_enabled() &&
+        if (cfg->conv_algo == PEANUT_ALGO_AUTO && (s == 1 || !rs_planes_of(cfg->precision)) && planes % 32 == 0 && inplanes % 32 == 0 && conv_pw_enabled() &&
             (rc = add_fused_c3d(h.get(), tm, p, planes, inplanes, planes * 4, &b.c3d)))
           return rc;
+        b.c3d_stride = s;
       }
       blocks.push_back(b);
       inplanes = planes * 4;
@@ -944,6 +953,25 @@
   return launch_conv_layer(c->L, a, (float*)c->wino_v.p, (float*)c->wino_m.p, (hipStream_t)stream);
 }
 
+int peanut_conv_forward2(peanut_conv_t* c, const float* x, const float* x2, int c1, const float* res, float* y, int B, int H, int W,
+                         int H2, int W2, int s2, void* stream) {
+  if (!c || !x || !x2 || !y) return fail(PEANUT_EINVAL, "peanut_conv_forward2: null argument");
+  if (H2 < 1 || W2 < 1 || s2 < 1) return fail(PEANUT_EINVAL, "peanut_conv_forward2: bad geometry of the second source");
+  OptionScope option_scope(&c->opts);
+  const ConvDesc& d = c->L.d;
+  if (c1 <= 0 || c1 >= d.cin) return fail(PEANUT_EINVAL, "peanut_conv_forward2: c1 must split the layer's input channels");
+  ConvArgs a{};
+  a.x = x; a.x2 = x2; a.res = res; a.y = y; a.B = B; a.H = H; a.W = W;
+  a.c1 = c1; a.c2 = d.cin - c1;
+  a.s2 = s2; a.H2 = H2; a.W2 = W2;
+  a.Ho = conv_out_dim(H, d.kh, d.stride, d.pad, d.dil);
+  a.Wo = conv_out_dim(W, d.kw, d.stride, d.pad, d.dil);
+  if (a.Ho < 1 || a.Wo < 1) return fail(PEANUT_EINVAL, "peanut_conv_forward2: empty output");
+  if (int rc = c->ws.ensure(kSplitKScratchFloats * sizeof(float))) return rc;
+  a.ws = (float*)c->ws.p; a.ws_floats = kSplitKScratchFloats;
+  return launch_conv(d, a, (hipStream_t)stream);
+}
+
 int peanut_debug_weight_pieces(const float* values, int n, int precision, unsigned short* pieces, float* pack_scale) {
   const int planes = rs_planes_of(precision);
   if (!values || !pieces || !pack_scale || n < 1 || !planes) return fail(PEANUT_EINVAL, "peanut_debug_weight_pieces: bad arguments");
diff --git a/peanut_amd/ops.py b/peanut_amd/ops.py
--- a/peanut_amd/ops.py
+++ b/peanut_amd/ops.py
@@ -53,21 +53,34 @@
         return o(h, self.kh), o(w, self.kw)
 
     def __call__(self, x: torch.Tensor, x2: Optional[torch.Tensor] = None,
-                 residual: Optional[torch.Tensor] = None) -> torch.Tensor:
+                 residual: Optional[torch.Tensor] = None, x2_stride: Optional[int] = None) -> torch.Tensor:
         assert x.is_cuda and x.dtype == torch.float32 and x.is_contiguous() and x.dim() == 4
         if x.device != self.device:
             raise ValueError(f"input lives on {x.device}, the conv's weights on {self.device}")
         b, h, w, c1 = x.shape
         c2 = 0
         if x2 is not None:
-            assert x2.is_cuda and x2.is_contiguous() and x2.shape[:3] == x.shape[:3]
+            assert x2.is_cuda and x2.dtype == torch.float32 and x2.is_contiguous() and x2.dim() == 4
+            assert x2_stride is not None or x2.shape[:3] == x.shape[:3]
             c2 = x2.shape[3]
+        elif x2_stride is not None:
+            raise ValueError("x2_stride needs x2")
         if c1 + c2 != self.cin_pad:
             raise ValueError(f"input carries {c1 + c2} channels, conv was built for {self.cin_pad}")
         ho, wo = self.out_hw(h, w)
         y = torch.empty((b, ho, wo, self.cout), dtype=torch.float32, device=x.device)
         if residual is not None:
             assert residual.is_contiguous() and tuple(residual.shape) == tuple(y.shape)
+        if x2_stride is not None:
+            s2 = int(x2_stride)
+            if x2.shape[0] != b or s2 < 1 or (ho - 1) * s2 >= x2.shape[1] or (wo - 1) * s2 >= x2.shape[2]:
+                raise ValueError(f"x2 {tuple(x2.shape)} read at stride {s2} does not cover the {ho} x {wo} output of batch {b}")
+            with torch.cuda.device(x.device):
+                rc = self._lib.peanut_conv_forward2(
+                    self._h, x.data_ptr(), x2.data_ptr(), c1, None if residual is None else residual.data_ptr(), y.data_ptr(),
+                    b, h, w, x2.shape[1], x2.shape[2], s2, _lib.current_stream_ptr(x.device))
+            _lib.check(rc, "peanut_conv_forward2")
+            return y
         with torch.cuda.device(x.device):
             rc = self._lib.peanut_conv_forward(
                 self._h, x.data_ptr(), None if x2 is None else x2.data_ptr(), c1,
```

Result: no change. 890.4 maps/s, median of 6 (+0.4%).
